# writingindy/SWMHD

Measured on AMD Instinct MI355X. Metric: Mcell-steps/sec (fp64) on 4096^2 periodic grid, higher is better.
Workload: dtype f64

## Files before the change

### include/swmhd.h

```cpp
#ifndef SWMHD_H
#define SWMHD_H

#include <stdint.h>

#ifdef __cplusplus
extern "C" {
#endif

#define SWMHD_VERSION 300

#define SWMHD_FAST 0
#define SWMHD_STRICT 1
#define SWMHD_TILE_KERNEL 2
#define SWMHD_MARCH_KERNEL 4
#define SWMHD_WRAP_X 16
#define SWMHD_WRAP_Y 32
#define SWMHD_BOUNDED_X 256
#define SWMHD_BOUNDED_Y 512
#define SWMHD_GM_IS_PREV_STATE 1024
#define SWMHD_LEAVE_ROOM 64

#define SWMHD_PERIODIC 0
#define SWMHD_BOUNDED 1

#define SWMHD_OK 0
#define SWMHD_EINVAL 1
#define SWMHD_EHALO 2
#define SWMHD_ENOTSUP 3
#define SWMHD_ECOMM 4

int swmhd_version(void);
const char *swmhd_strerror(int rc);

int swmhd_event_create(void **event);
int swmhd_event_record(void *event, void *stream);
int swmhd_event_elapsed_ms(void *start, void *stop, float *ms);
int swmhd_event_destroy(void *event);
int swmhd_probe_fp64_issue(double *scratch, float *ns_per_wave_instruction, void *stream);
int swmhd_probe_copy(void *dst, const void *src, size_t bytes, int reps, float *gbytes_per_s, void *stream);

int swmhd_lorentz_jacobian_f64(const double *A, const double *h, double *Fx, double *Fy,
                               int Nx, int Ny, int Hx, int Hy, int64_t stride_y,
                               double dx, double dy, int flags, void *stream);
int swmhd_lorentz_jacobian_f32(const float *A, const float *h, float *Fx, float *Fy,
                               int Nx, int Ny, int Hx, int Hy, int64_t stride_y,
                               float dx, float dy, int flags, void *stream);
int swmhd_lorentz_jacobian_rows_f64(const double *A, const double *h, double *Fx, double *Fy,
                                    int Nx, int Ny, int Hx, int Hy, int64_t stride_y,
                                    double dx, double dy, int j_begin, int j_end, int flags, void *stream);
int swmhd_lorentz_jacobian_rows_f32(const float *A, const float *h, float *Fx, float *Fy,
                                    int Nx, int Ny, int Hx, int Hy, int64_t stride_y,
                                    float dx, float dy, int j_begin, int j_end, int flags, void *stream);

int swmhd_lorentz_divergence_f64(const double *A, const double *h, double *Fx, double *Fy,
                                 int Nx, int Ny, int Hx, int Hy, int64_t stride_y,
                                 double dx, double dy, int flags, void *stream);
int swmhd_lorentz_divergence_f32(const float *A, const float *h, float *Fx, float *Fy,
                                 int Nx, int Ny, int Hx, int Hy, int64_t stride_y,
                                 float dx, float dy, int flags, void *stream);
int swmhd_lorentz_divergence_rows_f64(const double *A, const double *h, double *Fx, double *Fy,
                                      int Nx, int Ny, int Hx, int Hy, int64_t stride_y,
                                      double dx, double dy, int topo_x, int topo_y,
                                      int j_begin, int j_end, int flags, void *stream);
int swmhd_lorentz_divergence_rows_f32(const float *A, const float *h, float *Fx, float *Fy,
                                      int Nx, int Ny, int Hx, int Hy, int64_t stride_y,
                                      float dx, float dy, int topo_x, int topo_y,
                                      int j_begin, int j_end, int flags, void *stream);

#define SWMHD_HALO_X 1
#define SWMHD_HALO_Y 2
int swmhd_fill_halo_periodic_f64(double *field, int Nx, int Ny, int Hx, int Hy, int64_t stride_y,
                                 int which, void *stream);
int swmhd_fill_halo_periodic_f32(float *field, int Nx, int Ny, int Hx, int Hy, int64_t stride_y,
                                 int which, void *stream);

int swmhd_fill_halo_periodic_multi_f64(double *const *fields, int nfields, int Nx, int Ny, int Hx, int Hy,
                                       int64_t stride_y, int which, void *stream);
int swmhd_fill_halo_periodic_multi_f32(float *const *fields, int nfields, int Nx, int Ny, int Hx, int Hy,
                                       int64_t stride_y, int which, void *stream);

int swmhd_fill_halo_f64(double *const *fields, int nf, int Nx, int Ny, int Hx, int Hy, int64_t stride_y, int topo_x, int topo_y,
                        int face_x, int face_y, const double *gradient, double dx, double dy, void *stream);
int swmhd_fill_halo_f32(float *const *fields, int nf, int Nx, int Ny, int Hx, int Hy, int64_t stride_y, int topo_x, int topo_y,
                        int face_x, int face_y, const float *gradient, float dx, float dy, void *stream);

#define SWMHD_CONSERVATIVE 0
#define SWMHD_VECTOR_INVARIANT 1
#define SWMHD_LORENTZ_NONE 0
#define SWMHD_LORENTZ_JACOBIAN 1
#define SWMHD_LORENTZ_DIVERGENCE 2
int swmhd_tendencies_f64(const double *q1, const double *q2, const double *h, const double *A,
                         double *G1, double *G2, double *Gh, double *GA,
                         int Nx, int Ny, int Hx, int Hy, int64_t stride_y, double dx, double dy,
                         double g, double f, int formulation, int lorentz,
                         int j_begin, int j_end, int flags, void *stream);
int swmhd_tendencies_f32(const float *q1, const float *q2, const float *h, const float *A,
                         float *G1, float *G2, float *Gh, float *GA,
                         int Nx, int Ny, int Hx, int Hy, int64_t stride_y, float dx, float dy,
                         float g, float f, int formulation, int lorentz,
                         int j_begin, int j_end, int flags, void *stream);

int swmhd_rk3_substep_f64(double *const *U, const double *const *Gn, const double *const *Gm,
                          int Nx, int Ny, int Hx, int Hy, int64_t stride_y,
                          double dt, double gamma, double zeta, int j_begin, int j_end, int flags, void *stream);
int swmhd_rk3_substep_f32(float *const *U, const float *const *Gn, const float *const *Gm,
                          int Nx, int Ny, int Hx, int Hy, int64_t stride_y,
                          float dt, float gamma, float zeta, int j_begin, int j_end, int flags, void *stream);

int swmhd_tendencies_rk3_f64(const double *const *q, double *const *qnew, double *const *Gn, const double *const *Gm,
                             int Nx, int Ny, int Hx, int Hy, int64_t stride_y, double dx, double dy,
                             double g, double f, int formulation, int lorentz,
                             double dt, double gamma, double zeta, int store_G,
                             int j_begin, int j_end, int flags, void *stream);
int swmhd_tendencies_rk3_f32(const float *const *q, float *const *qnew, float *const *Gn, const float *const *Gm,
                             int Nx, int Ny, int Hx, int Hy, int64_t stride_y, float dx, float dy,
                             float g, float f, int formulation, int lorentz,
                             float dt, float gamma, float zeta, int store_G,
                             int j_begin, int j_end, int flags, void *stream);

int swmhd_step_rk3_f64(double *const *q, double *const *q_alt, double *const *Ga, double *const *Gb,
                       int Nx, int Ny, int Hx, int Hy, int64_t stride_y, double dx, double dy,
                       double g, double f, int formulation, int lorentz, double dt, int nsteps,
                       int flags, int *state_in_alt, void *stream);
int swmhd_step_rk3_f32(float *const *q, float *const *q_alt, float *const *Ga, float *const *Gb,
                       int Nx, int Ny, int Hx, int Hy, int64_t stride_y, float dx, float dy,
                       float g, float f, int formulation, int lorentz, float dt, int nsteps,
                       int flags, int *state_in_alt, void *stream);

int swmhd_tendency_launch_geometry(int Nx, int rows, int formulation, int elem_size, int flags, int out[8]);

#define SWMHD_RING_ID_BYTES 128
typedef struct swmhd_ring swmhd_ring;
int swmhd_ring_available(const char *rccl_path);
int swmhd_ring_unique_id(const char *rccl_path, void *id128);
int swmhd_ring_create(swmhd_ring **ring, const char *rccl_path, int nranks, int rank, const void *id128);
int swmhd_ring_create_loopback(swmhd_ring **rings, int nranks, double timeout_s);
int swmhd_ring_destroy(swmhd_ring *ring);
const char *swmhd_ring_last_error(const swmhd_ring *ring);
void *swmhd_ring_comm_stream(const swmhd_ring *ring);

int swmhd_ring_exchange_y_f64(swmhd_ring *ring, double *const *fields, int nfields, int Nx, int Ny, int Hx, int Hy,
                              int64_t stride_y, void *stream);
int swmhd_ring_exchange_y_f32(swmhd_ring *ring, float *const *fields, int nfields, int Nx, int Ny, int Hx, int Hy,
                              int64_t stride_y, void *stream);

int swmhd_ring_step_rk3_f64(swmhd_ring *ring, double *const *q, double *const *q_alt, double *const *Ga, double *const *Gb,
                            int Nx, int Ny, int Hx, int Hy, int64_t stride_y, double dx, double dy,
                            double g, double f, int formulation, int lorentz, double dt, int nsteps,
                            int flags, int *state_in_alt, void *stream);
int swmhd_ring_step_rk3_f32(swmhd_ring *ring, float *const *q, float *const *q_alt, float *const *Ga, float *const *Gb,
                            int Nx, int Ny, int Hx, int Hy, int64_t stride_y, float dx, float dy,
                            float g, float f, int formulation, int lorentz, float dt, int nsteps,
                            int flags, int *state_in_alt, void *stream);
int swmhd_ring_join(swmhd_ring *ring, void *stream);

int swmhd_ring_time_launches(swmhd_ring *ring, int max_launches);
int swmhd_ring_launch_times(swmhd_ring *ring, float *ms, int *rows, int capacity);

#define SWMHD_DIAG_NOUT 7
#define SWMHD_DIAG_WORKSPACE (1024 * 7)
int swmhd_diagnostics_f64(const double *q1, const double *q2, const double *h, const double *A,
                          int Nx, int Ny, int Hx, int Hy, int64_t stride_y, double dx, double dy,
                          double g, double h_ref, int formulation, int j_begin, int j_end,
                          double *workspace, double *out, void *stream);
int swmhd_diagnostics_f32(const float *q1, const float *q2, const float *h, const float *A,
                          int Nx, int Ny, int Hx, int Hy, int64_t stride_y, float dx, float dy,
                          float g, float h_ref, int formulation, int j_begin, int j_end,
                          double *workspace, double *out, void *stream);

#ifdef __cplusplus
}
#endif
#endif
```

### swmhd_amd/_lib.py

```python
import ctypes as C
import os

_HERE = os.path.dirname(os.path.abspath(__file__))
LIB_PATH = os.path.join(_HERE, "libswmhd.so")
_LIB = None

STRICT = 1
FAST = 0
TILE_KERNEL = 2
MARCH_KERNEL = 4
WRAP_X, WRAP_Y = 16, 32
LEAVE_ROOM = 64
GM_IS_PREV_STATE = 1024
BOUNDED_X, BOUNDED_Y = 256, 512
KERNEL_FLAGS = {None: 0, "auto": 0, "tile": 2, "march": 4}
PERIODIC, BOUNDED = 0, 1
HALO_X, HALO_Y = 1, 2
DIAG_NOUT, DIAG_WORKSPACE = 7, 1024 * 7
CONSERVATIVE, VECTOR_INVARIANT = 0, 1
LORENTZ_NONE, LORENTZ_JACOBIAN, LORENTZ_DIVERGENCE = 0, 1, 2


def ptr_array(ptrs):
    return (C.c_void_p * len(ptrs))(*ptrs)


class SwmhdError(RuntimeError):
    pass


def _declare(lib):
    p, i, i64 = C.c_void_p, C.c_int, C.c_int64
    lib.swmhd_version.restype = i
    lib.swmhd_strerror.restype = C.c_char_p
    lib.swmhd_strerror.argtypes = [i]
    lib.swmhd_event_create.argtypes = [C.POINTER(p)]
    lib.swmhd_event_record.argtypes = [p, p]
    lib.swmhd_event_elapsed_ms.argtypes = [p, p, C.POINTER(C.c_float)]
    lib.swmhd_event_destroy.argtypes = [p]
    for n in ("create", "record", "elapsed_ms", "destroy"):
        getattr(lib, "swmhd_event_" + n).restype = i
    lib.swmhd_probe_fp64_issue.argtypes = [p, C.POINTER(C.c_float), p]
    lib.swmhd_probe_fp64_issue.restype = i
    lib.swmhd_probe_copy.argtypes = [p, p, C.c_size_t, i, C.POINTER(C.c_float), p]
    lib.swmhd_probe_copy.restype = i
    for sfx, ft in (("f64", C.c_double), ("f32", C.c_float)):
        for form in ("jacobian", "divergence"):
            f = getattr(lib, f"swmhd_lorentz_{form}_{sfx}")
            f.argtypes = [p, p, p, p, i, i, i, i, i64, ft, ft, i, p]
            f.restype = i
        f = getattr(lib, f"swmhd_lorentz_jacobian_rows_{sfx}")
        f.argtypes = [p, p, p, p, i, i, i, i, i64, ft, ft, i, i, i, p]
        f.restype = i
        f = getattr(lib, f"swmhd_lorentz_divergence_rows_{sfx}")
        f.argtypes = [p, p, p, p, i, i, i, i, i64, ft, ft, i, i, i, i, i, p]
        f.restype = i
        f = getattr(lib, f"swmhd_fill_halo_periodic_{sfx}")
        f.argtypes = [p, i, i, i, i, i64, i, p]
        f.restype = i
        f = getattr(lib, f"swmhd_fill_halo_{sfx}")
        f.argtypes = [C.POINTER(p), i, i, i, i, i, i64, i, i, i, i, p, ft, ft, p]
        f.restype = i
        f = getattr(lib, f"swmhd_fill_halo_periodic_multi_{sfx}")
        f.argtypes = [C.POINTER(p), i, i, i, i, i, i64, i, p]
        f.restype = i
        f = getattr(lib, f"swmhd_tendencies_{sfx}")
        f.argtypes = [p] * 8 + [i, i, i, i, i64, ft, ft, ft, ft, i, i, i, i, i, p]
        f.restype = i
        f = getattr(lib, f"swmhd_tendencies_rk3_{sfx}")
        f.argtypes = [C.POINTER(p)] * 4 + [i, i, i, i, i64, ft, ft, ft, ft, i, i, ft, ft, ft, i, i, i, i, p]
        f.restype = i
        f = getattr(lib, f"swmhd_step_rk3_{sfx}")
        f.argtypes = [C.POINTER(p)] * 4 + [i, i, i, i, i64, ft, ft, ft, ft, i, i, ft, i, i, C.POINTER(i), p]
        f.restype = i
        f = getattr(lib, f"swmhd_diagnostics_{sfx}")
        f.argtypes = [p, p, p, p, i, i, i, i, i64, ft, ft, ft, ft, i, i, i, p, p, p]
        f.restype = i
        f = getattr(lib, f"swmhd_rk3_substep_{sfx}")
        f.argtypes = [C.POINTER(p), C.POINTER(p), C.POINTER(p), i, i, i, i, i64, ft, ft, ft, i, i, i, p]
        f.restype = i
        f = getattr(lib, f"swmhd_ring_exchange_y_{sfx}")
        f.argtypes = [p, C.POINTER(p), i, i, i, i, i, i64, p]
        f.restype = i
        f = getattr(lib, f"swmhd_ring_step_rk3_{sfx}")
        f.argtypes = [p] + [C.POINTER(p)] * 4 + [i, i, i, i, i64, ft, ft, ft, ft, i, i, ft, i, i, C.POINTER(i), p]
        f.restype = i
    lib.swmhd_tendency_launch_geometry.argtypes = [i, i, i, i, i, C.POINTER(i)]
    lib.swmhd_tendency_launch_geometry.restype = i
    lib.swmhd_ring_available.argtypes = [C.c_char_p]
    lib.swmhd_ring_available.restype = i
    lib.swmhd_ring_unique_id.argtypes = [C.c_char_p, p]
    lib.swmhd_ring_unique_id.restype = i
    lib.swmhd_ring_create.argtypes = [C.POINTER(p), C.c_char_p, i, i, p]
    lib.swmhd_ring_create.restype = i
    lib.swmhd_ring_create_loopback.argtypes = [C.POINTER(p), i, C.c_double]
    lib.swmhd_ring_create_loopback.restype = i
    lib.swmhd_ring_destroy.argtypes = [p]
    lib.swmhd_ring_destroy.restype = i
    lib.swmhd_ring_last_error.argtypes = [p]
    lib.swmhd_ring_last_error.restype = C.c_char_p
    lib.swmhd_ring_comm_stream.argtypes = [p]
    lib.swmhd_ring_comm_stream.restype = p
    lib.swmhd_ring_join.argtypes = [p, p]
    lib.swmhd_ring_join.restype = i
    lib.swmhd_ring_time_launches.argtypes = [p, i]
    lib.swmhd_ring_time_launches.restype = i
    lib.swmhd_ring_launch_times.argtypes = [p, C.POINTER(C.c_float), C.POINTER(i), i]
    lib.swmhd_ring_launch_times.restype = i


EXPORTS = ["swmhd_version", "swmhd_strerror", "swmhd_tendency_launch_geometry", "swmhd_probe_fp64_issue", "swmhd_probe_copy"] + ["swmhd_event_" + n for n in ("create", "record", "elapsed_ms", "destroy")] + [
    f"swmhd_{name}_{sfx}" for sfx in ("f64", "f32") for name in (
        "lorentz_jacobian", "lorentz_jacobian_rows", "lorentz_divergence", "lorentz_divergence_rows",
        "fill_halo", "fill_halo_periodic", "fill_halo_periodic_multi", "tendencies", "tendencies_rk3", "rk3_substep", "step_rk3", "diagnostics",
        "ring_exchange_y", "ring_step_rk3")] + [
    "swmhd_ring_" + name for name in ("available", "unique_id", "create", "create_loopback", "destroy", "last_error", "comm_stream", "join", "time_launches",
                                      "launch_times")]
RING_ID_BYTES = 128


class TimingEvent:

    def __init__(self):
        self._e = C.c_void_p()
        check(lib().swmhd_event_create(C.byref(self._e)), "swmhd_event_create")

    def record(self, stream=None):
        if stream is None:
            import torch
            stream = torch.cuda.current_stream().cuda_stream
        check(lib().swmhd_event_record(self._e, C.c_void_p(stream)), "swmhd_event_record")

    def elapsed_time(self, stop):
        ms = C.c_float()
        check(lib().swmhd_event_elapsed_ms(self._e, stop._e, C.byref(ms)), "swmhd_event_elapsed_ms")
        return ms.value

    def __del__(self):
        try:
            if self._e:
                lib().swmhd_event_destroy(self._e)
        except Exception:
            pass


def lib():
    global _LIB
    if _LIB is None:
        path = os.environ.get("SWMHD_LIBRARY", LIB_PATH)
        if not os.path.exists(path):
            raise SwmhdError(
                f"{path} not found: build it with `python -c 'import __graft_entry__ as g; g.build()'` "
                "(hipcc --offload-arch=gfx950).  swmhd_amd has no CPU fallback.")
        _LIB = C.CDLL(path)
        _declare(_LIB)
    return _LIB


def tendency_launch_geometry(Nx, rows, formulation, elem_size=8, flags=0):
    out = (C.c_int * 8)()
    check(lib().swmhd_tendency_launch_geometry(Nx, rows, formulation, elem_size, flags, out), "swmhd_tendency_launch_geometry")
    keys = ("kind", "threads", "nstrips", "nseg", "rows_per_segment", "wg_per_cu", "halo_lanes", "cus")
    return dict(zip(keys, list(out)))


def source_hash():
    import glob, hashlib
    h = hashlib.sha256()
    src = os.path.join(_HERE, "csrc")
    for f in sorted(glob.glob(os.path.join(src, "*.hip")) + glob.glob(os.path.join(src, "*.inc")) + glob.glob(os.path.join(src, "*.hpp"))
                    + [os.path.join(src, "Makefile")]):
        h.update(os.path.basename(f).encode()); h.update(open(f, "rb").read())
    return h.hexdigest()[:16]


def check(rc, what=""):
    if rc != 0:
        raise SwmhdError(f"{what}: rc={rc}: {lib().swmhd_strerror(rc).decode()}")
```

### swmhd_amd/csrc/common.hpp

```cpp
#pragma once
#include <hip/hip_runtime.h>
#include <stdint.h>
#include <stdio.h>
#include <stdlib.h>

namespace swmhd {

template <typename T>
struct OpArgs {
    const T *A;
    const T *h;
    T *Fx;
    T *Fy;
    int Nx, Ny, Hx, Hy;
    long sy;
    T dx, dy, rdx, rdy;
    int j0, j1;
    int topo_x, topo_y;
    int kernel_variant;
    int edge_cols;
};

template <typename T> hipError_t launch_lorentz_jacobian_fast(const OpArgs<T> &a, hipStream_t s);
template <typename T> hipError_t launch_lorentz_jacobian_strict(const OpArgs<T> &a, hipStream_t s);
template <typename T> hipError_t launch_lorentz_divergence_fast(const OpArgs<T> &a, hipStream_t s);
template <typename T> hipError_t launch_lorentz_divergence_strict(const OpArgs<T> &a, hipStream_t s);

template <typename T>
hipError_t launch_fill_halo_periodic(T *interior, int Nx, int Ny, int Hx, int Hy, long sy, int which, hipStream_t s);
template <typename T>
hipError_t launch_fill_halo_periodic_multi(T *const *interiors, int nfields, int Nx, int Ny, int Hx, int Hy, long sy,
                                           int which, hipStream_t s);
template <typename T>
struct HaloBc {
    T *f[4];
    T grad[4][4];
    int nf, Nx, Ny, Hx, Hy, topo_x, topo_y, face_x, face_y;
    long sy;
    T dx, dy;
};
template <typename T> hipError_t launch_fill_halo_bc(const HaloBc<T> &a, hipStream_t s);

template <typename T>
struct TendArgs {
    const T *q1, *q2, *h, *A;
    T *G1, *G2, *Gh, *GA;
    int Nx, Ny, Hx, Hy;
    long sy;
    T dx, dy, rdx, rdy, grav, fcor;
    int j0, j1;
    int j0b, j1b;
    int fuse, first, store_G;
    int gm_prev;
    int drop_G;
    int wrap;
    int kernel_variant;
    int topo_x, topo_y;
    int leave_room;
    int edge_cols;
    T *Unew[4];
    const T *Gm[4];
    T dt, gamma, zeta;
    T dtg;
    T cu, cg;
};
constexpr int GM_IS_PREV_STATE = 1024;
template <typename T>
struct Rk3Stage {
    T gamma, zeta;
    int store_G;
    const T *const *Gm;
    int flags;
};
template <typename T>
struct Rk3Buffers {
    T *cur[4], *alt[4], *gn[4], *gm[4];
    int swaps = 0;
    bool set(T *const *q, T *const *q_alt, T *const *Ga, T *const *Gb) {
        for (int f = 0; f < 4; ++f) {
            if (!q[f] || !q_alt[f] || !Ga[f] || !Gb[f]) return false;
            cur[f] = q[f]; alt[f] = q_alt[f]; gn[f] = Ga[f]; gm[f] = Gb[f];
        }
        return true;
    }
    Rk3Stage<T> stage(int st, bool from_state) const {
        const T gam[3] = {T(8.0 / 15.0), T(5.0 / 12.0), T(3.0 / 4.0)};
        const T zet[3] = {T(0), T(-17.0 / 60.0), T(-5.0 / 12.0)};
        const bool fs = from_state && st == 1;
        return {gam[st], fs ? zet[1] / gam[0] : zet[st], (st == 1 || (st == 0 && !from_state)) ? 1 : 0,
                st == 0 ? nullptr : (fs ? alt : gm), fs ? GM_IS_PREV_STATE : 0};
    }
    void rotate() {
        for (int f = 0; f < 4; ++f) { T *t = cur[f]; cur[f] = alt[f]; alt[f] = t; t = gn[f]; gn[f] = gm[f]; gm[f] = t; }
        ++swaps;
    }
};

template <typename T>
struct Rk3Args {
    T *U[4];
    const T *Gn[4];
    const T *Gm[4];
    int Nx;
    long sy;
    int j0, j1;
    T dt, gamma, zeta;
    int first;
};
typedef int sw_v2i __attribute__((ext_vector_type(2)));
typedef float sw_f2 __attribute__((ext_vector_type(2)));
typedef sw_f2 sw_f2_u __attribute__((aligned(4)));
constexpr unsigned SW_OOB = 0xFFFFFFC0u;
template <typename T> __device__ __forceinline__ __amdgpu_buffer_rsrc_t out_rsrc(T *parent, unsigned bytes) {
    return __builtin_amdgcn_make_buffer_rsrc(parent, 0, (int)bytes, 0x00020000);
}
template <typename T> __device__ __forceinline__ void buffer_store(T v, __amdgpu_buffer_rsrc_t r, unsigned off) {
    if constexpr (sizeof(T) == 8) __builtin_amdgcn_raw_buffer_store_b64(__builtin_bit_cast(sw_v2i, v), r, off, 0, 0);
    else __builtin_amdgcn_raw_buffer_store_b32(__builtin_bit_cast(int, v), r, off, 0, 0);
}
template <int N> __device__ __forceinline__ void wait_vmem_all_but() {
    static_assert(N >= 0 && N < 64, "vmcnt is a 6-bit counter");
    __builtin_amdgcn_s_waitcnt((N & 15) | ((N >> 4) << 14) | (7 << 4) | (15 << 8));
}

struct ProgressPriority {
    int t1, t2, t3;
    __device__ __forceinline__ explicit ProgressPriority(int niter)
        : t1((niter * 3) / 5), t2((niter * 17) / 20), t3((niter * 19) / 20) {
        __builtin_amdgcn_s_setprio(3);
    }
    __device__ __forceinline__ void at(int it) const {
        if (it == t1) __builtin_amdgcn_s_setprio(2);
        if (it == t2) __builtin_amdgcn_s_setprio(1);
        if (it == t3) __builtin_amdgcn_s_setprio(0);
    }
};

struct MarchGeometry {
    int nt;
    int nstrips, nseg, LY;
    int wg_per_cu;
};
inline int device_cu_count() {
    static int cus = 0;
    if (cus <= 0) {
        int dev = 0, n = 0;
        if (hipGetDevice(&dev) != hipSuccess || hipDeviceGetAttribute(&n, hipDeviceAttributeMultiprocessorCount, dev) != hipSuccess || n <= 0)
            n = 256;
        cus = n;
    }
    return cus;
}
inline int env_knob(const char *name, int &cache) {
    if (cache == 0) {
        const char *e = getenv(name);
        const int v = e ? atoi(e) : 0;
        cache = v > 0 ? v : -1;
    }
    return cache > 0 ? cache : 0;
}
inline int leave_room_64ths(int rows) {
    static int cache = 0;
    const int v = env_knob("SWMHD_RING_ROOM", cache);
    return v > 0 ? (v < 32 ? v : 32) : (rows >= 3072 ? 1 : 3);
}
inline MarchGeometry march_geometry(int Nx, int rows, int xh, const int *nts, const int *wgs, int ncand, int ly_min, bool leave_room,
                                    int force_nt, int force_ly) {
    MarchGeometry g{};
    long best = -1;
    for (int k = 0; k < ncand; ++k) {
        const int txo = nts[k] - 2 * xh, ns = (Nx + txo - 1) / txo;
        const long lanes = (long)ns * nts[k];
        const bool take = force_nt ? nts[k] == force_nt : (best < 0 || lanes * 20 <= best * 19);
        if (take) { best = lanes; g.nt = nts[k]; g.nstrips = ns; g.wg_per_cu = wgs[k]; }
    }
    if (best < 0) { g.nt = nts[0]; g.nstrips = (Nx + nts[0] - 2 * xh - 1) / (nts[0] - 2 * xh); g.wg_per_cu = wgs[0]; }
    int slots = device_cu_count() * g.wg_per_cu;
    if (leave_room) slots -= (slots * leave_room_64ths(rows)) / 64;
    int LY = 32;
    for (int k = 1; k <= 64; ++k) {
        const int ns = (slots * k) / g.nstrips;
        if (ns < 1) continue;
        const int ly = (rows + ns - 1) / ns;
        if (ly <= 128) { LY = ly < ly_min ? ly_min : ly; break; }
    }
    if (force_ly > 0) LY = force_ly;
    g.LY = LY;
    g.nseg = (rows + LY - 1) / LY;
    return g;
}

template <typename T> hipError_t launch_tendency_fast(const TendArgs<T> &a, int formulation, int lorentz, hipStream_t s);
int tendency_launch_geometry(int Nx, int rows, int formulation, int elem_size, int kernel_variant, int leave_room, int wrap, int out[8]);
template <typename T> hipError_t launch_tendency_strict(const TendArgs<T> &a, int formulation, int lorentz, hipStream_t s);
template <typename T> hipError_t launch_rk3_substep_fast(const Rk3Args<T> &a, hipStream_t s);
template <typename T>
int tendencies_rk3_two_ranges(const T *const *q, T *const *qnew, T *const *Gn, const T *const *Gm, int Nx, int Ny, int Hx, int Hy, long sy,
                              T dx, T dy, T grav, T fcor, int formulation, int lorentz, T dt, T gamma, T zeta, int store_G, int j0, int j1,
                              int j0b, int j1b, int flags, void *stream);
template <typename T>
int fill_halo_periodic_multi(T *const *f, int nf, int Nx, int Ny, int Hx, int Hy, long sy, int which, void *stream);
template <typename T> hipError_t launch_rk3_substep_strict(const Rk3Args<T> &a, hipStream_t s);

template <typename T>
hipError_t launch_diagnostics(const T *q1, const T *q2, const T *h, const T *A, int Nx, int Ny, int j0, int j1, long sy, T dx, T dy,
                              T grav, T href, int form, double *workspace, double *out, hipStream_t s);

__device__ __forceinline__ int wrap_index(int v, int n, int lo, int hi, bool wrap) {
    if (wrap) v = v < 0 ? v + n : (v >= n ? v - n : v);
    return v < lo ? lo : (v > hi ? hi : v);
}

__device__ __forceinline__ unsigned xcd_remap(unsigned bid, unsigned nblk) {
    constexpr unsigned NXCD = 8;
    unsigned q = nblk / NXCD, r = nblk % NXCD;
    unsigned x = bid % NXCD, k = bid / NXCD;
    unsigned base = x < r ? x * (q + 1) : r * (q + 1) + (x - r) * q;
    return base + k;
}

}
```

### swmhd_amd/csrc/ring.hip

```cpp
#include "common.hpp"
#include "../../include/swmhd.h"
#include <chrono>
#include <condition_variable>
#include <cstring>
#include <dlfcn.h>
#include <memory>
#include <mutex>
#include <new>
#include <rccl/rccl.h>
#include <string>
#include <vector>

namespace {

struct RcclApi {
    void *handle = nullptr;
    ncclResult_t (*GetUniqueId)(ncclUniqueId *) = nullptr;
    ncclResult_t (*CommInitRank)(ncclComm_t *, int, ncclUniqueId, int) = nullptr;
    ncclResult_t (*CommDestroy)(ncclComm_t) = nullptr;
    ncclResult_t (*GroupStart)() = nullptr;
    ncclResult_t (*GroupEnd)() = nullptr;
    ncclResult_t (*Send)(const void *, size_t, ncclDataType_t, int, ncclComm_t, hipStream_t) = nullptr;
    ncclResult_t (*Recv)(void *, size_t, ncclDataType_t, int, ncclComm_t, hipStream_t) = nullptr;
    const char *(*GetErrorString)(ncclResult_t) = nullptr;
};

bool load_rccl(const char *path, RcclApi &api, std::string &err) {
    const char *candidates[] = {path, "librccl.so.1", "librccl.so"};
    for (const char *c : candidates) {
        if (!c || !*c) continue;
        api.handle = dlopen(c, RTLD_NOW | RTLD_LOCAL);
        if (api.handle) break;
        err = dlerror();
    }
    if (!api.handle) return false;
#define SW_SYM(field, name)                                                                \
    api.field = reinterpret_cast<decltype(api.field)>(dlsym(api.handle, name));           \
    if (!api.field) { err = std::string("missing symbol ") + name; return false; }
    SW_SYM(GetUniqueId, "ncclGetUniqueId")
    SW_SYM(CommInitRank, "ncclCommInitRank")
    SW_SYM(CommDestroy, "ncclCommDestroy")
    SW_SYM(GroupStart, "ncclGroupStart")
    SW_SYM(GroupEnd, "ncclGroupEnd")
    SW_SYM(Send, "ncclSend")
    SW_SYM(Recv, "ncclRecv")
    SW_SYM(GetErrorString, "ncclGetErrorString")
#undef SW_SYM
    return true;
}

struct LoopHub {
    static constexpr int MAXF = 8, SLOTS = 4;
    struct Post {
        unsigned long seq = 0;
        unsigned long done = 0;
        const char *send_s[SLOTS][MAXF] = {}, *send_n[SLOTS][MAXF] = {};
        size_t bytes[SLOTS] = {};
        int nf[SLOTS] = {};
        hipEvent_t ready[SLOTS] = {}, consumed[SLOTS] = {};
    };
    std::mutex mu;
    std::condition_variable cv;
    std::vector<Post> post;
    double timeout_s = 60.0;
    explicit LoopHub(int n) : post(n) {}
    ~LoopHub() {
        for (auto &p : post)
            for (int k = 0; k < SLOTS; ++k) { if (p.ready[k]) (void)hipEventDestroy(p.ready[k]); if (p.consumed[k]) (void)hipEventDestroy(p.consumed[k]); }
    }
};

}

struct swmhd_ring {
    RcclApi api;
    ncclComm_t comm = nullptr;
    std::shared_ptr<LoopHub> hub;
    int nranks = 1, rank = 0, south = 0, north = 0;
    hipStream_t comm_stream = nullptr;
    hipEvent_t ev_main = nullptr, ev_comm = nullptr;
    const void *pending = nullptr;
    std::string err;
    std::vector<hipEvent_t> t0, t1;
    std::vector<int> trows;
    size_t tcap = 0;
};

namespace {

int fail(swmhd_ring *r, const char *what, ncclResult_t rc) {
    r->err = std::string(what) + ": " + (r->api.GetErrorString ? r->api.GetErrorString(rc) : "rccl error");
    return SWMHD_ECOMM;
}
int hipfail(swmhd_ring *r, const char *what, hipError_t e) {
    r->err = std::string(what) + ": " + hipGetErrorString(e);
    return -(int)e;
}

template <typename T> constexpr ncclDataType_t nccl_type();
template <> constexpr ncclDataType_t nccl_type<double>() { return ncclFloat64; }
template <> constexpr ncclDataType_t nccl_type<float>() { return ncclFloat32; }

int loopback_exchange(swmhd_ring *r, const char *const *send_s, const char *const *send_n, char *const *recv_s, char *const *recv_n,
                      int nf, size_t bytes, hipStream_t s) {
    LoopHub &h = *r->hub;
    if (nf > LoopHub::MAXF) return SWMHD_EINVAL;
    hipError_t e;
    unsigned long k;
    int slot;
    {
        std::unique_lock<std::mutex> lk(h.mu);
        LoopHub::Post &me = h.post[r->rank];
        k = me.seq + 1; slot = (int)(k % LoopHub::SLOTS);
        if (!me.ready[slot] && (e = hipEventCreateWithFlags(&me.ready[slot], hipEventDisableTiming)) != hipSuccess) return hipfail(r, "loopback event", e);
        if (!me.consumed[slot] && (e = hipEventCreateWithFlags(&me.consumed[slot], hipEventDisableTiming)) != hipSuccess) return hipfail(r, "loopback event", e);
        if ((e = hipEventRecord(me.ready[slot], s)) != hipSuccess) return hipfail(r, "loopback record", e);
        for (int f = 0; f < nf; ++f) { me.send_s[slot][f] = send_s[f]; me.send_n[slot][f] = send_n[f]; }
        me.bytes[slot] = bytes; me.nf[slot] = nf;
        me.seq = k;
    }
    h.cv.notify_all();
    const auto deadline = std::chrono::steady_clock::now() + std::chrono::duration<double>(h.timeout_s);
    auto wait_for = [&](auto pred, const char *what) {
        std::unique_lock<std::mutex> lk(h.mu);
        if (!h.cv.wait_until(lk, deadline, pred)) {
            r->err = std::string("loopback exchange ") + std::to_string(k) + " of rank " + std::to_string(r->rank) + ": " + what +
                     " (every ring of the hub must be driven from its own host thread, and all of them must make the same calls)";
            return false;
        }
        return true;
    };
    const int peers[2] = {r->south, r->north};
    for (int side = 0; side < 2; ++side) {
        const int p = peers[side];
        if (!wait_for([&] { return h.post[p].seq >= k; }, "a neighbour did not reach its matching exchange")) return SWMHD_ECOMM;
        hipEvent_t ready; const char *src[LoopHub::MAXF]; size_t pbytes; int pnf;
        {
            std::unique_lock<std::mutex> lk(h.mu);
            const LoopHub::Post &pp = h.post[p];
            ready = pp.ready[slot]; pbytes = pp.bytes[slot]; pnf = pp.nf[slot];
            for (int f = 0; f < nf && f < pnf; ++f) src[f] = side == 0 ? pp.send_n[slot][f] : pp.send_s[slot][f];
        }
        if (pbytes != bytes || pnf != nf) { r->err = "loopback exchange: neighbour posted a different message (fields / bytes)"; return SWMHD_ECOMM; }
        if ((e = hipStreamWaitEvent(s, ready, 0)) != hipSuccess) return hipfail(r, "loopback wait", e);
        for (int f = 0; f < nf; ++f)
            if ((e = hipMemcpyAsync(side == 0 ? recv_s[f] : recv_n[f], src[f], bytes, hipMemcpyDeviceToDevice, s)) != hipSuccess)
                return hipfail(r, "loopback copy", e);
    }
    {
        std::unique_lock<std::mutex> lk(h.mu);
        LoopHub::Post &me = h.post[r->rank];
        if ((e = hipEventRecord(me.consumed[slot], s)) != hipSuccess) return hipfail(r, "loopback record", e);
        me.done = k;
    }
    h.cv.notify_all();
    for (int side = 0; side < 2; ++side) {
        const int p = peers[side];
        if (!wait_for([&] { return h.post[p].done >= k; }, "a neighbour did not take the rows sent to it")) return SWMHD_ECOMM;
        hipEvent_t consumed;
        { std::unique_lock<std::mutex> lk(h.mu); consumed = h.post[p].consumed[slot]; }
        if ((e = hipStreamWaitEvent(s, consumed, 0)) != hipSuccess) return hipfail(r, "loopback wait", e);
    }
    return SWMHD_OK;
}

template <typename T>
int exchange(swmhd_ring *r, T *const *fields, int nf, int Nx, int Ny, int Hx, int Hy, int64_t sy, hipStream_t s) {
    if (!r || !fields || nf <= 0) return SWMHD_EINVAL;
    if (Nx <= 0 || Ny < Hy || Hy <= 0 || sy < (int64_t)Nx + 2 * Hx) return SWMHD_EINVAL;
    const size_t count = (size_t)Hy * (size_t)sy;
    if (r->hub) {
        if (nf > LoopHub::MAXF) return SWMHD_EINVAL;
        const char *ss[LoopHub::MAXF], *sn[LoopHub::MAXF]; char *rs[LoopHub::MAXF], *rn[LoopHub::MAXF];
        for (int f = 0; f < nf; ++f) {
            T *p = fields[f];
            if (!p) return SWMHD_EINVAL;
            ss[f] = (const char *)(p + (size_t)Hy * sy); sn[f] = (const char *)(p + (size_t)Ny * sy);
            rs[f] = (char *)p; rn[f] = (char *)(p + (size_t)(Ny + Hy) * sy);
        }
        return loopback_exchange(r, ss, sn, rs, rn, nf, count * sizeof(T), s);
    }
    ncclResult_t rc = r->api.GroupStart();
    if (rc != ncclSuccess) return fail(r, "ncclGroupStart", rc);
    for (int f = 0; f < nf; ++f) {
        T *p = fields[f];
        if (!p) { r->api.GroupEnd(); return SWMHD_EINVAL; }
        T *send_s = p + (size_t)Hy * sy, *send_n = p + (size_t)Ny * sy;
        T *recv_s = p, *recv_n = p + (size_t)(Ny + Hy) * sy;
        if ((rc = r->api.Send(send_n, count, nccl_type<T>(), r->north, r->comm, s)) != ncclSuccess) break;
        if ((rc = r->api.Recv(recv_s, count, nccl_type<T>(), r->south, r->comm, s)) != ncclSuccess) break;
        if ((rc = r->api.Send(send_s, count, nccl_type<T>(), r->south, r->comm, s)) != ncclSuccess) break;
        if ((rc = r->api.Recv(recv_n, count, nccl_type<T>(), r->north, r->comm, s)) != ncclSuccess) break;
    }
    ncclResult_t rc2 = r->api.GroupEnd();
    if (rc != ncclSuccess) return fail(r, "ncclSend/ncclRecv", rc);
    if (rc2 != ncclSuccess) return fail(r, "ncclGroupEnd", rc2);
    return SWMHD_OK;
}

template <typename T>
int ring_step(swmhd_ring *r, T *const *q, T *const *q_alt, T *const *Ga, T *const *Gb, int Nx, int Ny, int Hx, int Hy, int64_t sy,
              T dx, T dy, T grav, T fcor, int formulation, int lorentz, T dt, int nsteps, int flags, int *state_in_alt,
              void *stream) {
    if (!r || !q || !q_alt || !Ga || !Gb || nsteps < 0) return SWMHD_EINVAL;
    if (flags & SWMHD_WRAP_Y) return SWMHD_EINVAL;
    if (Ny < 2 * Hy + 1) return SWMHD_EINVAL;
    hipStream_t s = (hipStream_t)stream, c = r->comm_stream;
    swmhd::Rk3Buffers<T> b;
    if (!b.set(q, q_alt, Ga, Gb)) return SWMHD_EINVAL;
    if (r->pending && r->pending != (const void *)b.cur[0]) {
        hipError_t e = hipEventRecord(r->ev_comm, c);
        if (e == hipSuccess) e = hipStreamWaitEvent(s, r->ev_comm, 0);
        if (e != hipSuccess) return hipfail(r, "join", e);
        r->pending = nullptr;
    }
    hipError_t e;
    const bool from_state = !(flags & SWMHD_STRICT);
    if ((e = hipEventRecord(r->ev_main, s)) != hipSuccess) return hipfail(r, "record", e);
    if ((e = hipStreamWaitEvent(c, r->ev_main, 0)) != hipSuccess) return hipfail(r, "wait", e);
    auto bail = [&](int code) {
        if (hipEventRecord(r->ev_comm, c) == hipSuccess) (void)hipStreamWaitEvent(s, r->ev_comm, 0);
        r->pending = nullptr;
        if (state_in_alt) *state_in_alt = b.swaps & 1;
        return code;
    };
    auto run = [&](const swmhd::Rk3Stage<T> &g, int j0, int j1, int j0b, int j1b, int fl, hipStream_t on) {
        return swmhd::tendencies_rk3_two_ranges<T>(b.cur, b.alt, b.gn, g.Gm, Nx, Ny, Hx, Hy, (long)sy, dx, dy, grav, fcor, formulation,
                                                   lorentz, dt, g.gamma, g.zeta, g.store_G, j0, j1, j0b, j1b, fl | g.flags, (void *)on);
    };
    auto run_interior = [&](const swmhd::Rk3Stage<T> &g, int j0, int j1, int fl) {
        if (r->t0.size() >= r->tcap) return run(g, j0, j1, 0, 0, fl, s);
        hipEvent_t t0 = nullptr, t1 = nullptr;
        if ((e = hipEventCreateWithFlags(&t0, hipEventDisableSystemFence)) != hipSuccess) return hipfail(r, "hipEventCreate", e);
        if ((e = hipEventCreateWithFlags(&t1, hipEventDisableSystemFence)) != hipSuccess) { (void)hipEventDestroy(t0); return hipfail(r, "hipEventCreate", e); }
        (void)hipEventRecord(t0, s);
        const int rc = run(g, j0, j1, 0, 0, fl, s);
        if (rc) { (void)hipEventDestroy(t0); (void)hipEventDestroy(t1); return rc; }
        (void)hipEventRecord(t1, s);
        r->t0.push_back(t0); r->t1.push_back(t1); r->trows.push_back(j1 - j0);
        return 0;
    };
    if ((flags & SWMHD_WRAP_X) && Hy >= 9 && Ny >= 32) {
        const int ilo[3] = {3, 9, 12}, blo[3] = {-6, -3, 0};
        const int bflags = flags | ((!(flags & (SWMHD_STRICT | SWMHD_TILE_KERNEL | SWMHD_MARCH_KERNEL)) && Nx >= 1024) ? SWMHD_MARCH_KERNEL : 0);
        for (int n = 0; n < nsteps; ++n) {
            for (int st = 0; st < 3; ++st) {
                const swmhd::Rk3Stage<T> g = b.stage(st, from_state);
                if (int rc = run_interior(g, ilo[st], Ny - ilo[st], flags | SWMHD_LEAVE_ROOM)) return bail(rc);
                if (st < 2) {
                    if ((e = hipEventRecord(r->ev_main, s)) != hipSuccess) return bail(hipfail(r, "record", e));
                }
                if (int rc = run(g, blo[st], ilo[st], Ny - ilo[st], Ny - blo[st], bflags, c)) return bail(rc);
                if (st < 2) {
                    if ((e = hipStreamWaitEvent(c, r->ev_main, 0)) != hipSuccess) return bail(hipfail(r, "wait", e));
                }
                b.rotate();
            }
            r->pending = nullptr;
            if ((e = hipEventRecord(r->ev_comm, c)) != hipSuccess) return bail(hipfail(r, "record", e));
            if ((e = hipStreamWaitEvent(s, r->ev_comm, 0)) != hipSuccess) return bail(hipfail(r, "wait", e));
            if (int rc = exchange<T>(r, b.cur, 4, Nx, Ny, Hx, Hy, sy, c)) return bail(rc);
            r->pending = b.cur[0];
        }
        if (state_in_alt) *state_in_alt = b.swaps & 1;
        return SWMHD_OK;
    }
    for (int n = 0; n < nsteps; ++n)
        for (int st = 0; st < 3; ++st) {
            const swmhd::Rk3Stage<T> g = b.stage(st, from_state);
            int rc;
            const bool split = r->pending != nullptr;
            if ((rc = split ? run_interior(g, Hy, Ny - Hy, flags | SWMHD_LEAVE_ROOM) : run_interior(g, 0, Ny, flags))) return bail(rc);
            if (split) {
                if ((rc = run(g, 0, Hy, Ny - Hy, Ny, flags, c))) return bail(rc);
                if ((e = hipEventRecord(r->ev_comm, c)) != hipSuccess) return bail(hipfail(r, "record", e));
                if ((e = hipStreamWaitEvent(s, r->ev_comm, 0)) != hipSuccess) return bail(hipfail(r, "wait", e));
            }
            b.rotate();
            r->pending = nullptr;
            if (split && (flags & SWMHD_WRAP_X)) {
                if ((rc = exchange<T>(r, b.cur, 4, Nx, Ny, Hx, Hy, sy, c))) return bail(rc);
                r->pending = b.cur[0];
                if ((e = hipEventRecord(r->ev_main, s)) != hipSuccess) return bail(hipfail(r, "record", e));
                if ((e = hipStreamWaitEvent(c, r->ev_main, 0)) != hipSuccess) return bail(hipfail(r, "wait", e));
                continue;
            }
            if (!(flags & SWMHD_WRAP_X) && (rc = swmhd::fill_halo_periodic_multi<T>(b.cur, 4, Nx, Ny, Hx, Hy, (long)sy, SWMHD_HALO_X, (void *)s)))
                return bail(rc);
            if ((e = hipEventRecord(r->ev_main, s)) != hipSuccess) return bail(hipfail(r, "record", e));
            if ((e = hipStreamWaitEvent(c, r->ev_main, 0)) != hipSuccess) return bail(hipfail(r, "wait", e));
            if ((rc = exchange<T>(r, b.cur, 4, Nx, Ny, Hx, Hy, sy, c))) return bail(rc);
            r->pending = b.cur[0];
        }
    if (state_in_alt) *state_in_alt = b.swaps & 1;
    return SWMHD_OK;
}

}

extern "C" {

int swmhd_ring_available(const char *rccl_path) {
    RcclApi api;
    std::string err;
    return load_rccl(rccl_path, api, err) ? SWMHD_OK : SWMHD_ENOTSUP;
}

int swmhd_ring_unique_id(const char *rccl_path, void *id128) {
    if (!id128) return SWMHD_EINVAL;
    RcclApi api;
    std::string err;
    if (!load_rccl(rccl_path, api, err)) return SWMHD_ENOTSUP;
    ncclUniqueId id;
    if (api.GetUniqueId(&id) != ncclSuccess) return SWMHD_ECOMM;
    static_assert(sizeof(id) == SWMHD_RING_ID_BYTES, "ncclUniqueId size");
    memcpy(id128, &id, sizeof(id));
    return SWMHD_OK;
}

int swmhd_ring_create(swmhd_ring **out, const char *rccl_path, int nranks, int rank, const void *id128) {
    if (!out || !id128 || nranks < 1 || rank < 0 || rank >= nranks) return SWMHD_EINVAL;
    swmhd_ring *r = new (std::nothrow) swmhd_ring;
    if (!r) return SWMHD_EINVAL;
    if (!load_rccl(rccl_path, r->api, r->err)) { delete r; return SWMHD_ENOTSUP; }
    r->nranks = nranks; r->rank = rank;
    r->south = (rank + nranks - 1) % nranks;
    r->north = (rank + 1) % nranks;
    ncclUniqueId id;
    memcpy(&id, id128, sizeof(id));
    if (r->api.CommInitRank(&r->comm, nranks, id, rank) != ncclSuccess) { delete r; return SWMHD_ECOMM; }
    int lo = 0, hi = 0;
    (void)hipDeviceGetStreamPriorityRange(&lo, &hi);
    hipError_t e = hipStreamCreateWithPriority(&r->comm_stream, hipStreamNonBlocking, hi);
    if (e == hipSuccess) e = hipEventCreateWithFlags(&r->ev_main, hipEventDisableTiming);
    if (e == hipSuccess) e = hipEventCreateWithFlags(&r->ev_comm, hipEventDisableTiming);
    if (e != hipSuccess) { swmhd_ring_destroy(r); return -(int)e; }
    *out = r;
    return SWMHD_OK;
}

int swmhd_ring_create_loopback(swmhd_ring **out, int nranks, double timeout_s) {
    if (!out || nranks < 1 || nranks > 64) return SWMHD_EINVAL;
    std::shared_ptr<LoopHub> hub;
    try { hub = std::make_shared<LoopHub>(nranks); } catch (...) { return SWMHD_EINVAL; }
    if (timeout_s > 0) hub->timeout_s = timeout_s;
    int lo = 0, hi = 0;
    (void)hipDeviceGetStreamPriorityRange(&lo, &hi);
    for (int k = 0; k < nranks; ++k) out[k] = nullptr;
    for (int k = 0; k < nranks; ++k) {
        swmhd_ring *r = new (std::nothrow) swmhd_ring;
        hipError_t e = r ? hipSuccess : hipErrorOutOfMemory;
        if (r) {
            r->hub = hub; r->nranks = nranks; r->rank = k;
            r->south = (k + nranks - 1) % nranks; r->north = (k + 1) % nranks;
            e = hipStreamCreateWithPriority(&r->comm_stream, hipStreamNonBlocking, hi);
            if (e == hipSuccess) e = hipEventCreateWithFlags(&r->ev_main, hipEventDisableTiming);
            if (e == hipSuccess) e = hipEventCreateWithFlags(&r->ev_comm, hipEventDisableTiming);
        }
        if (e != hipSuccess) {
            if (r) swmhd_ring_destroy(r);
            for (int j = 0; j < k; ++j) { swmhd_ring_destroy(out[j]); out[j] = nullptr; }
            return -(int)e;
        }
        out[k] = r;
    }
    return SWMHD_OK;
}

int swmhd_ring_destroy(swmhd_ring *r) {
    if (!r) return SWMHD_OK;
    if (r->comm_stream) (void)hipStreamSynchronize(r->comm_stream);
    for (auto ev : r->t0) (void)hipEventDestroy(ev);
    for (auto ev : r->t1) (void)hipEventDestroy(ev);
    if (r->comm) r->api.CommDestroy(r->comm);
    if (r->ev_main) (void)hipEventDestroy(r->ev_main);
    if (r->ev_comm) (void)hipEventDestroy(r->ev_comm);
    if (r->comm_stream) (void)hipStreamDestroy(r->comm_stream);
    delete r;
    return SWMHD_OK;
}

const char *swmhd_ring_last_error(const swmhd_ring *r) { return r ? r->err.c_str() : "null ring"; }

void *swmhd_ring_comm_stream(const swmhd_ring *r) { return r ? (void *)r->comm_stream : nullptr; }

int swmhd_ring_join(swmhd_ring *r, void *stream) {
    if (!r) return SWMHD_EINVAL;
    if (!r->pending) return SWMHD_OK;
    hipError_t e = hipEventRecord(r->ev_comm, r->comm_stream);
    if (e == hipSuccess) e = hipStreamWaitEvent((hipStream_t)stream, r->ev_comm, 0);
    if (e != hipSuccess) return hipfail(r, "join", e);
    r->pending = nullptr;
    return SWMHD_OK;
}

int swmhd_ring_time_launches(swmhd_ring *r, int max_launches) {
    if (!r || max_launches < 0) return SWMHD_EINVAL;
    for (auto ev : r->t0) (void)hipEventDestroy(ev);
    for (auto ev : r->t1) (void)hipEventDestroy(ev);
    r->t0.clear(); r->t1.clear(); r->trows.clear();
    r->tcap = (size_t)max_launches;
    return SWMHD_OK;
}

int swmhd_ring_launch_times(swmhd_ring *r, float *ms, int *rows, int capacity) {
    if (!r || !ms || !rows) return -1;
    int n = 0;
    for (size_t i = 0; i < r->t0.size() && n < capacity; ++i) {
        if (hipEventSynchronize(r->t1[i]) != hipSuccess) break;
        if (hipEventElapsedTime(&ms[n], r->t0[i], r->t1[i]) != hipSuccess) break;
        rows[n++] = r->trows[i];
    }
    return n;
}

#define SWMHD_DEF_RING(sfx, T)                                                                                                   \
    int swmhd_ring_exchange_y_##sfx(swmhd_ring *r, T *const *fields, int nfields, int Nx, int Ny, int Hx, int Hy, int64_t sy,    \
                                    void *stream) {                                                                              \
        return exchange<T>(r, fields, nfields, Nx, Ny, Hx, Hy, sy, (hipStream_t)stream);                                         \
    }                                                                                                                            \
    int swmhd_ring_step_rk3_##sfx(swmhd_ring *r, T *const *q, T *const *q_alt, T *const *Ga, T *const *Gb, int Nx, int Ny,       \
                                  int Hx, int Hy, int64_t sy, T dx, T dy, T g, T f, int formulation, int lorentz, T dt,          \
                                  int nsteps, int flags, int *state_in_alt, void *stream) {                                      \
        return ring_step<T>(r, q, q_alt, Ga, Gb, Nx, Ny, Hx, Hy, sy, dx, dy, g, f, formulation, lorentz, dt, nsteps, flags,      \
                            state_in_alt, stream);                                                                               \
    }

SWMHD_DEF_RING(f64, double)
SWMHD_DEF_RING(f32, float)

}
```

### swmhd_amd/csrc/swmhd_api.hip

```cpp
#include "../../include/swmhd.h"
#include "common.hpp"
#include <math.h>

using namespace swmhd;

namespace {

inline int hiprc(hipError_t e) { return e == hipSuccess ? SWMHD_OK : -(int)e; }

template <typename T>
int lorentz_common(bool divergence, const T *A, const T *h, T *Fx, T *Fy, int Nx, int Ny, int Hx, int Hy,
                   int64_t sy, T dx, T dy, int topo_x, int topo_y, int j_begin, int j_end, int flags, void *stream) {
    if (!A || !h || !Fx || !Fy) return SWMHD_EINVAL;
    if (Nx <= 0 || Ny <= 0 || Hx < 0 || Hy < 0 || sy < (int64_t)Nx + 2 * Hx) return SWMHD_EINVAL;
    if (!(dx > T(0)) || !(dy > T(0))) return SWMHD_EINVAL;
    if (j_begin < 0 || j_end > Ny || j_begin > j_end) return SWMHD_EINVAL;
    const int need = divergence ? 3 : 2;
    if (Hx < need || Hy < need) return SWMHD_EHALO;
    if ((topo_x != SWMHD_BOUNDED && topo_x != SWMHD_PERIODIC) || (topo_y != SWMHD_BOUNDED && topo_y != SWMHD_PERIODIC))
        return SWMHD_EINVAL;
    if (!divergence && (topo_x != SWMHD_PERIODIC || topo_y != SWMHD_PERIODIC)) return SWMHD_EINVAL;
    if (flags & ~(SWMHD_STRICT | SWMHD_TILE_KERNEL | SWMHD_MARCH_KERNEL)) return SWMHD_EINVAL;
    if (j_begin == j_end) return SWMHD_OK;
    OpArgs<T> a;
    a.kernel_variant = (flags & SWMHD_TILE_KERNEL) ? 1 : ((flags & SWMHD_MARCH_KERNEL) ? 2 : 0);
    const long off = (long)Hy * sy + Hx;
    a.A = A + off; a.h = h + off; a.Fx = Fx + off; a.Fy = Fy + off;
    a.Nx = Nx; a.Ny = Ny; a.Hx = Hx; a.Hy = Hy; a.sy = (long)sy;
    a.dx = dx; a.dy = dy; a.rdx = T(1) / dx; a.rdy = T(1) / dy;
    a.j0 = j_begin; a.j1 = j_end; a.topo_x = topo_x; a.topo_y = topo_y;
    a.edge_cols = 0;
    hipStream_t s = (hipStream_t)stream;
    const bool strict = (flags & SWMHD_STRICT) != 0;
    hipError_t e;
    if (divergence) e = strict ? launch_lorentz_divergence_strict<T>(a, s) : launch_lorentz_divergence_fast<T>(a, s);
    else e = strict ? launch_lorentz_jacobian_strict<T>(a, s) : launch_lorentz_jacobian_fast<T>(a, s);
    return hiprc(e);
}

template <typename T>
int halo_common(T *f, int Nx, int Ny, int Hx, int Hy, int64_t sy, int which, void *stream) {
    if (!f || Nx <= 0 || Ny <= 0 || Hx < 0 || Hy < 0 || sy < (int64_t)Nx + 2 * Hx) return SWMHD_EINVAL;
    if (Hx > Nx || Hy > Ny) return SWMHD_EHALO;
    if (which & ~(SWMHD_HALO_X | SWMHD_HALO_Y)) return SWMHD_EINVAL;
    return hiprc(launch_fill_halo_periodic<T>(f + (long)Hy * sy + Hx, Nx, Ny, Hx, Hy, (long)sy, which, (hipStream_t)stream));
}

template <typename T>
int halo_multi_common(T *const *f, int nf, int Nx, int Ny, int Hx, int Hy, int64_t sy, int which, void *stream) {
    if (!f || nf < 1 || nf > 4 || Nx <= 0 || Ny <= 0 || Hx < 0 || Hy < 0 || sy < (int64_t)Nx + 2 * Hx) return SWMHD_EINVAL;
    if (Hx > Nx || Hy > Ny) return SWMHD_EHALO;
    if (which & ~(SWMHD_HALO_X | SWMHD_HALO_Y)) return SWMHD_EINVAL;
    T *p[4] = {nullptr, nullptr, nullptr, nullptr};
    for (int k = 0; k < nf; ++k) {
        if (!f[k]) return SWMHD_EINVAL;
        p[k] = f[k] + (long)Hy * sy + Hx;
    }
    return hiprc(launch_fill_halo_periodic_multi<T>(p, nf, Nx, Ny, Hx, Hy, (long)sy, which, (hipStream_t)stream));
}

template <typename T>
int halo_bc_common(T *const *f, int nf, int Nx, int Ny, int Hx, int Hy, int64_t sy, int topo_x, int topo_y, int face_x, int face_y,
                   const T *gradient, T dx, T dy, void *stream) {
    if (!f || nf < 1 || nf > 4 || Nx <= 0 || Ny <= 0 || Hx < 0 || Hy < 0 || sy < (int64_t)Nx + 2 * Hx) return SWMHD_EINVAL;
    if ((topo_x != SWMHD_BOUNDED && topo_x != SWMHD_PERIODIC) || (topo_y != SWMHD_BOUNDED && topo_y != SWMHD_PERIODIC)) return SWMHD_EINVAL;
    if (Hx > Nx || Hy > Ny) return SWMHD_EHALO;
    if ((topo_x == SWMHD_BOUNDED && Hx < 1) || (topo_y == SWMHD_BOUNDED && Hy < 1)) return SWMHD_EHALO;
    if (!(dx > T(0)) || !(dy > T(0))) return SWMHD_EINVAL;
    HaloBc<T> a;
    for (int k = 0; k < 4; ++k) {
        a.f[k] = nullptr;
        for (int e = 0; e < 4; ++e) a.grad[k][e] = (gradient && k < nf) ? gradient[4 * k + e] : T(NAN);
    }
    for (int k = 0; k < nf; ++k) {
        if (!f[k]) return SWMHD_EINVAL;
        a.f[k] = f[k] + (long)Hy * sy + Hx;
    }
    a.nf = nf; a.Nx = Nx; a.Ny = Ny; a.Hx = Hx; a.Hy = Hy; a.topo_x = topo_x; a.topo_y = topo_y; a.face_x = face_x; a.face_y = face_y;
    a.sy = (long)sy; a.dx = dx; a.dy = dy;
    return hiprc(launch_fill_halo_bc<T>(a, (hipStream_t)stream));
}

template <typename T>
struct FuseRk3 {
    T *Unew[4];
    const T *const *Gm;
    T dt, gamma, zeta;
    int store_G;
};

template <typename T>
int tend_common(const T *q1, const T *q2, const T *h, const T *A, T *G1, T *G2, T *Gh, T *GA, int Nx, int Ny, int Hx, int Hy,
                int64_t sy, T dx, T dy, T grav, T fcor, int formulation, int lorentz, int j0, int j1, int flags, void *stream,
                const FuseRk3<T> *rk = nullptr, int j0b = 0, int j1b = 0) {
    if (!q1 || !q2 || !h || !A || !G1 || !G2 || !Gh || !GA) return SWMHD_EINVAL;
    if (Nx <= 0 || Ny <= 0 || Hx < 0 || Hy < 0 || sy < (int64_t)Nx + 2 * Hx) return SWMHD_EINVAL;
    if (!(dx > T(0)) || !(dy > T(0))) return SWMHD_EINVAL;
    const int ext = ((flags & (SWMHD_WRAP_Y | SWMHD_BOUNDED_Y)) || Hy < 3) ? 0 : Hy - 3;
    if (j0 < -ext || j1 > Ny + ext || j0 > j1) return SWMHD_EINVAL;
    if (j1b > j0b && (j0b < j1 || j1b > Ny + ext)) return SWMHD_EINVAL;
    if (flags & ~(SWMHD_STRICT | SWMHD_TILE_KERNEL | SWMHD_MARCH_KERNEL | SWMHD_WRAP_X | SWMHD_WRAP_Y | SWMHD_LEAVE_ROOM | SWMHD_BOUNDED_X | SWMHD_BOUNDED_Y | SWMHD_GM_IS_PREV_STATE)) return SWMHD_EINVAL;
    if (flags & SWMHD_GM_IS_PREV_STATE) {
        if (!rk || !rk->Gm) return SWMHD_EINVAL;
        if (flags & (SWMHD_STRICT | SWMHD_BOUNDED_X | SWMHD_BOUNDED_Y)) return SWMHD_ENOTSUP;
    }
    if (((flags & SWMHD_BOUNDED_X) && (flags & SWMHD_WRAP_X)) || ((flags & SWMHD_BOUNDED_Y) && (flags & SWMHD_WRAP_Y))) return SWMHD_EINVAL;
    if ((flags & (SWMHD_BOUNDED_X | SWMHD_BOUNDED_Y)) && (flags & SWMHD_MARCH_KERNEL)) return SWMHD_ENOTSUP;
    if (((flags & SWMHD_WRAP_X) && Hx > Nx) || ((flags & SWMHD_WRAP_Y) && Hy > Ny)) return SWMHD_EHALO;
    if (formulation != SWMHD_CONSERVATIVE && formulation != SWMHD_VECTOR_INVARIANT) return SWMHD_EINVAL;
    const bool ok = lorentz == SWMHD_LORENTZ_NONE || (formulation == SWMHD_VECTOR_INVARIANT && lorentz == SWMHD_LORENTZ_JACOBIAN) ||
                    (formulation == SWMHD_CONSERVATIVE && lorentz == SWMHD_LORENTZ_DIVERGENCE);
    if (!ok) return SWMHD_EINVAL;
    if (Hx < 3 || Hy < 3) return SWMHD_EHALO;
    if (j0 == j1 && j1b <= j0b) return SWMHD_OK;
    TendArgs<T> a;
    const long off = (long)Hy * sy + Hx;
    a.q1 = q1 + off; a.q2 = q2 + off; a.h = h + off; a.A = A + off;
    a.G1 = G1 + off; a.G2 = G2 + off; a.Gh = Gh + off; a.GA = GA + off;
    a.Nx = Nx; a.Ny = Ny; a.Hx = Hx; a.Hy = Hy; a.sy = (long)sy;
    a.dx = dx; a.dy = dy; a.rdx = T(1) / dx; a.rdy = T(1) / dy; a.grav = grav; a.fcor = fcor; a.j0 = j0; a.j1 = j1;
    a.j0b = j1b > j0b ? j0b : 0; a.j1b = j1b > j0b ? j1b : 0;
    a.fuse = 0; a.first = 0; a.store_G = 1; a.drop_G = 0; a.dt = a.gamma = a.zeta = T(0);
    a.gm_prev = (flags & SWMHD_GM_IS_PREV_STATE) ? 1 : 0; a.cu = a.cg = a.dtg = T(0);
    a.wrap = ((flags & SWMHD_WRAP_X) ? 1 : 0) | ((flags & SWMHD_WRAP_Y) ? 2 : 0);
    a.leave_room = (flags & SWMHD_LEAVE_ROOM) ? 1 : 0;
    a.edge_cols = 0;
    a.topo_x = (flags & SWMHD_BOUNDED_X) ? SWMHD_BOUNDED : SWMHD_PERIODIC; a.topo_y = (flags & SWMHD_BOUNDED_Y) ? SWMHD_BOUNDED : SWMHD_PERIODIC;
    a.kernel_variant = (flags & SWMHD_TILE_KERNEL) ? 1 : ((flags & SWMHD_MARCH_KERNEL) ? 2 : 0);
    for (int f = 0; f < 4; ++f) { a.Unew[f] = nullptr; a.Gm[f] = nullptr; }
    if (rk) {
        a.fuse = 1; a.first = rk->Gm ? 0 : 1; a.store_G = rk->store_G; a.dt = rk->dt; a.gamma = rk->gamma; a.zeta = rk->zeta;
        a.cu = a.gm_prev ? rk->zeta : T(0); a.cg = a.gm_prev ? -rk->zeta : rk->dt * rk->zeta; a.dtg = rk->dt * rk->gamma;
        for (int f = 0; f < 4; ++f) { a.Unew[f] = rk->Unew[f] + off; a.Gm[f] = rk->Gm ? rk->Gm[f] + off : nullptr; }
    }
    hipStream_t s = (hipStream_t)stream;
    return hiprc((flags & SWMHD_STRICT) ? launch_tendency_strict<T>(a, formulation, lorentz, s)
                                        : launch_tendency_fast<T>(a, formulation, lorentz, s));
}

template <typename T>
int tend_rk3_common(const T *const *q, T *const *qnew, T *const *Gn, const T *const *Gm, int Nx, int Ny, int Hx, int Hy, int64_t sy,
                    T dx, T dy, T grav, T fcor, int formulation, int lorentz, T dt, T gamma, T zeta, int store_G, int j0, int j1,
                    int flags, void *stream, int j0b = 0, int j1b = 0) {
    if (!q || !qnew || !Gn) return SWMHD_EINVAL;
    for (int f = 0; f < 4; ++f) {
        if (!q[f] || !qnew[f] || !Gn[f] || (Gm && !Gm[f])) return SWMHD_EINVAL;
        for (int k = 0; k < 4; ++k)
            if (qnew[f] == q[k]) return SWMHD_EINVAL;
    }
    FuseRk3<T> rk{{qnew[0], qnew[1], qnew[2], qnew[3]}, Gm, dt, gamma, zeta, store_G ? 1 : 0};
    return tend_common<T>(q[0], q[1], q[2], q[3], Gn[0], Gn[1], Gn[2], Gn[3], Nx, Ny, Hx, Hy, sy, dx, dy, grav, fcor, formulation,
                          lorentz, j0, j1, flags, stream, &rk, j0b, j1b);
}

template <typename T>
int rk3_common(T *const *U, const T *const *Gn, const T *const *Gm, int Nx, int Ny, int Hx, int Hy, int64_t sy, T dt, T gamma,
               T zeta, int j0, int j1, int flags, void *stream) {
    if (!U || !Gn || Nx <= 0 || Ny <= 0 || Hx < 0 || Hy < 0 || sy < (int64_t)Nx + 2 * Hx) return SWMHD_EINVAL;
    if (j0 < 0 || j1 > Ny || j0 > j1 || (flags & ~SWMHD_STRICT)) return SWMHD_EINVAL;
    Rk3Args<T> a;
    const long off = (long)Hy * sy + Hx;
    for (int f = 0; f < 4; ++f) {
        if (!U[f] || !Gn[f] || (Gm && !Gm[f])) return SWMHD_EINVAL;
        a.U[f] = U[f] + off; a.Gn[f] = Gn[f] + off; a.Gm[f] = Gm ? Gm[f] + off : Gn[f] + off;
    }
    a.Nx = Nx; a.sy = (long)sy; a.j0 = j0; a.j1 = j1; a.dt = dt; a.gamma = gamma; a.zeta = zeta; a.first = Gm ? 0 : 1;
    hipStream_t s = (hipStream_t)stream;
    return hiprc((flags & SWMHD_STRICT) ? launch_rk3_substep_strict<T>(a, s) : launch_rk3_substep_fast<T>(a, s));
}

template <typename T>
int step_common(T *const *q, T *const *q_alt, T *const *Ga, T *const *Gb, int Nx, int Ny, int Hx, int Hy, int64_t sy, T dx, T dy, T grav,
                T fcor, int formulation, int lorentz, T dt, int nsteps, int flags, int *state_in_alt, void *stream) {
    if (!q || !q_alt || !Ga || !Gb || nsteps < 0) return SWMHD_EINVAL;
    if (flags & (SWMHD_BOUNDED_X | SWMHD_BOUNDED_Y)) return SWMHD_ENOTSUP;
    Rk3Buffers<T> b;
    if (!b.set(q, q_alt, Ga, Gb)) return SWMHD_EINVAL;
    const bool from_state = !(flags & SWMHD_STRICT);
    const int need = (SWMHD_HALO_X | SWMHD_HALO_Y) & ~(((flags & SWMHD_WRAP_X) ? SWMHD_HALO_X : 0) | ((flags & SWMHD_WRAP_Y) ? SWMHD_HALO_Y : 0));
    for (int n = 0; n < nsteps; ++n)
        for (int st = 0; st < 3; ++st) {
            const Rk3Stage<T> g = b.stage(st, from_state);
            int rc = tend_rk3_common<T>(b.cur, b.alt, b.gn, g.Gm, Nx, Ny, Hx, Hy, sy, dx, dy, grav, fcor, formulation, lorentz, dt, g.gamma,
                                        g.zeta, g.store_G, 0, Ny, flags | g.flags, stream);
            if (rc) return rc;
            b.rotate();
            if (need && (rc = halo_multi_common<T>(b.cur, 4, Nx, Ny, Hx, Hy, sy, need, stream))) return rc;
        }
    if (state_in_alt) *state_in_alt = b.swaps & 1;
    return SWMHD_OK;
}

template <typename T>
int diag_common(const T *q1, const T *q2, const T *h, const T *A, int Nx, int Ny, int Hx, int Hy, int64_t sy, T dx, T dy, T grav,
                T href, int form, int j0, int j1, double *ws, double *out, void *stream) {
    if (!q1 || !q2 || !h || !A || !ws || !out) return SWMHD_EINVAL;
    if (Nx <= 0 || Ny <= 0 || Hx < 0 || Hy < 0 || sy < (int64_t)Nx + 2 * Hx || !(dx > T(0)) || !(dy > T(0))) return SWMHD_EINVAL;
    if (j0 < 0 || j1 > Ny || j0 > j1) return SWMHD_EINVAL;
    if (form != SWMHD_CONSERVATIVE && form != SWMHD_VECTOR_INVARIANT) return SWMHD_EINVAL;
    if (Hx < 1 || Hy < 1) return SWMHD_EHALO;
    const long off = (long)Hy * sy + Hx;
    return hiprc(launch_diagnostics<T>(q1 + off, q2 + off, h + off, A + off, Nx, Ny, j0, j1, (long)sy, dx, dy, grav, href, form, ws,
                                       out, (hipStream_t)stream));
}

}

namespace swmhd {
template <typename T>
int tendencies_rk3_two_ranges(const T *const *q, T *const *qnew, T *const *Gn, const T *const *Gm, int Nx, int Ny, int Hx, int Hy, long sy,
                              T dx, T dy, T grav, T fcor, int formulation, int lorentz, T dt, T gamma, T zeta, int store_G, int j0, int j1,
                              int j0b, int j1b, int flags, void *stream) {
    return tend_rk3_common<T>(q, qnew, Gn, Gm, Nx, Ny, Hx, Hy, (int64_t)sy, dx, dy, grav, fcor, formulation, lorentz, dt, gamma, zeta,
                              store_G, j0, j1, flags, stream, j0b, j1b);
}
template <typename T>
int fill_halo_periodic_multi(T *const *f, int nf, int Nx, int Ny, int Hx, int Hy, long sy, int which, void *stream) {
    return halo_multi_common<T>(f, nf, Nx, Ny, Hx, Hy, (int64_t)sy, which, stream);
}
static_assert(GM_IS_PREV_STATE == SWMHD_GM_IS_PREV_STATE, "common.hpp mirrors swmhd.h");
#define SW_INST(T)                                                                                                                   \
    template int tendencies_rk3_two_ranges<T>(const T *const *, T *const *, T *const *, const T *const *, int, int, int, int, long, T, \
                                              T, T, T, int, int, T, T, T, int, int, int, int, int, int, void *);                      \
    template int fill_halo_periodic_multi<T>(T *const *, int, int, int, int, int, long, int, void *);
SW_INST(double)
SW_INST(float)
#undef SW_INST
}

extern "C" {

int swmhd_version(void) { return SWMHD_VERSION; }

const char *swmhd_strerror(int rc) {
    switch (rc) {
        case SWMHD_OK: return "success";
        case SWMHD_EINVAL: return "invalid argument (null pointer, bad extents, stride, spacing, row range or flags)";
        case SWMHD_EHALO: return "halo too small for the operator's stencil (Jacobian form needs 2, divergence form 3)";
        case SWMHD_ENOTSUP: return "not supported by this build (or: the RCCL library could not be loaded)";
        case SWMHD_ECOMM: return "RCCL reported an error (swmhd_ring_last_error has its text)";
        default: return rc < 0 ? hipGetErrorString((hipError_t)(-rc)) : "unknown swmhd error";
    }
}

int swmhd_event_create(void **event) {
    if (!event) return SWMHD_EINVAL;
    hipEvent_t e;
    const hipError_t rc = hipEventCreateWithFlags(&e, hipEventDisableSystemFence);
    if (rc != hipSuccess) return hiprc(rc);
    *event = (void *)e;
    return SWMHD_OK;
}
int swmhd_event_record(void *event, void *stream) {
    return event ? hiprc(hipEventRecord((hipEvent_t)event, (hipStream_t)stream)) : SWMHD_EINVAL;
}
int swmhd_event_elapsed_ms(void *start, void *stop, float *ms) {
    if (!start || !stop || !ms) return SWMHD_EINVAL;
    const hipError_t rc = hipEventSynchronize((hipEvent_t)stop);
    if (rc != hipSuccess) return hiprc(rc);
    return hiprc(hipEventElapsedTime(ms, (hipEvent_t)start, (hipEvent_t)stop));
}
int swmhd_event_destroy(void *event) { return event ? hiprc(hipEventDestroy((hipEvent_t)event)) : SWMHD_OK; }

int swmhd_tendency_launch_geometry(int Nx, int rows, int formulation, int elem_size, int flags, int out[8]) {
    if (!out || Nx <= 0 || rows <= 0 || (elem_size != 4 && elem_size != 8)) return SWMHD_EINVAL;
    if (formulation != SWMHD_CONSERVATIVE && formulation != SWMHD_VECTOR_INVARIANT) return SWMHD_EINVAL;
    const int variant = (flags & SWMHD_TILE_KERNEL) ? 1 : ((flags & SWMHD_MARCH_KERNEL) ? 2 : 0);
    return tendency_launch_geometry(Nx, rows, formulation, elem_size, (flags & SWMHD_STRICT) ? 1 : variant, (flags & SWMHD_LEAVE_ROOM) ? 1 : 0,
                                    ((flags & SWMHD_WRAP_X) ? 1 : 0) | ((flags & SWMHD_WRAP_Y) ? 2 : 0), out);
}

#define SWMHD_DEF_LORENTZ(sfx, T)                                                                                      \
    int swmhd_lorentz_jacobian_##sfx(const T *A, const T *h, T *Fx, T *Fy, int Nx, int Ny, int Hx, int Hy,            \
                                     int64_t sy, T dx, T dy, int flags, void *stream) {                                \
        return lorentz_common<T>(false, A, h, Fx, Fy, Nx, Ny, Hx, Hy, sy, dx, dy, 0, 0, 0, Ny, flags, stream);         \
    }                                                                                                                  \
    int swmhd_lorentz_jacobian_rows_##sfx(const T *A, const T *h, T *Fx, T *Fy, int Nx, int Ny, int Hx, int Hy,       \
                                          int64_t sy, T dx, T dy, int j0, int j1, int flags, void *stream) {           \
        return lorentz_common<T>(false, A, h, Fx, Fy, Nx, Ny, Hx, Hy, sy, dx, dy, 0, 0, j0, j1, flags, stream);        \
    }                                                                                                                  \
    int swmhd_lorentz_divergence_##sfx(const T *A, const T *h, T *Fx, T *Fy, int Nx, int Ny, int Hx, int Hy,          \
                                       int64_t sy, T dx, T dy, int flags, void *stream) {                              \
        return lorentz_common<T>(true, A, h, Fx, Fy, Nx, Ny, Hx, Hy, sy, dx, dy, 0, 0, 0, Ny, flags, stream);          \
    }                                                                                                                  \
    int swmhd_lorentz_divergence_rows_##sfx(const T *A, const T *h, T *Fx, T *Fy, int Nx, int Ny, int Hx, int Hy,     \
                                            int64_t sy, T dx, T dy, int tx, int ty, int j0, int j1, int flags,         \
                                            void *stream) {                                                            \
        return lorentz_common<T>(true, A, h, Fx, Fy, Nx, Ny, Hx, Hy, sy, dx, dy, tx, ty, j0, j1, flags, stream);       \
    }                                                                                                                  \
    int swmhd_fill_halo_periodic_##sfx(T *f, int Nx, int Ny, int Hx, int Hy, int64_t sy, int which, void *stream) {    \
        return halo_common<T>(f, Nx, Ny, Hx, Hy, sy, which, stream);                                                   \
    }                                                                                                                  \
    int swmhd_fill_halo_##sfx(T *const *f, int nf, int Nx, int Ny, int Hx, int Hy, int64_t sy, int topo_x, int topo_y,  \
                              int face_x, int face_y, const T *gradient, T dx, T dy, void *stream) {                       \
        return halo_bc_common<T>(f, nf, Nx, Ny, Hx, Hy, sy, topo_x, topo_y, face_x, face_y, gradient, dx, dy, stream);     \
    }                                                                                                                  \
    int swmhd_fill_halo_periodic_multi_##sfx(T *const *f, int nf, int Nx, int Ny, int Hx, int Hy, int64_t sy,          \
                                             int which, void *stream) {                                                \
        return halo_multi_common<T>(f, nf, Nx, Ny, Hx, Hy, sy, which, stream);                                         \
    }                                                                                                                  \
    int swmhd_tendencies_##sfx(const T *q1, const T *q2, const T *h, const T *A, T *G1, T *G2, T *Gh, T *GA, int Nx,   \
                               int Ny, int Hx, int Hy, int64_t sy, T dx, T dy, T g, T f, int formulation, int lorentz, \
                               int j0, int j1, int flags, void *stream) {                                              \
        return tend_common<T>(q1, q2, h, A, G1, G2, Gh, GA, Nx, Ny, Hx, Hy, sy, dx, dy, g, f, formulation, lorentz,    \
                              j0, j1, flags, stream);                                                                  \
    }                                                                                                                  \
    int swmhd_tendencies_rk3_##sfx(const T *const *q, T *const *qnew, T *const *Gn, const T *const *Gm, int Nx, int Ny, \
                                   int Hx, int Hy, int64_t sy, T dx, T dy, T g, T f, int formulation, int lorentz, T dt, \
                                   T gamma, T zeta, int store_G, int j0, int j1, int flags, void *stream) {              \
        return tend_rk3_common<T>(q, qnew, Gn, Gm, Nx, Ny, Hx, Hy, sy, dx, dy, g, f, formulation, lorentz, dt, gamma,   \
                                  zeta, store_G, j0, j1, flags, stream);                                                \
    }                                                                                                                  \
    int swmhd_diagnostics_##sfx(const T *q1, const T *q2, const T *h, const T *A, int Nx, int Ny, int Hx, int Hy,      \
                                int64_t sy, T dx, T dy, T g, T href, int form, int j0, int j1, double *ws, double *out, \
                                void *stream) {                                                                        \
        return diag_common<T>(q1, q2, h, A, Nx, Ny, Hx, Hy, sy, dx, dy, g, href, form, j0, j1, ws, out, stream);       \
    }                                                                                                                  \
    int swmhd_step_rk3_##sfx(T *const *q, T *const *q_alt, T *const *Ga, T *const *Gb, int Nx, int Ny, int Hx, int Hy,   \
                             int64_t sy, T dx, T dy, T g, T f, int formulation, int lorentz, T dt, int nsteps, int flags,\
                             int *state_in_alt, void *stream) {                                                        \
        return step_common<T>(q, q_alt, Ga, Gb, Nx, Ny, Hx, Hy, sy, dx, dy, g, f, formulation, lorentz, dt, nsteps, flags, \
                              state_in_alt, stream);                                                                   \
    }                                                                                                                  \
    int swmhd_rk3_substep_##sfx(T *const *U, const T *const *Gn, const T *const *Gm, int Nx, int Ny, int Hx, int Hy,   \
                                int64_t sy, T dt, T gamma, T zeta, int j0, int j1, int flags, void *stream) {          \
        return rk3_common<T>(U, Gn, Gm, Nx, Ny, Hx, Hy, sy, dt, gamma, zeta, j0, j1, flags, stream);                   \
    }

SWMHD_DEF_LORENTZ(f64, double)
SWMHD_DEF_LORENTZ(f32, float)

}
```

### swmhd_amd/csrc/tendency_march_kernels.inc

```

template <typename TA> __device__ __forceinline__ void segment_rows(const TA &a, int seg, int LY, int &J0, int &J1) {
    const int nsa = (a.j1 - a.j0 + LY - 1) / LY;
    const bool second = seg >= nsa;
    const int base = second ? a.j0b + (seg - nsa) * LY : a.j0 + seg * LY, end = second ? a.j1b : a.j1;
    J0 = base;
    J1 = base + LY < end ? base + LY : end;
}

template <typename T, int LOR, int NT, int MODE>
__global__ __launch_bounds__(NT, 3) void k_tendency_vi_march(TendArgs<T> a, int nstrips, int nseg, int LY) {
    constexpr bool FUSE = (MODE & 1) != 0, HAS_GM = (MODE & 2) != 0, STORE_G = (MODE & 4) != 0;
    constexpr int XH = 3, RW = NT + 2 * XH, TXO = NT - 2 * XH;
    __shared__ T Ru[3][RW];
    __shared__ T Rvn[1][RW];
    __shared__ __attribute__((aligned(16))) T RHA[4][RW][2];
    __shared__ T RBx[3][RW];
    __shared__ T RBy[3][RW];
    __shared__ T RFh[1][RW];
    __shared__ T RFA[1][RW];
    __shared__ T RK[1][RW];
    __shared__ T RZUV[RW][3];

    const unsigned bid = xcd_remap(blockIdx.x, (unsigned)(nstrips * nseg));
    const int strip = (int)(bid % nstrips), seg = (int)(bid / nstrips);
    const int x0 = strip * TXO;
    int J0, J1;
    segment_rows(a, seg, LY, J0, J1);
    const int c = threadIdx.x, lc = c + XH;
    const int gx = x0 - XH + c;
    const bool wx = (a.wrap & 1) != 0, wy = (a.wrap & 2) != 0;
    const int gxc = wrap_index(gx, a.Nx, -a.Hx, a.Nx + a.Hx - 1, wx);
    const int ylo = -a.Hy, yhi = a.Ny + a.Hy - 1;
    const T rdx = a.rdx, rdy = a.rdy;
    const Geo<T> g{a.dx, a.dy, a.rdx, a.rdy};
    const bool col_ok = (c >= XH) && (c < NT - XH) && (gx < a.Nx);

    T uw[8], vw[7], zw[7], svw[7], hw[7], aw[7];
    T fhy = T(0), fay = T(0), km = T(0);

    const long off0 = (long)a.Hy * a.sy + a.Hx;
    const int isy = (int)a.sy;
    auto LD = [&](const T *interior, unsigned ob) -> T { return *reinterpret_cast<const T *>(reinterpret_cast<const char *>(interior - off0) + ob); };
    const unsigned colb = (unsigned)(gxc + a.Hx) * (unsigned)sizeof(T);
    auto rowoff = [&](int row) -> unsigned { return (unsigned)((row + a.Hy) * isy) * (unsigned)sizeof(T); };
    const unsigned pbytes = (unsigned)((a.Ny + 2 * a.Hy) * isy) * (unsigned)sizeof(T);
    __amdgpu_buffer_rsrc_t rG[4], rU[4];
    if constexpr (STORE_G) {
        rG[0] = out_rsrc(a.G1 - off0, pbytes); rG[1] = out_rsrc(a.G2 - off0, pbytes);
        rG[2] = out_rsrc(a.Gh - off0, pbytes); rG[3] = out_rsrc(a.GA - off0, pbytes);
    }
    if constexpr (FUSE) {
#pragma unroll
        for (int f = 0; f < 4; ++f) rU[f] = out_rsrc(a.Unew[f] - off0, pbytes);
    }

    {
        const unsigned colm = (unsigned)(wrap_index(gx - 1, a.Nx, -a.Hx, a.Nx + a.Hx - 1, wx) + a.Hx) * (unsigned)sizeof(T);
        const unsigned colp = (unsigned)(wrap_index(gx + 1, a.Nx, -a.Hx, a.Nx + a.Hx - 1, wx) + a.Hx) * (unsigned)sizeof(T);
        unsigned ro[7];
#pragma unroll
        for (int k = 0; k < 7; ++k) ro[k] = rowoff(wrap_index(J0 - 3 + k, a.Ny, ylo, yhi, wy));
        T pu[7], pv[7], ph[7], pa[7], pvl[5];
#pragma unroll
        for (int k = 0; k < 7; ++k) { pu[k] = LD(a.q1, ro[k] + colb); pv[k] = LD(a.q2, ro[k] + colb); ph[k] = LD(a.h, ro[k] + colb); pa[k] = LD(a.A, ro[k] + colb); }
#pragma unroll
        for (int k = 0; k < 5; ++k) pvl[k] = LD(a.q2, ro[k + 1] + colm);
        const T ue_m = LD(a.q1, ro[2] + colp);
        T a_wm = T(0), a_em = T(0), a_wo = T(0), a_eo = T(0);
        if constexpr (LOR == 1) {
            a_wm = LD(a.A, ro[2] + colm); a_em = LD(a.A, ro[2] + colp);
            a_wo = LD(a.A, ro[3] + colm); a_eo = LD(a.A, ro[3] + colp);
        }
#pragma unroll
        for (int k = 0; k < 7; ++k) uw[k] = pu[k];
#pragma unroll
        for (int k = 0; k < 6; ++k) { vw[k] = pv[k + 1]; hw[k] = ph[k + 1]; aw[k] = pa[k + 1]; }
#pragma unroll
        for (int k = 0; k < 5; ++k) {
            zw[k] = (pv[k + 1] - pvl[k]) * rdx - (pu[k + 1] - pu[k]) * rdy;
            svw[k] = pvl[k] + pv[k + 1];
        }
        uw[7] = T(0); vw[6] = T(0); zw[5] = T(0); zw[6] = T(0); svw[5] = T(0); svw[6] = T(0); hw[6] = T(1); aw[6] = T(0);
        fhy = upwind_weno<T>(vw[2], ph);
        fay = upwind_weno<T>(vw[2], pa);
        km = T(0.25) * ((sq(uw[2]) + sq(ue_m)) + (sq(vw[1]) + sq(vw[2])));
        const int q3o = ((J0 % 3) + 3) % 3, q3m = (q3o + 2) % 3;
        Ru[q3m][lc] = uw[2];
        RHA[(J0 - 1) & 3][lc][0] = aw[1];
        RHA[J0 & 3][lc][0] = aw[2];
        if constexpr (LOR == 1) {
            const T rhm = recip<T>(hw[1]), rho = recip<T>(hw[2]);
            RBy[q3m][lc] = (T(0.5) * rdx) * (a_em - a_wm) * rhm;
            RBx[q3m][lc] = -(T(0.5) * rdy) * (aw[2] - aw[0]) * rhm;
            RBy[q3o][lc] = (T(0.5) * rdx) * (a_eo - a_wo) * rho;
            RBx[q3o][lc] = -(T(0.5) * rdy) * (aw[3] - aw[1]) * rho;
        }
    }

    auto body = [&](const int it) {
        constexpr int LU = 7, LW = 6;
        T *const U = uw, *const V = vw, *const Z = zw, *const SV = svw, *const Hh = hw, *const Aa = aw;
        const int jr = J0 - 3 + it;
        const int jo = jr - 3;
        {
            const unsigned ob = rowoff(wrap_index(jr + 1, a.Ny, ylo, yhi, wy)) + colb;
            uw[LU] = LD(a.q1, ob); vw[LW] = LD(a.q2, ob); hw[LW] = LD(a.h, ob); aw[LW] = LD(a.A, ob);
        }
        T gm0 = T(0), gm1 = T(0), gm2 = T(0), gm3 = T(0);
        const unsigned rowb = rowoff(jo);

        const int s3o = ((jo % 3) + 3) % 3, s3m = (s3o + 2) % 3, s3p = (s3o + 1) % 3;
        const int s4o = jo & 3, s4p = (jo + 1) & 3;

        Ru[s3o][lc] = U[3];
        RHA[s4o][lc][1] = Hh[2];
        RHA[s4p][lc][0] = Aa[3];
        Rvn[0][lc] = V[5];
        __syncthreads();

        {
            const T vl = Rvn[0][lc - 1];
            Z[5] = (V[5] - vl) * rdx - (U[6] - U[5]) * rdy;
            SV[5] = vl + V[5];
        }
        if constexpr (LOR == 1) {
            const T cxA = RHA[s4p][lc + 1][0] - RHA[s4p][lc - 1][0];
            const T cyA = Aa[4] - Aa[2];
            const T rh = recip<T>(Hh[3]);
            RBy[s3p][lc] = (T(0.5) * rdx) * cxA * rh;
            RBx[s3p][lc] = -(T(0.5) * rdy) * cyA * rh;
        }
        {
            const T ue2 = Ru[s3o][lc + 1];
            RK[0][lc] = T(0.25) * ((sq(U[3]) + sq(ue2)) + (sq(V[2]) + sq(V[3])));
        }
        RZUV[lc][0] = Z[2];
        RZUV[lc][1] = T(0.5) * (U[2] + U[3]);
        RZUV[lc][2] = T(0.5) * SV[2];
        {
            const T uadv = U[3];
            const bool pos = uadv >= T(0);
            const int base = pos ? lc - 3 : lc + 2, st = pos ? 1 : -1;
            T qh[5], qa[5];
#pragma unroll
            for (int k = 0; k < 5; ++k) { const T *r = RHA[s4o][base + st * k]; qa[k] = r[0]; qh[k] = r[1]; }
            RFh[0][lc] = uadv * weno5_upwind_ordered<T>(qh, pos);
            RFA[0][lc] = uadv * weno5_upwind_ordered<T>(qa, pos);
        }
        __syncthreads();
        if constexpr (FUSE && HAS_GM) {
            const unsigned og = rowb + colb;
            gm0 = LD(a.Gm[0], og); gm1 = LD(a.Gm[1], og); gm2 = LD(a.Gm[2], og); gm3 = LD(a.Gm[3], og);
        }

        const T fhy_n = upwind_weno<T>(V[3], Hh);
        const T fay_n = upwind_weno<T>(V[3], Aa);
        const T vhat = T(0.25) * (SV[2] + SV[3]);
        const T vortU = -upwind_weno_vel_raw<T>(vhat, Z, U, SV);
        const T *su0 = Ru[s3m], *su1 = Ru[s3o];
        const T ue = su1[lc + 1];
        const T uhat = T(0.25) * ((su0[lc] + su0[lc + 1]) + (U[3] + ue));
        T vortV;
        {
            const bool pos = uhat >= T(0);
            const int base = pos ? lc - 2 : lc + 3, st = pos ? 1 : -1;
            T zx[5], ufx[5], vfx[5];
#pragma unroll
            for (int k = 0; k < 5; ++k) { const T *r = RZUV[base + st * k]; zx[k] = r[0]; ufx[k] = r[1]; vfx[k] = r[2]; }
            vortV = uhat * weno5_vel_upwind_ordered<T>(zx, ufx, vfx, pos);
        }
        const T kc = RK[0][lc], kl = RK[0][lc - 1];
        const T hl = RHA[s4o][lc - 1][1];
        T Fx = T(0), Fy = T(0);
        if constexpr (LOR == 1) {
            auto A_ = [&](int di, int dj) -> T { return di == 0 ? Aa[2 + dj] : RHA[(jo + dj) & 3][lc + di][0]; };
            auto H_ = [&](int di, int dj) -> T { return di == 0 ? Hh[2 + dj] : hl; };
            auto BX_ = [&](int di, int dj) -> T { return RBx[dj < 0 ? s3m : (dj > 0 ? s3p : s3o)][lc + di]; };
            auto BY_ = [&](int di, int dj) -> T { return RBy[dj < 0 ? s3m : (dj > 0 ? s3p : s3o)][lc + di]; };
            jac_force<T>(A_, H_, BX_, BY_, 0, 0, g, Fx, Fy);
        }
        const T G1 = -vortU - (kc - kl) * rdx - a.grav * (Hh[2] - hl) * rdx + a.fcor * vhat + Fx;
        const T G2 = -vortV - (kc - km) * rdy - a.grav * (Hh[2] - Hh[1]) * rdy - a.fcor * uhat + Fy;
        const T Gh = -((RFh[0][lc + 1] - RFh[0][lc]) * rdx + (fhy_n - fhy) * rdy);
        const T GA = -((RFA[0][lc + 1] - RFA[0][lc]) * rdx + (fay_n - fay) * rdy)
                     + Aa[2] * ((ue - U[3]) * rdx + (V[3] - V[2]) * rdy);
        const unsigned o = col_ok ? rowb + colb : SW_OOB;
        const T Gs[4] = {G1, G2, Gh, GA};
        if constexpr (STORE_G) {
            const unsigned oG = a.drop_G ? SW_OOB : o;
#pragma unroll
            for (int f = 0; f < 4; ++f) buffer_store<T>(Gs[f], rG[f], oG);
        }
        if constexpr (FUSE) {
            const T Us[4] = {U[3], V[2], Hh[2], Aa[2]};
            const T Gms[4] = {gm0, gm1, gm2, gm3};
#pragma unroll
            for (int f = 0; f < 4; ++f) {
                T un;
                if constexpr (!HAS_GM) un = Us[f] + a.dtg * Gs[f];
                else if constexpr (STORE_G) un = fma_<T>(a.cg, Gms[f], fma_<T>(a.dtg, Gs[f], fma_<T>(a.cu, Us[f], Us[f])));
                else un = Us[f] + a.dt * (a.gamma * Gs[f] + a.zeta * Gms[f]);
                buffer_store<T>(un, rU[f], o);
            }
        }
        fhy = fhy_n; fay = fay_n; km = kc;
        constexpr int YOUNGER = ((FUSE && HAS_GM) ? 4 : 0) + (STORE_G ? 4 : 0) + (FUSE ? 4 : 0);
        wait_vmem_all_but<YOUNGER>();
    };
    auto shift1 = [&]() {
#pragma unroll
        for (int k = 0; k < 7; ++k) uw[k] = uw[k + 1];
#pragma unroll
        for (int k = 0; k < 6; ++k) { vw[k] = vw[k + 1]; hw[k] = hw[k + 1]; aw[k] = aw[k + 1]; }
#pragma unroll
        for (int k = 0; k < 5; ++k) { zw[k] = zw[k + 1]; svw[k] = svw[k + 1]; }
    };

    const int niter = (J1 - J0) + 6;
    const ProgressPriority prio(niter);
    int it = 6;
    for (; it < niter; ++it) {
        prio.at(it);
        body(it);
        shift1();
    }
}

constexpr int CONS_W3_MODES = (1 << 7) | (1 << 5) | (1 << 4);
constexpr int cons_minwaves(int mode, int elem_size) { return elem_size == 4 ? 3 : (((CONS_W3_MODES >> mode) & 1) ? 3 : 2); }
template <typename T, int LOR, int NT, int MODE>
__global__ __launch_bounds__(NT, cons_minwaves(MODE, (int)sizeof(T))) void k_tendency_cons_march(TendArgs<T> a, int nstrips, int nseg, int LY) {
    constexpr bool FUSE = (MODE & 1) != 0, HAS_GM = (MODE & 2) != 0, STORE_G = (MODE & 4) != 0;
    constexpr int XH = 3, RW = NT + 2 * XH, TXO = NT - 2 * XH;
    __shared__ T Ruh[3][RW];
    __shared__ T Rvh[3][RW];
    __shared__ T Rh[3][RW];
    __shared__ T RA[4][RW];
    __shared__ T RXu[1][RW];
    __shared__ T RXv[1][RW];
    __shared__ T RXa[1][RW];
    __shared__ T RUe[1][RW];
    __shared__ T RBx[1][LOR == 2 ? RW : 1];
    __shared__ T RHBx[LOR == 2 ? 2 : 1][LOR == 2 ? RW : 1];
    __shared__ T RBy[1][LOR == 2 ? RW : 1];
    __shared__ T RHBy[LOR == 2 ? 2 : 1][LOR == 2 ? RW : 1];
    __shared__ T RF1[LOR == 2 ? 1 : 1][LOR == 2 ? RW : 1];
    __shared__ T RG1[LOR == 2 ? 1 : 1][LOR == 2 ? RW : 1];

    const unsigned bid = xcd_remap(blockIdx.x, (unsigned)(nstrips * nseg));
    const int strip = (int)(bid % nstrips), seg = (int)(bid / nstrips);
    const int x0 = strip * TXO;
    int J0, J1;
    segment_rows(a, seg, LY, J0, J1);
    const int c = threadIdx.x, lc = c + XH;
    const int gx = x0 - XH + c;
    const bool wx = (a.wrap & 1) != 0, wy = (a.wrap & 2) != 0;
    const int gxc = wrap_index(gx, a.Nx, -a.Hx, a.Nx + a.Hx - 1, wx);
    const int ylo = -a.Hy, yhi = a.Ny + a.Hy - 1;
    const T rdx = a.rdx, rdy = a.rdy;
    const Geo<T> g{a.dx, a.dy, a.rdx, a.rdy};
    const bool col_ok = (c >= XH) && (c < NT - XH) && (gx < a.Nx);
    const T hg = T(0.5) * a.grav;

    T uw[6], vw[6], aw[6], hw[5];
#pragma unroll
    for (int k = 0; k < 6; ++k) { uw[k] = T(0); vw[k] = T(0); aw[k] = T(0); }
#pragma unroll
    for (int k = 0; k < 5; ++k) hw[k] = T(1);
    T bxw[5], byw[5], hbx_pub = T(0), hby_pub = T(0);
#pragma unroll
    for (int k = 0; k < 5; ++k) { bxw[k] = T(0); byw[k] = T(0); }
    T d1 = T(0), d2 = T(0), fya_s = T(0), hff_s = T(1), vs_ = T(0);

    const long off0 = (long)a.Hy * a.sy + a.Hx;
    const int isy = (int)a.sy;
    auto LD = [&](const T *interior, unsigned ob) -> T { return *reinterpret_cast<const T *>(reinterpret_cast<const char *>(interior - off0) + ob); };
    const unsigned colb = (unsigned)(gxc + a.Hx) * (unsigned)sizeof(T);
    auto rowoff = [&](int row) -> unsigned { return (unsigned)((row + a.Hy) * isy) * (unsigned)sizeof(T); };
    auto ldrow = [&](int row, T &nu, T &nv, T &nh, T &na) {
        const unsigned ob = rowoff(wrap_index(row, a.Ny, ylo, yhi, wy)) + colb;
        nu = LD(a.q1, ob); nv = LD(a.q2, ob); nh = LD(a.h, ob); na = LD(a.A, ob);
    };
    const unsigned pbytes = (unsigned)((a.Ny + 2 * a.Hy) * isy) * (unsigned)sizeof(T);
    __amdgpu_buffer_rsrc_t rG[4], rU[4];
    if constexpr (STORE_G) {
        rG[0] = out_rsrc(a.G1 - off0, pbytes); rG[1] = out_rsrc(a.G2 - off0, pbytes);
        rG[2] = out_rsrc(a.Gh - off0, pbytes); rG[3] = out_rsrc(a.GA - off0, pbytes);
    }
    if constexpr (FUSE) {
#pragma unroll
        for (int f = 0; f < 4; ++f) rU[f] = out_rsrc(a.Unew[f] - off0, pbytes);
    }
    auto insert_row = [&](T nu, T nv, T nh, T na) {
#pragma unroll
        for (int k = 0; k < 5; ++k) { uw[k] = uw[k + 1]; vw[k] = vw[k + 1]; aw[k] = aw[k + 1]; }
#pragma unroll
        for (int k = 0; k < 4; ++k) hw[k] = hw[k + 1];
        uw[5] = nu; vw[5] = nv; aw[5] = na; hw[4] = nh;
    };
    {
        const int jo = J0;
        auto colo = [&](int dxi) -> unsigned { return (unsigned)(wrap_index(gx + dxi, a.Nx, -a.Hx, a.Nx + a.Hx - 1, wx) + a.Hx) * (unsigned)sizeof(T); };
        const unsigned cm1 = colo(-1), cm2 = colo(-2), cp1 = colo(1);
        unsigned ro[7];
#pragma unroll
        for (int k = 0; k < 7; ++k) ro[k] = rowoff(wrap_index(J0 - 3 + k, a.Ny, ylo, yhi, wy));
        T pu[7], pv[7], ph[7], pa[7];
#pragma unroll
        for (int k = 0; k < 7; ++k) { pu[k] = LD(a.q1, ro[k] + colb); pv[k] = LD(a.q2, ro[k] + colb); ph[k] = LD(a.h, ro[k] + colb); pa[k] = LD(a.A, ro[k] + colb); }
        T Hm1[4], Am1[6], Ap1[5], Am2[2];
#pragma unroll
        for (int k = 0; k < 4; ++k) Hm1[k] = LD(a.h, ro[k + 1] + cm1);
        const T Vm2 = LD(a.q2, ro[3] + cm2), Vm1 = LD(a.q2, ro[3] + cm1), Vp1 = LD(a.q2, ro[3] + cp1);
        if constexpr (LOR == 2) {
#pragma unroll
            for (int k = 0; k < 6; ++k) Am1[k] = LD(a.A, ro[k] + cm1);
#pragma unroll
            for (int k = 0; k < 5; ++k) Ap1[k] = LD(a.A, ro[k] + cp1);
            Am2[0] = LD(a.A, ro[2] + cm2); Am2[1] = LD(a.A, ro[3] + cm2);
        }
#pragma unroll
        for (int k = 0; k < 6; ++k) { uw[k] = pu[k + 1]; vw[k] = pv[k + 1]; aw[k] = pa[k + 1]; }
#pragma unroll
        for (int k = 0; k < 5; ++k) hw[k] = ph[k + 2];
        T F2 = T(0), G2 = T(0);
        if constexpr (LOR == 2) {
            T m_[4], n_[4], bx_[4], by_[4];
#pragma unroll
            for (int t = 0; t < 4; ++t) {
                m_[t] = -(T(0.25) * rdy) * ((Am1[t + 2] - Am1[t]) + (pa[t + 2] - pa[t]));
                n_[t] = (T(0.25) * rdx) * ((Ap1[t] - Am1[t]) + (Ap1[t + 1] - Am1[t + 1]));
                bx_[t] = m_[t] * (T(2) * recip<T>(Hm1[t] + ph[t + 1]));
                by_[t] = n_[t] * (T(2) * recip<T>(ph[t] + ph[t + 1]));
            }
            bxw[1] = bx_[0]; bxw[2] = bx_[1]; bxw[3] = bx_[2]; bxw[4] = bx_[3];
            byw[1] = by_[0]; byw[2] = by_[1]; byw[3] = by_[2]; byw[4] = by_[3];
            hbx_pub = m_[2];
            hby_pub = n_[3];
            RHBx[(jo + 1) & 1][lc] = m_[1];
            RHBy[jo & 1][lc] = n_[2];
            const T hby_w = (T(0.25) * rdx) * ((pa[2] - Am2[0]) + (pa[3] - Am2[1]));
            F2 = g.dx * upwind_biased_product<T>(T(0.5) * (hby_w + n_[2]), left3<T>(bx_[0], bx_[1], bx_[2]), right3<T>(bx_[1], bx_[2], bx_[3]));
            G2 = g.dx * upwind_biased_product<T>(T(0.5) * (n_[1] + n_[2]), left3<T>(by_[0], by_[1], by_[2]), right3<T>(by_[1], by_[2], by_[3]));
        }
        const T hff0 = T(0.25) * ((Hm1[1] + ph[2]) + (Hm1[2] + ph[3]));
        const T vtf = g.dx * sym4<T>(Vm2, Vm1, pv[3], Vp1);
        const T hvu0 = upwind_weno<T>(vtf, pu) * recip<T>(hff0);
        const T rhyf = T(2) * recip<T>(ph[2] + ph[3]);
        fya_s = g.dx * upwind_weno<T>(pv[3], pa) * rhyf;
        vs_ = pv[3] * rhyf;
        const T vtc = g.dx * sym4<T>(pv[1], pv[2], pv[3], pv[4]);
        T hvv0;
        {
            const auto pos = vtc >= T(0);
            T q[5];
#pragma unroll
            for (int k = 0; k < 5; ++k) q[k] = pos ? pv[k] : pv[5 - k];
            hvv0 = vtc * weno5_upwind_ordered<T>(q, pos) * recip<T>(ph[2]);
        }
        d1 = F2 - hvu0; d2 = G2 - hvv0; hff_s = hff0;
        const int r3o = ((jo % 3) + 3) % 3, r3m = (r3o + 2) % 3, r3p = (r3o + 1) % 3;
        Ruh[r3m][lc] = uw[1];
        Rvh[r3o][lc] = vw[2];
        Rh[r3o][lc] = hw[1];
        Rh[r3p][lc] = hw[2];
        RA[jo & 3][lc] = aw[2]; RA[(jo + 1) & 3][lc] = aw[3]; RA[(jo + 2) & 3][lc] = aw[4];
    }

    auto body = [&](const int it, auto steady_tag) {
        constexpr bool STEADY = decltype(steady_tag)::value;
        const int jr = J0 - 3 + it, jo = jr - 3, jf = jr - 1;
        T nu, nv, nh, na;
        ldrow(jr + 1, nu, nv, nh, na);
        T gm0 = T(0), gm1 = T(0), gm2 = T(0), gm3 = T(0);
        const unsigned rowb = rowoff(jo);
        const int r3o = ((jo % 3) + 3) % 3, r3m = (r3o + 2) % 3, r3p = (r3o + 1) % 3;

        Ruh[r3o][lc] = uw[2];
        Rvh[r3p][lc] = vw[3];
        Rh[r3m][lc] = hw[3];
        RA[jr & 3][lc] = aw[5];
        if constexpr (LOR == 2) {
            RBx[0][lc] = bxw[3];
            RHBx[jo & 1][lc] = hbx_pub;
            RBy[0][lc] = byw[3];
            RHBy[(jo + 1) & 1][lc] = hby_pub;
        }
        __syncthreads();

        const T *su = Ruh[r3o], *sv0 = Rvh[r3o], *sv1 = Rvh[r3p], *sh0 = Rh[r3o], *sh1 = Rh[r3p], *sa0 = RA[jo & 3];
        const T hc = hw[1], hl = sh0[lc - 1];
        const T rhc = recip<T>(hc);
        const T rhxf = T(2) * recip<T>(hl + hc);
        {
            const T ut = g.dy * sym4<T>(su[lc - 1], su[lc], su[lc + 1], su[lc + 2]);
            {
                const bool pos = ut >= T(0);
                const int base = pos ? lc - 2 : lc + 3, st = pos ? 1 : -1;
                T q[5];
#pragma unroll
                for (int k = 0; k < 5; ++k) q[k] = su[base + st * k];
                RXu[0][lc] = ut * weno5_upwind_ordered<T>(q, pos) * rhc;
            }
            const T utf = g.dy * sym4<T>(uw[0], uw[1], uw[2], uw[3]);
            {
                const bool pos = utf >= T(0);
                const int base = pos ? lc - 3 : lc + 2, st = pos ? 1 : -1;
                T q[5];
#pragma unroll
                for (int k = 0; k < 5; ++k) q[k] = sv0[base + st * k];
                RXv[0][lc] = utf * weno5_upwind_ordered<T>(q, pos) * recip<T>(hff_s);
            }
            {
                const T uadv = uw[2];
                const bool pos = uadv >= T(0);
                const int base = pos ? lc - 3 : lc + 2, st = pos ? 1 : -1;
                T q[5];
#pragma unroll
                for (int k = 0; k < 5; ++k) q[k] = sa0[base + st * k];
                RXa[0][lc] = g.dy * uadv * weno5_upwind_ordered<T>(q, pos) * rhxf;
                RUe[0][lc] = uadv * rhxf;
            }
        }
        __builtin_amdgcn_sched_barrier(0);
        if constexpr (LOR == 2) {
            const T *bx0 = RBx[0], *hbx0 = RHBx[jo & 1], *hbxm = RHBx[(jo + 1) & 1], *by0 = RBy[0];
            RF1[0][lc] = g.dy * upwind_biased_product<T>(T(0.5) * (hbx0[lc] + hbx0[lc + 1]), left3<T>(bx0[lc - 1], bx0[lc], bx0[lc + 1]),
                                                         right3<T>(bx0[lc], bx0[lc + 1], bx0[lc + 2]));
            RG1[0][lc] = g.dy * upwind_biased_product<T>(T(0.5) * (hbxm[lc] + hbx0[lc]), left3<T>(by0[lc - 2], by0[lc - 1], by0[lc]),
                                                         right3<T>(by0[lc - 1], by0[lc], by0[lc + 1]));
            __builtin_amdgcn_sched_barrier(0);
            const T *am = RA[(jf - 1) & 3], *a0 = RA[jf & 3], *ap = RA[(jf + 1) & 3], *shf = Rh[r3m];
            const T m = -(T(0.25) * rdy) * ((ap[lc - 1] - am[lc - 1]) + (aw[5] - aw[3]));
            const T n = (T(0.25) * rdx) * ((am[lc + 1] - am[lc - 1]) + (a0[lc + 1] - a0[lc - 1]));
            const T bx = m * (T(2) * recip<T>(shf[lc - 1] + hw[3]));
            const T by = n * (T(2) * recip<T>(hw[2] + hw[3]));
#pragma unroll
            for (int k = 0; k < 4; ++k) { bxw[k] = bxw[k + 1]; byw[k] = byw[k + 1]; }
            bxw[4] = bx; byw[4] = by;
            hby_pub = n;
            hbx_pub = bxw[3] * (T(0.5) * (sh1[lc - 1] + hw[2]));
        }
        __syncthreads();
        if constexpr (STEADY && FUSE && HAS_GM) {
            const unsigned og = rowb + colb;
            gm0 = LD(a.Gm[0], og); gm1 = LD(a.Gm[1], og); gm2 = LD(a.Gm[2], og); gm3 = LD(a.Gm[3], og);
        }

        if (!STEADY && it < 5) {
            hff_s = T(0.25) * ((sh1[lc - 1] + hw[2]) + (hl + hc));
        } else {
        const T hn1 = hw[2];
        const T hff_n = T(0.25) * ((hl + hc) + (sh1[lc - 1] + hn1));
        const T rhyf_n = T(2) * recip<T>(hc + hn1);
        const T vtf = g.dx * sym4<T>(sv1[lc - 2], sv1[lc - 1], vw[3], sv1[lc + 1]);
        const T hvu_n = upwind_weno<T>(vtf, uw) * recip<T>(hff_n);
        const T fya_n = g.dx * upwind_weno<T>(vw[3], aw) * rhyf_n;
        const T vn = vw[3] * rhyf_n;
        const T vtc = g.dx * sym4<T>(vw[1], vw[2], vw[3], vw[4]);
        T hvv_c;
        {
            const bool pos = vtc >= T(0);
            T q[5];
#pragma unroll
            for (int k = 0; k < 5; ++k) q[k] = pos ? vw[k] : vw[5 - k];
            hvv_c = vtc * weno5_upwind_ordered<T>(q, pos) * rhc;
        }
        T f2n = T(0), g2n = T(0);
        if constexpr (LOR == 2) {
            const T *hby1 = RHBy[(jo + 1) & 1];
            const T hby_o = RHBy[jo & 1][lc], hby_n = hby1[lc];
            f2n = g.dx * upwind_biased_product<T>(T(0.5) * (hby1[lc - 1] + hby_n), left3<T>(bxw[1], bxw[2], bxw[3]), right3<T>(bxw[2], bxw[3], bxw[4]));
            g2n = g.dx * upwind_biased_product<T>(T(0.5) * (hby_o + hby_n), left3<T>(byw[1], byw[2], byw[3]), right3<T>(byw[2], byw[3], byw[4]));
        }
        const T d1n = f2n - hvu_n, d2n = g2n - hvv_c;
        if constexpr (STEADY) {
            const T rAz = rdx * rdy;
            T xu = -(RXu[0][lc] - RXu[0][lc - 1]), xv = -(RXv[0][lc + 1] - RXv[0][lc]);
            if constexpr (LOR == 2) {
                xu += RF1[0][lc] - RF1[0][lc - 1];
                xv += RG1[0][lc + 1] - RG1[0][lc];
            }
            const T vbar = T(0.25) * ((sv0[lc - 1] + vw[2]) + (sv1[lc - 1] + vw[3]));
            const T G1 = rAz * (xu + (d1n - d1)) - (hg * sq(hc) - hg * sq(hl)) * rdx + a.fcor * vbar;
            const T ubar = T(0.25) * ((uw[1] + Ruh[r3m][lc + 1]) + (uw[2] + su[lc + 1]));
            const T G2 = rAz * (xv + (d2n - d2)) - (hg * sq(hc) - hg * sq(hw[0])) * rdy - a.fcor * ubar;
            const T ue_t = su[lc + 1];
            const T Gh = -((ue_t - uw[2]) * rdx + (vw[3] - vw[2]) * rdy);
            const T GA = -rAz * ((RXa[0][lc + 1] - RXa[0][lc]) + (fya_n - fya_s))
                         + aw[2] * ((RUe[0][lc + 1] - RUe[0][lc]) * rdx + (vn - vs_) * rdy);
            const unsigned o = col_ok ? rowb + colb : SW_OOB;
            const T Gs[4] = {G1, G2, Gh, GA};
            if constexpr (STORE_G) {
                const unsigned oG = a.drop_G ? SW_OOB : o;
#pragma unroll
                for (int f = 0; f < 4; ++f) buffer_store<T>(Gs[f], rG[f], oG);
            }
            if constexpr (FUSE) {
                const T Us[4] = {uw[2], vw[2], hc, aw[2]};
                const T Gms[4] = {gm0, gm1, gm2, gm3};
#pragma unroll
                for (int f = 0; f < 4; ++f) {
                    T un;
                    if constexpr (!HAS_GM) un = Us[f] + a.dtg * Gs[f];
                    else if constexpr (STORE_G) un = fma_<T>(a.cg, Gms[f], fma_<T>(a.dtg, Gs[f], fma_<T>(a.cu, Us[f], Us[f])));
                else un = Us[f] + a.dt * (a.gamma * Gs[f] + a.zeta * Gms[f]);
                    buffer_store<T>(un, rU[f], o);
                }
            }
        }
        d1 = d1n; d2 = d2n; fya_s = fya_n; hff_s = hff_n; vs_ = vn;
        }
        constexpr int YOUNGER = STEADY ? ((FUSE && HAS_GM) ? 4 : 0) + (STORE_G ? 4 : 0) + (FUSE ? 4 : 0) : 0;
        wait_vmem_all_but<YOUNGER>();
        insert_row(nu, nv, nh, na);
    };

    const int niter = (J1 - J0) + 6;
    const ProgressPriority prio(niter);
    for (int it = 6; it < niter; ++it) {
        prio.at(it);
        body(it, std::true_type{});
    }
}
```

### swmhd_amd/csrc/tendency_pk_kernels.inc

```


template <int LOR, int NT, int MODE>
__global__ __launch_bounds__(NT, 3) void k_tendency_vi_march_pk(TendArgs<float> a, int nstrips, int nseg, int LY) {
    using T = sw_f2;
    using S = float;
    constexpr bool FUSE = (MODE & 1) != 0, HAS_GM = (MODE & 2) != 0, STORE_G = (MODE & 4) != 0;
    constexpr int XL = 2, PAD = 4, RW = 2 * NT + 2 * PAD, TXO = 2 * (NT - 2 * XL);
    __shared__ __attribute__((aligned(8))) S Ru[3][RW];
    __shared__ __attribute__((aligned(8))) S Rvn[1][RW];
    __shared__ __attribute__((aligned(8))) S RA[4][RW];
    __shared__ __attribute__((aligned(8))) S RH[2][RW];
    __shared__ __attribute__((aligned(8))) S RBx[3][RW];
    __shared__ __attribute__((aligned(8))) S RBy[3][RW];
    __shared__ __attribute__((aligned(8))) S RFh[1][RW];
    __shared__ __attribute__((aligned(8))) S RFA[1][RW];
    __shared__ __attribute__((aligned(8))) S RK[1][RW];
    __shared__ __attribute__((aligned(8))) S RZ[1][RW];
    __shared__ __attribute__((aligned(8))) S RUf[1][RW];
    __shared__ __attribute__((aligned(8))) S RVf[1][RW];

    const unsigned bid = xcd_remap(blockIdx.x, (unsigned)(nstrips * nseg));
    const int strip = (int)(bid % nstrips), seg = (int)(bid / nstrips);
    const int x0 = strip * TXO;
    int J0, J1;
    segment_rows(a, seg, LY, J0, J1);
    const int lane = threadIdx.x, lc = 2 * lane + PAD;
    const int gx0 = x0 - 2 * XL + 2 * lane;
    const bool wy = (a.wrap & 2) != 0;
    const int xlo = -a.Hx, xhi = a.Nx + a.Hx - 1, ylo = -a.Hy, yhi = a.Ny + a.Hy - 1;
    auto wrapx = [&](int x) -> int { return wrap_index(x, a.Nx, xlo, xhi, true); };
    const T rdx = T(a.rdx), rdy = T(a.rdy);
    const Geo<T> g{T(a.dx), T(a.dy), T(a.rdx), T(a.rdy)};
    const bool col_ok = (lane >= XL) && (lane < NT - XL) && (gx0 < a.Nx);

    auto P = [&](const S *row, int k) -> T { T v; v.x = row[lc + k]; v.y = row[lc + k + 1]; return v; };
    auto W = [&](S *row, T v) { *reinterpret_cast<T *>(row + lc) = v; };

    T uw[8], vw[7], vlw[7], hw[7], aw[7];
    T fhy = T(0), fay = T(0), km = T(0);

    const long off0 = (long)a.Hy * a.sy + a.Hx;
    const int isy = (int)a.sy;
    auto LD = [&](const S *interior, unsigned ob) -> T { return *reinterpret_cast<const sw_f2_u *>(reinterpret_cast<const char *>(interior - off0) + ob); };
    auto LD1 = [&](const S *interior, unsigned ob) -> S { return *reinterpret_cast<const S *>(reinterpret_cast<const char *>(interior - off0) + ob); };
    const int gxw = wrap_index(gx0, a.Nx, xlo, xhi - 1, true);
    const unsigned colb = (unsigned)(gxw + a.Hx) * (unsigned)sizeof(S);
    auto rowoff = [&](int row) -> unsigned { return (unsigned)((row + a.Hy) * isy) * (unsigned)sizeof(S); };
    const unsigned pbytes = (unsigned)((a.Ny + 2 * a.Hy) * isy) * (unsigned)sizeof(S);
    __amdgpu_buffer_rsrc_t rG[4], rU[4];
    if constexpr (STORE_G) {
        rG[0] = out_rsrc(a.G1 - off0, pbytes); rG[1] = out_rsrc(a.G2 - off0, pbytes);
        rG[2] = out_rsrc(a.Gh - off0, pbytes); rG[3] = out_rsrc(a.GA - off0, pbytes);
    }
    if constexpr (FUSE) {
#pragma unroll
        for (int f = 0; f < 4; ++f) rU[f] = out_rsrc(a.Unew[f] - off0, pbytes);
    }

    {
        const unsigned colm = (unsigned)(wrapx(gx0 - 1) + a.Hx) * (unsigned)sizeof(S);
        const unsigned colp = (unsigned)(wrapx(gx0 + 2) + a.Hx) * (unsigned)sizeof(S);
        unsigned ro[7];
#pragma unroll
        for (int k = 0; k < 7; ++k) ro[k] = rowoff(wrap_index(J0 - 3 + k, a.Ny, ylo, yhi, wy));
        T pu[7], pv[7], ph[7], pa[7];
        S pvl[6];
#pragma unroll
        for (int k = 0; k < 7; ++k) { pu[k] = LD(a.q1, ro[k] + colb); pv[k] = LD(a.q2, ro[k] + colb); ph[k] = LD(a.h, ro[k] + colb); pa[k] = LD(a.A, ro[k] + colb); }
#pragma unroll
        for (int k = 0; k < 6; ++k) pvl[k] = LD1(a.q2, ro[k + 1] + colm);
        const S ue_r = LD1(a.q1, ro[2] + colp);
        S a_wm = 0, a_em = 0, a_wo = 0, a_eo = 0;
        if constexpr (LOR == 1) {
            a_wm = LD1(a.A, ro[2] + colm); a_em = LD1(a.A, ro[2] + colp);
            a_wo = LD1(a.A, ro[3] + colm); a_eo = LD1(a.A, ro[3] + colp);
        }
#pragma unroll
        for (int k = 0; k < 7; ++k) uw[k] = pu[k];
#pragma unroll
        for (int k = 0; k < 6; ++k) { vw[k] = pv[k + 1]; vlw[k] = T{pvl[k], pv[k + 1].x}; hw[k] = ph[k + 1]; aw[k] = pa[k + 1]; }
        uw[7] = T(0); vw[6] = T(0); vlw[6] = T(0); hw[6] = T(1); aw[6] = T(0);
        fhy = upwind_weno<T>(vw[2], ph);
        fay = upwind_weno<T>(vw[2], pa);
        const T ue_m = T{uw[2].y, ue_r};
        km = T(0.25) * ((sq(uw[2]) + sq(ue_m)) + (sq(vw[1]) + sq(vw[2])));
        const int q3o = ((J0 % 3) + 3) % 3, q3m = (q3o + 2) % 3;
        W(Ru[q3m], uw[2]);
        W(RA[(J0 - 1) & 3], aw[1]);
        W(RA[J0 & 3], aw[2]);
        if constexpr (LOR == 1) {
            const T rhm = recip<T>(hw[1]), rho = recip<T>(hw[2]);
            const T cxm = T{aw[1].y - a_wm, a_em - aw[1].x}, cxo = T{aw[2].y - a_wo, a_eo - aw[2].x};
            W(RBy[q3m], (T(0.5) * rdx) * cxm * rhm);
            W(RBx[q3m], -(T(0.5) * rdy) * (aw[2] - aw[0]) * rhm);
            W(RBy[q3o], (T(0.5) * rdx) * cxo * rho);
            W(RBx[q3o], -(T(0.5) * rdy) * (aw[3] - aw[1]) * rho);
        }
    }

    const int niter = (J1 - J0) + 6;
    const ProgressPriority prio(niter);
    for (int it = 6; it < niter; ++it) {
        prio.at(it);
        T *const U = uw, *const V = vw, *const VL = vlw, *const Hh = hw, *const Aa = aw;
        const int jr = J0 - 3 + it, jo = jr - 3;
        {
            const unsigned ob = rowoff(wrap_index(jr + 1, a.Ny, ylo, yhi, wy)) + colb;
            uw[7] = LD(a.q1, ob); vw[6] = LD(a.q2, ob); hw[6] = LD(a.h, ob); aw[6] = LD(a.A, ob);
        }
        T gm0 = T(0), gm1 = T(0), gm2 = T(0), gm3 = T(0);
        const unsigned rowb = rowoff(jo);
        const int s3o = ((jo % 3) + 3) % 3, s3m = (s3o + 2) % 3, s3p = (s3o + 1) % 3;
        const int s4o = jo & 3, s4p = (jo + 1) & 3;

        W(Ru[s3o], U[3]);
        W(RH[jo & 1], Hh[2]);
        W(RA[s4p], Aa[3]);
        W(Rvn[0], V[5]);
        __syncthreads();

        VL[5] = P(Rvn[0], -1);
        if constexpr (LOR == 1) {
            const T cxA = P(RA[s4p], 1) - P(RA[s4p], -1);
            const T cyA = Aa[4] - Aa[2];
            const T rh = recip<T>(Hh[3]);
            W(RBy[s3p], (T(0.5) * rdx) * cxA * rh);
            W(RBx[s3p], -(T(0.5) * rdy) * cyA * rh);
        }
        {
            const T ue2 = P(Ru[s3o], 1);
            W(RK[0], T(0.25) * ((sq(U[3]) + sq(ue2)) + (sq(V[2]) + sq(V[3]))));
        }
        W(RZ[0], (V[2] - VL[2]) * rdx - (U[3] - U[2]) * rdy);
        W(RUf[0], T(0.5) * (U[2] + U[3]));
        W(RVf[0], T(0.5) * (VL[2] + V[2]));
        {
            const T uadv = U[3];
            T qh[6], qa[6];
#pragma unroll
            for (int k = 0; k < 6; ++k) { qh[k] = P(RH[jo & 1], k - 3); qa[k] = P(RA[s4o], k - 3); }
            W(RFh[0], upwind_weno<T>(uadv, qh));
            W(RFA[0], upwind_weno<T>(uadv, qa));
        }
        __syncthreads();
        if constexpr (FUSE && HAS_GM) {
            const unsigned og = rowb + colb;
            gm0 = LD(a.Gm[0], og); gm1 = LD(a.Gm[1], og); gm2 = LD(a.Gm[2], og); gm3 = LD(a.Gm[3], og);
        }

        const T fhy_n = upwind_weno<T>(V[3], Hh);
        const T fay_n = upwind_weno<T>(V[3], Aa);
        T zy[6], svy[6];
#pragma unroll
        for (int k = 0; k < 6; ++k) {
            zy[k] = (V[k] - VL[k]) * rdx - (U[k + 1] - U[k]) * rdy;
            svy[k] = VL[k] + V[k];
        }
        const T vhat = T(0.25) * (svy[2] + svy[3]);
        const T vortU = -upwind_weno_vel_raw<T>(vhat, zy, U, svy);
        const T ue = P(Ru[s3o], 1);
        const T uhat = T(0.25) * ((U[2] + P(Ru[s3m], 1)) + (U[3] + ue));
        T vortV;
        {
            T zx[6], ufx[6], vfx[6];
#pragma unroll
            for (int k = 0; k < 6; ++k) { zx[k] = P(RZ[0], k - 2); ufx[k] = P(RUf[0], k - 2); vfx[k] = P(RVf[0], k - 2); }
            vortV = upwind_weno_vel<T>(uhat, zx, ufx, vfx);
        }
        const T kc = P(RK[0], 0), kl = P(RK[0], -1);
        const T hl = P(RH[jo & 1], -1);
        T Fx = T(0), Fy = T(0);
        if constexpr (LOR == 1) {
            auto A_ = [&](int di, int dj) -> T { return di == 0 ? Aa[2 + dj] : P(RA[(jo + dj) & 3], di); };
            auto H_ = [&](int di, int dj) -> T { return di == 0 ? Hh[2 + dj] : hl; };
            auto BX_ = [&](int di, int dj) -> T { return P(RBx[dj < 0 ? s3m : (dj > 0 ? s3p : s3o)], di); };
            auto BY_ = [&](int di, int dj) -> T { return P(RBy[dj < 0 ? s3m : (dj > 0 ? s3p : s3o)], di); };
            jac_force<T>(A_, H_, BX_, BY_, 0, 0, g, Fx, Fy);
        }
        const T G1 = -vortU - (kc - kl) * rdx - T(a.grav) * (Hh[2] - hl) * rdx + T(a.fcor) * vhat + Fx;
        const T G2 = -vortV - (kc - km) * rdy - T(a.grav) * (Hh[2] - Hh[1]) * rdy - T(a.fcor) * uhat + Fy;
        const T Gh = -((P(RFh[0], 1) - P(RFh[0], 0)) * rdx + (fhy_n - fhy) * rdy);
        const T GA = -((P(RFA[0], 1) - P(RFA[0], 0)) * rdx + (fay_n - fay) * rdy)
                     + Aa[2] * ((ue - U[3]) * rdx + (V[3] - V[2]) * rdy);
        const unsigned o = col_ok ? rowb + colb : SW_OOB;
        const T Gs[4] = {G1, G2, Gh, GA};
        if constexpr (STORE_G) {
#pragma unroll
            for (int f = 0; f < 4; ++f) buffer_store<T>(Gs[f], rG[f], o);
        }
        if constexpr (FUSE) {
            const T Us[4] = {U[3], V[2], Hh[2], Aa[2]};
            const T Gms[4] = {gm0, gm1, gm2, gm3};
#pragma unroll
            for (int f = 0; f < 4; ++f) {
                T un;
                if constexpr (!HAS_GM) un = Us[f] + T(a.dtg) * Gs[f];
                else if constexpr (STORE_G) un = fma_<T>(T(a.cg), Gms[f], fma_<T>(T(a.dtg), Gs[f], fma_<T>(T(a.cu), Us[f], Us[f])));
                else un = Us[f] + T(a.dt) * (T(a.gamma) * Gs[f] + T(a.zeta) * Gms[f]);
                buffer_store<T>(un, rU[f], o);
            }
        }
        fhy = fhy_n; fay = fay_n; km = kc;
        constexpr int YOUNGER = ((FUSE && HAS_GM) ? 4 : 0) + (STORE_G ? 4 : 0) + (FUSE ? 4 : 0);
        wait_vmem_all_but<YOUNGER>();
#pragma unroll
        for (int k = 0; k < 7; ++k) uw[k] = uw[k + 1];
#pragma unroll
        for (int k = 0; k < 6; ++k) { vw[k] = vw[k + 1]; vlw[k] = vlw[k + 1]; hw[k] = hw[k + 1]; aw[k] = aw[k + 1]; }
    }
}
```

### swmhd_amd/csrc/tendency_tile_kernels.inc

```

#ifndef SWMHD_STRICT
#error "include with SWMHD_STRICT defined"
#endif

namespace swmhd {
namespace {

constexpr bool STRICT = (SWMHD_STRICT != 0);

#include <type_traits>
#include "tile_common.inc"
#include "lorentz_device.inc"
#include "sw_device.inc"

template <typename T, int FORM, int LOR, int TX, int TYB, int RY, bool BND = false>
__global__ __launch_bounds__(TX *TYB) void k_tendency_tile(TendArgs<T> a, int ntx, int nty) {
    constexpr int TY = TYB * RY, NT = TX * TYB;
    constexpr int W = TX + 6, HH = TY + 6;
    __shared__ T s1[HH][W];
    __shared__ T s2[HH][W];
    __shared__ T sh[HH][W];
    __shared__ T sA[HH][W];
    constexpr int LW = LOR == 1 ? TX + 2 : (LOR == 2 ? TX + 4 : 1), LH = LOR == 1 ? TY + 2 : (LOR == 2 ? TY + 4 : 1);
    constexpr int LO = LOR == 1 ? 1 : 2;
    __shared__ T sL0[LH][LW];
    __shared__ T sL1[LH][LW];
    __shared__ T sL2[LOR == 2 ? LH : 1][LOR == 2 ? LW : 1];
    __shared__ T sL3[LOR == 2 ? LH : 1][LOR == 2 ? LW : 1];

    const unsigned bid = xcd_remap(blockIdx.x, (unsigned)(ntx * nty));
    const int tyi = (int)(bid / ntx), ntya = (a.j1 - a.j0 + TY - 1) / TY;
    const bool second = tyi >= ntya;
    int txi = (int)(bid % ntx);
    if (a.edge_cols && txi > 0) txi = (a.Nx + TX - 1) / TX - (ntx - txi);
    const int x0 = txi * TX, y0 = second ? a.j0b + (tyi - ntya) * TY : a.j0 + tyi * TY, jend = second ? a.j1b : a.j1;
    const int tid = threadIdx.y * TX + threadIdx.x;
    const int xlo = -a.Hx, xhi = a.Nx + a.Hx - 1, ylo = -a.Hy, yhi = a.Ny + a.Hy - 1;
    const Geo<T> g{a.dx, a.dy, a.rdx, a.rdy};

    load_tile<T, W, HH, NT>(s1, a.q1, a.sy, x0 - 3, y0 - 3, xlo, xhi, ylo, yhi, tid, a.Nx, a.Ny, a.wrap);
    load_tile<T, W, HH, NT>(s2, a.q2, a.sy, x0 - 3, y0 - 3, xlo, xhi, ylo, yhi, tid, a.Nx, a.Ny, a.wrap);
    load_tile<T, W, HH, NT>(sh, a.h, a.sy, x0 - 3, y0 - 3, xlo, xhi, ylo, yhi, tid, a.Nx, a.Ny, a.wrap);
    load_tile<T, W, HH, NT>(sA, a.A, a.sy, x0 - 3, y0 - 3, xlo, xhi, ylo, yhi, tid, a.Nx, a.Ny, a.wrap);
    __syncthreads();

    auto U_ = [&](int ii, int jj) -> T { return s1[jj + 3][ii + 3]; };
    auto V_ = [&](int ii, int jj) -> T { return s2[jj + 3][ii + 3]; };
    auto H_ = [&](int ii, int jj) -> T { return sh[jj + 3][ii + 3]; };
    auto A_ = [&](int ii, int jj) -> T { return sA[jj + 3][ii + 3]; };
    auto L0_ = [&](int ii, int jj) -> T { return sL0[jj + LO][ii + LO]; };
    auto L1_ = [&](int ii, int jj) -> T { return sL1[jj + LO][ii + LO]; };
    auto L2_ = [&](int ii, int jj) -> T { return sL2[jj + LO][ii + LO]; };
    auto L3_ = [&](int ii, int jj) -> T { return sL3[jj + LO][ii + LO]; };

    if constexpr (LOR == 1) {
        for (int e = tid; e < LW * LH; e += NT) {
            int r = e / LW, c = e - r * LW;
            T bx, by;
            jac_centre_B<T>(A_, H_, c - 1, r - 1, g, bx, by);
            sL0[r][c] = bx; sL1[r][c] = by;
        }
        __syncthreads();
    } else if constexpr (LOR == 2) {
        for (int e = tid; e < LW * LH; e += NT) {
            int r = e / LW, c = e - r * LW;
            T hbx, bx, hby, by;
            div_faces<T>(A_, H_, c - 2, r - 2, g, hbx, bx, hby, by);
            sL0[r][c] = hbx; sL1[r][c] = bx; sL2[r][c] = hby; sL3[r][c] = by;
        }
        __syncthreads();
    }

    auto gx6 = [&](auto &F, int f, int jj, T *q) {
#pragma unroll
        for (int m = 0; m < 6; ++m) q[m] = F(f - 3 + m, jj);
    };
    auto gy6 = [&](auto &F, int ii, int f, T *q) {
#pragma unroll
        for (int m = 0; m < 6; ++m) q[m] = F(ii, f - 3 + m);
    };
    const bool bx = BND && a.topo_x == 1, by = BND && a.topo_y == 1;
    auto oLx = [&](int ii) -> int { return BND ? left_order(bx, x0 + ii + 1, a.Nx) : 5; };
    auto oRx = [&](int ii) -> int { return BND ? right_order(bx, x0 + ii + 1, a.Nx) : 5; };
    auto oLy = [&](int jj) -> int { return BND ? left_order(by, y0 + jj + 1, a.Ny) : 5; };
    auto oRy = [&](int jj) -> int { return BND ? right_order(by, y0 + jj + 1, a.Ny) : 5; };
    auto s4x = [&](int ii) -> bool { return BND ? sym_fourth(bx, x0 + ii + 1, a.Nx) : true; };
    auto s4y = [&](int jj) -> bool { return BND ? sym_fourth(by, y0 + jj + 1, a.Ny) : true; };
    auto tflux_x = [&](auto &Uf, auto &C, int ii, int jj) -> T { T q[6]; gx6(C, ii, jj, q); return g.dy * upwind_recon<T>(Uf(ii, jj), q, oLx(ii), oRx(ii)); };
    auto tflux_y = [&](auto &Vf, auto &C, int ii, int jj) -> T { T q[6]; gy6(C, ii, jj, q); return g.dx * upwind_recon<T>(Vf(ii, jj), q, oLy(jj), oRy(jj)); };
    auto div_centered = [&](auto &Q1, auto &Q2, int ii, int jj) -> T {
        if constexpr (STRICT) return T(1) / (g.dx * g.dy) * ((g.dy * Q1(ii + 1, jj) - g.dy * Q1(ii, jj)) + (g.dx * Q2(ii, jj + 1) - g.dx * Q2(ii, jj)));
        else return (Q1(ii + 1, jj) - Q1(ii, jj)) * g.rdx + (Q2(ii, jj + 1) - Q2(ii, jj)) * g.rdy;
    };
    auto avg4 = [&](T p, T q, T r, T s) -> T {
        if constexpr (STRICT) return ((p + q) / T(2) + (r + s) / T(2)) / T(2);
        else return T(0.25) * ((p + q) + (r + s));
    };
    const T rAz = STRICT ? T(0) : g.rdx * g.rdy;

    const int i = threadIdx.x, gxi = x0 + i;
#pragma unroll 1
    for (int r = 0; r < RY; ++r) {
        const int j = threadIdx.y * RY + r, gyj = y0 + j;
        T G1, G2, Gh, GA;
        if constexpr (FORM == 1) {
            auto zeta = [&](int ii, int jj) -> T {
                if constexpr (STRICT) return ((g.dy * V_(ii, jj) - g.dy * V_(ii - 1, jj)) - (g.dx * U_(ii, jj) - g.dx * U_(ii, jj - 1))) / (g.dx * g.dy);
                else return (V_(ii, jj) - V_(ii - 1, jj)) * g.rdx - (U_(ii, jj) - U_(ii, jj - 1)) * g.rdy;
            };
            auto u_ff = [&](int ii, int jj) -> T { return half_sum<T>(U_(ii, jj - 1), U_(ii, jj)); };
            auto v_ff = [&](int ii, int jj) -> T { return half_sum<T>(V_(ii - 1, jj), V_(ii, jj)); };
            auto Kh = [&](int ii, int jj) -> T {
                if constexpr (STRICT) return ((sq(U_(ii, jj)) + sq(U_(ii + 1, jj))) / T(2) + (sq(V_(ii, jj)) + sq(V_(ii, jj + 1))) / T(2)) / T(2);
                else return T(0.25) * ((sq(U_(ii, jj)) + sq(U_(ii + 1, jj))) + (sq(V_(ii, jj)) + sq(V_(ii, jj + 1))));
            };
            T z[6], us[6], vs[6];
            T vhat;
            if constexpr (STRICT) vhat = (((g.dx * V_(i - 1, j) + g.dx * V_(i - 1, j + 1)) / T(2) + (g.dx * V_(i, j) + g.dx * V_(i, j + 1)) / T(2)) / T(2)) / g.dx;
            else vhat = T(0.25) * ((V_(i - 1, j) + V_(i - 1, j + 1)) + (V_(i, j) + V_(i, j + 1)));
#pragma unroll
            for (int m = 0; m < 6; ++m) { int jj = j - 2 + m; z[m] = zeta(i, jj); us[m] = u_ff(i, jj); vs[m] = v_ff(i, jj); }
            T vortU = -upwind_recon_vel<T>(vhat, z, us, vs, oLy(j), oRy(j));
            T uhat;
            if constexpr (STRICT) uhat = (((g.dy * U_(i, j - 1) + g.dy * U_(i + 1, j - 1)) / T(2) + (g.dy * U_(i, j) + g.dy * U_(i + 1, j)) / T(2)) / T(2)) / g.dy;
            else uhat = T(0.25) * ((U_(i, j - 1) + U_(i + 1, j - 1)) + (U_(i, j) + U_(i + 1, j)));
#pragma unroll
            for (int m = 0; m < 6; ++m) { int ii = i - 2 + m; z[m] = zeta(ii, j); us[m] = u_ff(ii, j); vs[m] = v_ff(ii, j); }
            T vortV = upwind_recon_vel<T>(uhat, z, us, vs, oLx(i), oRx(i));
            T k00 = Kh(i, j);
            T Fx = T(0), Fy = T(0);
            if constexpr (LOR == 1) jac_force<T>(A_, H_, L0_, L1_, i, j, g, Fx, Fy);
            if constexpr (STRICT) {
                T bern_u = (k00 - Kh(i - 1, j)) / g.dx;
                T div_u = vortU + bern_u;
                T pgx = a.grav * ((H_(i, j) - H_(i - 1, j)) / g.dx);
                T xfU = -a.fcor * avg4(V_(i - 1, j), V_(i, j), V_(i - 1, j + 1), V_(i, j + 1));
                G1 = -div_u - pgx - xfU + Fx;
                T bern_v = (k00 - Kh(i, j - 1)) / g.dy;
                T div_v = vortV + bern_v;
                T pgy = a.grav * ((H_(i, j) - H_(i, j - 1)) / g.dy);
                T yfU = a.fcor * avg4(U_(i, j - 1), U_(i + 1, j - 1), U_(i, j), U_(i + 1, j));
                G2 = -div_v - pgy - yfU + Fy;
                T Az = g.dx * g.dy;
                Gh = -(T(1) / Az * ((tflux_x(U_, H_, i + 1, j) - tflux_x(U_, H_, i, j)) + (tflux_y(V_, H_, i, j + 1) - tflux_y(V_, H_, i, j))));
                T div_Uc = T(1) / Az * ((tflux_x(U_, A_, i + 1, j) - tflux_x(U_, A_, i, j)) + (tflux_y(V_, A_, i, j + 1) - tflux_y(V_, A_, i, j)));
                GA = -div_Uc + A_(i, j) * div_centered(U_, V_, i, j);
            } else {
                G1 = -vortU - (k00 - Kh(i - 1, j)) * g.rdx - a.grav * (H_(i, j) - H_(i - 1, j)) * g.rdx
                     + a.fcor * avg4(V_(i - 1, j), V_(i, j), V_(i - 1, j + 1), V_(i, j + 1)) + Fx;
                G2 = -vortV - (k00 - Kh(i, j - 1)) * g.rdy - a.grav * (H_(i, j) - H_(i, j - 1)) * g.rdy
                     - a.fcor * avg4(U_(i, j - 1), U_(i + 1, j - 1), U_(i, j), U_(i + 1, j)) + Fy;
                Gh = -rAz * ((tflux_x(U_, H_, i + 1, j) - tflux_x(U_, H_, i, j)) + (tflux_y(V_, H_, i, j + 1) - tflux_y(V_, H_, i, j)));
                GA = -rAz * ((tflux_x(U_, A_, i + 1, j) - tflux_x(U_, A_, i, j)) + (tflux_y(V_, A_, i, j + 1) - tflux_y(V_, A_, i, j)))
                     + A_(i, j) * div_centered(U_, V_, i, j);
            }
        } else {
            auto dv = [&](T x, T y) -> T { if constexpr (STRICT) return x / y; else return x * recip<T>(y); };
            auto h_ff = [&](int ii, int jj) -> T { return avg4(H_(ii - 1, jj - 1), H_(ii, jj - 1), H_(ii - 1, jj), H_(ii, jj)); };
            auto flux_huu = [&](int ii, int jj) -> T {
                T q[6]; gx6(U_, ii + 1, jj, q);
                T ut = symc<T>(s4x(ii), g.dy * U_(ii - 1, jj), g.dy * U_(ii, jj), g.dy * U_(ii + 1, jj), g.dy * U_(ii + 2, jj));
                return dv(upwind_recon<T>(ut, q, oLx(ii), oRx(ii)), H_(ii, jj));
            };
            auto flux_hvu = [&](int ii, int jj) -> T {
                T q[6]; gy6(U_, ii, jj, q);
                T vt = symc<T>(s4x(ii), g.dx * V_(ii - 2, jj), g.dx * V_(ii - 1, jj), g.dx * V_(ii, jj), g.dx * V_(ii + 1, jj));
                return dv(upwind_recon<T>(vt, q, oLy(jj), oRy(jj)), h_ff(ii, jj));
            };
            auto flux_huv = [&](int ii, int jj) -> T {
                T q[6]; gx6(V_, ii, jj, q);
                T ut = symc<T>(s4y(jj), g.dy * U_(ii, jj - 2), g.dy * U_(ii, jj - 1), g.dy * U_(ii, jj), g.dy * U_(ii, jj + 1));
                return dv(upwind_recon<T>(ut, q, oLx(ii), oRx(ii)), h_ff(ii, jj));
            };
            auto flux_hvv = [&](int ii, int jj) -> T {
                T q[6]; gy6(V_, ii, jj + 1, q);
                T vt = symc<T>(s4y(jj), g.dx * V_(ii, jj - 1), g.dx * V_(ii, jj), g.dx * V_(ii, jj + 1), g.dx * V_(ii, jj + 2));
                return dv(upwind_recon<T>(vt, q, oLy(jj), oRy(jj)), H_(ii, jj));
            };
            T Fx = T(0), Fy = T(0);
            if constexpr (LOR == 2) {
                const T rAzs = T(1) / (g.dx * g.dy);
                const int iJ = gxi + 1, jJ = gyj + 1;
                const int cF1 = BND ? wall_code(bx, iJ, 0, a.Nx) : 0, cF1m = BND ? wall_code(bx, iJ - 1, 0, a.Nx) : 0;
                const int cG1 = BND ? wall_code(bx, iJ, 1, a.Nx + 1) : 0, cG1p = BND ? wall_code(bx, iJ + 1, 1, a.Nx + 1) : 0;
                const int cF2 = BND ? wall_code(by, jJ, 1, a.Ny + 1) : 0, cF2p = BND ? wall_code(by, jJ + 1, 1, a.Ny + 1) : 0;
                const int cG2 = BND ? wall_code(by, jJ, 0, a.Ny) : 0, cG2m = BND ? wall_code(by, jJ - 1, 0, a.Ny) : 0;
                Fx = rAzs * ((div_F1<T>(L0_, L1_, i, j, g, cF1) - div_F1<T>(L0_, L1_, i - 1, j, g, cF1m)) + (div_F2<T>(L2_, L1_, i, j + 1, g, cF2p) - div_F2<T>(L2_, L1_, i, j, g, cF2)));
                Fy = rAzs * ((div_G1<T>(L0_, L3_, i + 1, j, g, cG1p) - div_G1<T>(L0_, L3_, i, j, g, cG1)) + (div_G2<T>(L2_, L3_, i, j, g, cG2) - div_G2<T>(L2_, L3_, i, j - 1, g, cG2m)));
            }
            const T Vol = g.dx * g.dy;
            const T hg = T(0.5) * a.grav;
            T div_u = T(1) / Vol * ((flux_huu(i, j) - flux_huu(i - 1, j)) + (flux_hvu(i, j + 1) - flux_hvu(i, j)));
            T pgx = STRICT ? (hg * sq(H_(i, j)) - hg * sq(H_(i - 1, j))) / g.dx : (hg * sq(H_(i, j)) - hg * sq(H_(i - 1, j))) * g.rdx;
            T xfU = -a.fcor * avg4(V_(i - 1, j), V_(i, j), V_(i - 1, j + 1), V_(i, j + 1));
            G1 = -div_u - pgx - xfU + Fx;
            T div_v = T(1) / Vol * ((flux_huv(i + 1, j) - flux_huv(i, j)) + (flux_hvv(i, j) - flux_hvv(i, j - 1)));
            T pgy = STRICT ? (hg * sq(H_(i, j)) - hg * sq(H_(i, j - 1))) / g.dy : (hg * sq(H_(i, j)) - hg * sq(H_(i, j - 1))) * g.rdy;
            T yfU = a.fcor * avg4(U_(i, j - 1), U_(i + 1, j - 1), U_(i, j), U_(i + 1, j));
            G2 = -div_v - pgy - yfU + Fy;
            T dUh;
            if constexpr (STRICT) dUh = T(1) / Vol * ((g.dy * U_(i + 1, j) - g.dy * U_(i, j)) + (g.dx * V_(i, j + 1) - g.dx * V_(i, j)));
            else dUh = (U_(i + 1, j) - U_(i, j)) * g.rdx + (V_(i, j + 1) - V_(i, j)) * g.rdy;
            Gh = -dUh;
            T he = half_sum<T>(H_(i, j), H_(i + 1, j)), hw = half_sum<T>(H_(i - 1, j), H_(i, j));
            T hn = half_sum<T>(H_(i, j), H_(i, j + 1)), hs = half_sum<T>(H_(i, j - 1), H_(i, j));
            T fxe = dv(tflux_x(U_, A_, i + 1, j), he), fxw = dv(tflux_x(U_, A_, i, j), hw);
            T fyn = dv(tflux_y(V_, A_, i, j + 1), hn), fys = dv(tflux_y(V_, A_, i, j), hs);
            T div_Uc = T(1) / Vol * ((fxe - fxw) + (fyn - fys));
            T ue = dv(U_(i + 1, j), he), uw = dv(U_(i, j), hw), vn = dv(V_(i, j + 1), hn), vs_ = dv(V_(i, j), hs);
            T c_div_U = A_(i, j) * (T(1) / Vol * ((g.dy * ue - g.dy * uw) + (g.dx * vn - g.dx * vs_)));
            GA = -div_Uc + c_div_U;
        }
        if (gxi < a.Nx && gyj < jend) {
            const long o = (long)gyj * a.sy + gxi;
            if (a.store_G) { a.G1[o] = G1; a.G2[o] = G2; a.Gh[o] = Gh; a.GA[o] = GA; }
            if (a.fuse) {
                const T Gs[4] = {G1, G2, Gh, GA};
                const T Us[4] = {U_(i, j), V_(i, j), H_(i, j), A_(i, j)};
#pragma unroll
                for (int f = 0; f < 4; ++f) {
                    T un;
                    if (a.first) {
                        if constexpr (STRICT) un = Us[f] + a.dt * a.gamma * Gs[f];
                        else un = Us[f] + (a.dt * a.gamma) * Gs[f];
                    } else if (!STRICT && a.gm_prev) {
                        un = Us[f] + (a.dt * a.gamma) * Gs[f] + a.zeta * (Us[f] - a.Gm[f][o]);
                    } else {
                        un = Us[f] + a.dt * (a.gamma * Gs[f] + a.zeta * a.Gm[f][o]);
                    }
                    a.Unew[f][o] = un;
                }
            }
        }
    }
}

template <typename T>
__global__ void k_rk3_substep(Rk3Args<T> a) {
    const int x = blockIdx.x * blockDim.x + threadIdx.x;
    const int y = a.j0 + blockIdx.y;
    if (x >= a.Nx || y >= a.j1) return;
    const long o = (long)y * a.sy + x;
#pragma unroll
    for (int f = 0; f < 4; ++f) {
        T u = a.U[f][o];
        if (a.first) {
            if constexpr (STRICT) u += a.dt * a.gamma * a.Gn[f][o];
            else u += (a.dt * a.gamma) * a.Gn[f][o];
        } else {
            u += a.dt * (a.gamma * a.Gn[f][o] + a.zeta * a.Gm[f][o]);
        }
        a.U[f][o] = u;
    }
}

#if !SWMHD_STRICT
#include "tendency_march_kernels.inc"
#include "tendency_pk_kernels.inc"
#endif

}

#define LAUNCH_NAME_(base, sfx) base##sfx
#define LAUNCH_NAME(base, sfx) LAUNCH_NAME_(base, sfx)

constexpr long SW_MARCH_MIN_CELLS = 330000L;

#if !SWMHD_STRICT
static bool tendency_uses_packed_fp32(int Nx, int formulation, int wrap) {
    return formulation == 1 && (wrap & 1) && (Nx % 2 == 0) && Nx >= 8;
}
static MarchGeometry packed_fp32_geometry(int Nx, int rows, int leave_room) {
    static int ly_cache = 0;
    MarchGeometry g{};
    g.nt = 256; g.wg_per_cu = 3; g.nstrips = (Nx + 503) / 504;
    int slots = device_cu_count() * g.wg_per_cu;
    if (leave_room) slots -= (slots * leave_room_64ths(rows)) / 64;
    int LY = 32;
    for (int k = 1; k <= 64; ++k) {
        const int ns = (slots * k) / g.nstrips;
        if (ns < 1) continue;
        const int ly = (rows + ns - 1) / ns;
        if (ly <= 128) { LY = ly < 6 ? 6 : ly; break; }
    }
    if (const int f = env_knob("SWMHD_T_LY", ly_cache)) LY = f;
    g.LY = LY; g.nseg = (rows + LY - 1) / LY;
    return g;
}
static MarchGeometry tendency_march_geometry(int Nx, int rows, int formulation, int leave_room, int elem_size, int mode = 7) {
    static int ly_cache = 0, nt_cache = 0;
    const int force_ly = env_knob("SWMHD_T_LY", ly_cache), force_nt = env_knob("SWMHD_T_NT", nt_cache);
    if (formulation == 1) {
        static const int nts[2] = {256, 128}, wgs64[2] = {3, 6}, wgs32[2] = {4, 8};
        return march_geometry(Nx, rows, 3, nts, elem_size == 8 ? wgs64 : wgs32, 2, 6, leave_room != 0, force_nt, force_ly);
    }
    const int w = cons_minwaves(mode, elem_size);
    const int nts[2] = {256, 128}, wgs[2] = {w, 2 * w};
    return march_geometry(Nx, rows, 3, nts, wgs, 2, 6, leave_room != 0, force_nt, force_ly);
}
#endif

template <typename T>
hipError_t LAUNCH_NAME(launch_tendency_, LAUNCH_SFX)(const TendArgs<T> &a, int formulation, int lorentz, hipStream_t s) {
    constexpr int TX = 64, TYB = 4, RY = 2;
    const bool two = a.j1b > a.j0b;
    const int rows_b = two ? a.j1b - a.j0b : 0;
    [[maybe_unused]] const int rows = a.j1 - a.j0 + rows_b;
    auto one_by_one = [&]() {
        TendArgs<T> b = a;
        b.j0b = b.j1b = 0;
        hipError_t e = LAUNCH_NAME(launch_tendency_, LAUNCH_SFX)<T>(b, formulation, lorentz, s);
        if (e != hipSuccess) return e;
        b.j0 = a.j0b; b.j1 = a.j1b;
        return LAUNCH_NAME(launch_tendency_, LAUNCH_SFX)<T>(b, formulation, lorentz, s);
    };
    if (two && a.j1 <= a.j0) return one_by_one();
    int ntx = (a.Nx + TX - 1) / TX, nty = (a.j1 - a.j0 + TYB * RY - 1) / (TYB * RY) + (rows_b + TYB * RY - 1) / (TYB * RY);
    if (ntx <= 0 || nty <= 0) return hipSuccess;
    if (a.edge_cols) {
        const int ne = (a.Nx % TX == 0 || a.Nx % TX >= 8) ? 2 : 3;
        ntx = ntx < ne ? ntx : ne;
    }
#if !SWMHD_STRICT
    const bool fits32 = (long)(a.Ny + 2 * a.Hy) * a.sy * (long)sizeof(T) < (1L << 32) - 64;
    const bool bnd = a.topo_x == 1 || a.topo_y == 1;
    const bool march = !bnd && fits32 && (a.kernel_variant == 2 || (a.kernel_variant == 0 && (long)a.Nx * rows >= SW_MARCH_MIN_CELLS));
    if (bnd && !two && !a.edge_cols && fits32 && a.kernel_variant == 0 && (long)a.Nx * rows >= SW_MARCH_MIN_CELLS && a.Nx >= 4 * TX &&
        a.Ny >= 48) {
        constexpr int FW = 8;
        TendArgs<T> p = a;
        p.topo_x = p.topo_y = 0;
        hipError_t e = LAUNCH_NAME(launch_tendency_, LAUNCH_SFX)<T>(p, formulation, lorentz, s);
        if (e != hipSuccess) return e;
        TendArgs<T> f = a;
        f.kernel_variant = 1;
        if (a.topo_y == 1) {
            const int a0 = a.j0, a1 = a.j1 < FW ? a.j1 : FW, b0 = a.j0 > a.Ny - FW ? a.j0 : a.Ny - FW, b1 = a.j1;
            f.j0 = a0; f.j1 = a1 > a0 ? a1 : a0; f.j0b = b0; f.j1b = b1 > b0 ? b1 : b0;
            if (f.j1 > f.j0 || f.j1b > f.j0b) {
                e = LAUNCH_NAME(launch_tendency_, LAUNCH_SFX)<T>(f, formulation, lorentz, s);
                if (e != hipSuccess) return e;
            }
        }
        if (a.topo_x == 1) {
            f.j0 = a.j0; f.j1 = a.j1; f.j0b = f.j1b = 0; f.edge_cols = 1;
            e = LAUNCH_NAME(launch_tendency_, LAUNCH_SFX)<T>(f, formulation, lorentz, s);
            if (e != hipSuccess) return e;
        }
        return hipSuccess;
    }
    auto two_range_segments = [&](int LY) { return (a.j1 - a.j0 + LY - 1) / LY + (rows_b + LY - 1) / LY; };
    if constexpr (std::is_same<T, float>::value) {
        if (march && tendency_uses_packed_fp32(a.Nx, formulation, a.wrap)) {
            const MarchGeometry mg = packed_fp32_geometry(a.Nx, rows, a.leave_room);
            const int nstrips = mg.nstrips, LY = mg.LY, nseg = two ? two_range_segments(LY) : mg.nseg;
            dim3 mgrid(nstrips * nseg), mblock(256);
            int mode = (a.fuse ? 1 : 0) | ((a.fuse && !a.first) ? 2 : 0) | ((a.store_G || !a.fuse) ? 4 : 0);
            TendArgs<T> ap = a;
            if (a.gm_prev && mode == 3) { mode = 7; ap.drop_G = 1; }
#define SW_PK_MARCH(MODE_)                                                                                                  \
            case MODE_:                                                                                                         \
                if (lorentz == 1) hipLaunchKernelGGL((k_tendency_vi_march_pk<1, 256, MODE_>), mgrid, mblock, 0, s, ap, nstrips, nseg, LY); \
                else hipLaunchKernelGGL((k_tendency_vi_march_pk<0, 256, MODE_>), mgrid, mblock, 0, s, ap, nstrips, nseg, LY);            \
                break;
            switch (mode) { SW_PK_MARCH(4) SW_PK_MARCH(5) SW_PK_MARCH(1) SW_PK_MARCH(7) SW_PK_MARCH(3) default: return hipErrorInvalidValue; }
#undef SW_PK_MARCH
            return hipGetLastError();
        }
    }
    if (march) {
        int mode = (a.fuse ? 1 : 0) | ((a.fuse && !a.first) ? 2 : 0) | ((a.store_G || !a.fuse) ? 4 : 0);
        TendArgs<T> ax = a;
        if (formulation == 0 && mode == 3 && sizeof(T) == 8 && cons_minwaves(7, 8) > cons_minwaves(3, 8)) {
            mode = 7; ax.drop_G = 1;
        }
        if (a.gm_prev && mode == 3) { mode = 7; ax.drop_G = 1; }
        if (formulation == 0 && mode == 1 && sizeof(T) == 8 && cons_minwaves(5, 8) > cons_minwaves(1, 8)) {
            mode = 5; ax.drop_G = 1;
        }
        const MarchGeometry mg = tendency_march_geometry(a.Nx, rows, formulation, a.leave_room, (int)sizeof(T), mode);
        const int nstrips = mg.nstrips, LY = mg.LY, nseg = two ? two_range_segments(LY) : mg.nseg;
        dim3 mgrid(nstrips * nseg), mblock(mg.nt);
        if (formulation == 1) {
#define SW_VI_GO(NT_, MODE_)                                                                                                \
            do {                                                                                                                \
                if (lorentz == 1) hipLaunchKernelGGL((k_tendency_vi_march<T, 1, NT_, MODE_>), mgrid, mblock, 0, s, ax, nstrips, nseg, LY); \
                else hipLaunchKernelGGL((k_tendency_vi_march<T, 0, NT_, MODE_>), mgrid, mblock, 0, s, ax, nstrips, nseg, LY);            \
            } while (0)
#define SW_VI_MARCH(MODE_)                                                                                                  \
            case MODE_:                                                                                                         \
                if (mg.nt == 128) SW_VI_GO(128, MODE_);                                                                         \
                else SW_VI_GO(256, MODE_);                                                                                      \
                break;
            switch (mode) { SW_VI_MARCH(4) SW_VI_MARCH(5) SW_VI_MARCH(1) SW_VI_MARCH(7) SW_VI_MARCH(3) default: return hipErrorInvalidValue; }
#undef SW_VI_MARCH
#undef SW_VI_GO
        } else {
#define SW_CONS_MARCH(MODE_)                                                                                                \
            case MODE_:                                                                                                         \
                if (mg.nt == 128) {                                                                                             \
                    if (lorentz == 2) hipLaunchKernelGGL((k_tendency_cons_march<T, 2, 128, MODE_>), mgrid, mblock, 0, s, ax, nstrips, nseg, LY); \
                    else hipLaunchKernelGGL((k_tendency_cons_march<T, 0, 128, MODE_>), mgrid, mblock, 0, s, ax, nstrips, nseg, LY);            \
                } else {                                                                                                        \
                    if (lorentz == 2) hipLaunchKernelGGL((k_tendency_cons_march<T, 2, 256, MODE_>), mgrid, mblock, 0, s, ax, nstrips, nseg, LY); \
                    else hipLaunchKernelGGL((k_tendency_cons_march<T, 0, 256, MODE_>), mgrid, mblock, 0, s, ax, nstrips, nseg, LY);            \
                }                                                                                                               \
                break;
            switch (mode) { SW_CONS_MARCH(4) SW_CONS_MARCH(5) SW_CONS_MARCH(1) SW_CONS_MARCH(7) SW_CONS_MARCH(3) default: return hipErrorInvalidValue; }
#undef SW_CONS_MARCH
        }
        return hipGetLastError();
    }
#endif
#if !SWMHD_STRICT
    if (!(a.topo_x == 1 || a.topo_y == 1) && (long)a.Nx * rows < SW_MARCH_MIN_CELLS) {
        constexpr int RY1 = 1;
        const int nty1 = (a.j1 - a.j0 + TYB * RY1 - 1) / (TYB * RY1) + (rows_b + TYB * RY1 - 1) / (TYB * RY1);
        dim3 grid1(ntx * nty1), block1(TX, TYB);
        if (formulation == 1 && lorentz == 1) hipLaunchKernelGGL((k_tendency_tile<T, 1, 1, TX, TYB, RY1>), grid1, block1, 0, s, a, ntx, nty1);
        else if (formulation == 1 && lorentz == 0) hipLaunchKernelGGL((k_tendency_tile<T, 1, 0, TX, TYB, RY1>), grid1, block1, 0, s, a, ntx, nty1);
        else if (formulation == 0 && lorentz == 2) hipLaunchKernelGGL((k_tendency_tile<T, 0, 2, TX, TYB, RY1>), grid1, block1, 0, s, a, ntx, nty1);
        else if (formulation == 0 && lorentz == 0) hipLaunchKernelGGL((k_tendency_tile<T, 0, 0, TX, TYB, RY1>), grid1, block1, 0, s, a, ntx, nty1);
        else return hipErrorInvalidValue;
        return hipGetLastError();
    }
#endif
    dim3 grid(ntx * nty), block(TX, TYB);
    if (a.topo_x == 1 || a.topo_y == 1) {
        if (formulation == 1 && lorentz == 1) hipLaunchKernelGGL((k_tendency_tile<T, 1, 1, TX, TYB, RY, true>), grid, block, 0, s, a, ntx, nty);
        else if (formulation == 1 && lorentz == 0) hipLaunchKernelGGL((k_tendency_tile<T, 1, 0, TX, TYB, RY, true>), grid, block, 0, s, a, ntx, nty);
        else if (formulation == 0 && lorentz == 2) hipLaunchKernelGGL((k_tendency_tile<T, 0, 2, TX, TYB, RY, true>), grid, block, 0, s, a, ntx, nty);
        else if (formulation == 0 && lorentz == 0) hipLaunchKernelGGL((k_tendency_tile<T, 0, 0, TX, TYB, RY, true>), grid, block, 0, s, a, ntx, nty);
        else return hipErrorInvalidValue;
        return hipGetLastError();
    }
    if (formulation == 1 && lorentz == 1) hipLaunchKernelGGL((k_tendency_tile<T, 1, 1, TX, TYB, RY>), grid, block, 0, s, a, ntx, nty);
    else if (formulation == 1 && lorentz == 0) hipLaunchKernelGGL((k_tendency_tile<T, 1, 0, TX, TYB, RY>), grid, block, 0, s, a, ntx, nty);
    else if (formulation == 0 && lorentz == 2) hipLaunchKernelGGL((k_tendency_tile<T, 0, 2, TX, TYB, RY>), grid, block, 0, s, a, ntx, nty);
    else if (formulation == 0 && lorentz == 0) hipLaunchKernelGGL((k_tendency_tile<T, 0, 0, TX, TYB, RY>), grid, block, 0, s, a, ntx, nty);
    else return hipErrorInvalidValue;
    return hipGetLastError();
}

template <typename T>
hipError_t LAUNCH_NAME(launch_rk3_substep_, LAUNCH_SFX)(const Rk3Args<T> &a, hipStream_t s) {
    if (a.j1 <= a.j0) return hipSuccess;
    hipLaunchKernelGGL((k_rk3_substep<T>), dim3((a.Nx + 255) / 256, a.j1 - a.j0), dim3(256), 0, s, a);
    return hipGetLastError();
}

#if !SWMHD_STRICT
int tendency_launch_geometry(int Nx, int rows, int formulation, int elem_size, int kernel_variant, int leave_room, int wrap, int out[8]) {
    const bool march = (kernel_variant == 2 || (kernel_variant == 0 && (long)Nx * rows >= SW_MARCH_MIN_CELLS));
    if (march && elem_size == 4 && tendency_uses_packed_fp32(Nx, formulation, wrap)) {
        const MarchGeometry mg = packed_fp32_geometry(Nx, rows, leave_room);
        out[0] = 3; out[1] = mg.nt; out[2] = mg.nstrips; out[3] = mg.nseg; out[4] = mg.LY; out[5] = mg.wg_per_cu; out[6] = 2;
    } else if (march) {
        const MarchGeometry mg = tendency_march_geometry(Nx, rows, formulation, leave_room, elem_size);
        out[0] = 2; out[1] = mg.nt; out[2] = mg.nstrips; out[3] = mg.nseg; out[4] = mg.LY; out[5] = mg.wg_per_cu; out[6] = 3;
    } else {
        const int ry = (kernel_variant == 1 || (long)Nx * rows >= SW_MARCH_MIN_CELLS) ? 2 : 1;
        out[0] = 1; out[1] = 256; out[2] = (Nx + 63) / 64; out[3] = (rows + 4 * ry - 1) / (4 * ry); out[4] = 4 * ry; out[5] = 0; out[6] = 3;
    }
    out[7] = device_cu_count();
    return 0;
}
#endif

template hipError_t LAUNCH_NAME(launch_tendency_, LAUNCH_SFX)<double>(const TendArgs<double> &, int, int, hipStream_t);
template hipError_t LAUNCH_NAME(launch_tendency_, LAUNCH_SFX)<float>(const TendArgs<float> &, int, int, hipStream_t);
template hipError_t LAUNCH_NAME(launch_rk3_substep_, LAUNCH_SFX)<double>(const Rk3Args<double> &, hipStream_t);
template hipError_t LAUNCH_NAME(launch_rk3_substep_, LAUNCH_SFX)<float>(const Rk3Args<float> &, hipStream_t);

}
```

### swmhd_amd/model.py

```python
import torch

from . import _lib
from .distributed import SlabDecomposition, agree_rc, exchange_y_halos
from .fields import Field, _SFX, _stream_ptr
from .grid import Center, Face

VectorInvariantFormulation, ConservativeFormulation = "VectorInvariant", "Conservative"
RK3_GAMMA = (8.0 / 15.0, 5.0 / 12.0, 3.0 / 4.0)
RK3_ZETA = (0.0, -17.0 / 60.0, -5.0 / 12.0)


def rk3_stage(stage, from_state):
    fs = from_state and stage == 1
    store = 1 if stage == 1 or (stage == 0 and not from_state) else 0
    return RK3_GAMMA[stage], RK3_ZETA[1] / RK3_GAMMA[0] if fs else RK3_ZETA[stage], store, fs


def loopback_rings(nranks, timeout_s=60.0):
    import ctypes
    arr = (ctypes.c_void_p * nranks)()
    _lib.check(_lib.lib().swmhd_ring_create_loopback(arr, nranks, float(timeout_s)), "swmhd_ring_create_loopback")
    return [ctypes.c_void_p(arr[k]) for k in range(nranks)]


class ShallowWaterModel:
    def __init__(self, grid, gravitational_acceleration=9.81, coriolis_f=1.0, formulation=VectorInvariantFormulation,
                 lorentz_forcing=True, dtype=torch.float64, device="cuda", strict=False, decomp=None, group=None,
                 overlap=True, fused=True, kernel="auto", fuse_halo=True, native_ring=True, boundary_conditions=None, ring=None):
        self.grid, self.g, self.f = grid, float(gravitational_acceleration), float(coriolis_f)
        self.formulation = formulation
        self.form_code = _lib.VECTOR_INVARIANT if formulation == VectorInvariantFormulation else _lib.CONSERVATIVE
        if not lorentz_forcing:
            self.lorentz_code = _lib.LORENTZ_NONE
        else:
            self.lorentz_code = _lib.LORENTZ_JACOBIAN if self.form_code == _lib.VECTOR_INVARIANT else _lib.LORENTZ_DIVERGENCE
        self.strict = strict
        self._flags = (_lib.STRICT if strict else _lib.FAST) | _lib.KERNEL_FLAGS[kernel]
        tx, ty = grid.topo_codes()
        self._bounded = (tx == _lib.BOUNDED, ty == _lib.BOUNDED)
        self._flags |= (_lib.BOUNDED_X if self._bounded[0] else 0) | (_lib.BOUNDED_Y if self._bounded[1] else 0)
        self.decomp = decomp or SlabDecomposition(grid.Ny_global, 1, 0)
        if any(self._bounded) and self.decomp.ring:
            raise _lib.SwmhdError("y-slab decomposition (ring halo exchange) supports (Periodic, Periodic) grids only (SWMHD_ENOTSUP)")
        self.boundary_conditions = dict(boundary_conditions or {})
        for name, bc in self.boundary_conditions.items():
            sides = [(bc.west, 0), (bc.east, 0), (bc.south, 1), (bc.north, 1)]
            if any(b is not None and not self._bounded[d] for b, d in sides):
                raise _lib.SwmhdError(f"boundary condition on a Periodic side of {name} (Oceananigans rejects it as well)")
        self.group, self.overlap = group, overlap
        n1, n2 = ("u", "v") if self.form_code == _lib.VECTOR_INVARIANT else ("uh", "vh")
        self.names = (n1, n2, "h", "A")
        locs = ((Face, Center), (Center, Face), (Center, Center), (Center, Center))
        mk = lambda loc: Field(grid, loc, dtype, device)
        self._state = {n: mk(l) for n, l in zip(self.names, locs)}
        self.fused = fused
        self._rwrap = 0
        if fuse_halo and grid.Nx >= grid.Hx and grid.Ny >= grid.Hy:
            self._rwrap = (0 if self._bounded[0] else _lib.WRAP_X) | (0 if (self.decomp.ring or self._bounded[1]) else _lib.WRAP_Y)
        self._halo_stale = False
        self._exchange_in_flight = False
        self._alt = {n: mk(l) for n, l in zip(self.names, locs)} if fused else None
        self.Gn = [mk(l) for l in locs]
        self.Gm = [mk(l) for l in locs]
        self.sfx = _SFX[dtype]
        self.clock_time, self.iteration = 0.0, 0
        self._comm_stream = torch.cuda.Stream() if (self.decomp.ring and torch.cuda.is_available()) else None
        self._L = _lib.lib()
        self.tendency_events = None
        if any(not f.data.is_cuda for f in self._state.values()):
            raise _lib.SwmhdError("ShallowWaterModel runs on the GPU only (no CPU fallback)")
        self._ring = None
        if ring is not None:
            if not (self.decomp.ring and fused and grid.Ny > 2 * grid.Hy):
                raise _lib.SwmhdError("ring= needs a ring decomposition, the fused stage kernel and a slab taller than its two strips")
            self._ring, self._comm_stream = ring, None
        elif self.decomp.ring and native_ring and fused and grid.Ny > 2 * grid.Hy:
            self._ring = self._create_ring()

    def _create_ring(self):
        import ctypes, os
        import torch.distributed as dist
        if not (dist.is_available() and dist.is_initialized() and dist.get_backend(self.group) == "nccl"):
            return None
        dev = self._raw_fields[0].data.device
        rccl = os.path.join(os.path.dirname(torch.__file__), "lib", "librccl.so")
        rccl = rccl.encode() if os.path.exists(rccl) else None
        rc = self._L.swmhd_ring_available(rccl)
        ok = torch.tensor([1 if rc == 0 else 0], dtype=torch.int32, device=dev)
        dist.all_reduce(ok, op=dist.ReduceOp.MIN, group=self.group)
        if int(ok.item()) == 0:
            if rc != 0:
                import sys
                print(f"swmhd_amd: native ring unavailable ({self._L.swmhd_strerror(rc).decode()}); using torch.distributed p2p",
                      file=sys.stderr)
            return None
        ident = torch.zeros(_lib.RING_ID_BYTES, dtype=torch.uint8)
        if self.decomp.rank == 0:
            buf = (ctypes.c_ubyte * _lib.RING_ID_BYTES)()
            _lib.check(self._L.swmhd_ring_unique_id(rccl, buf), "swmhd_ring_unique_id")
            ident = torch.tensor(list(buf), dtype=torch.uint8)
        ident = ident.to(dev)
        src = dist.get_global_rank(self.group, 0) if self.group is not None else 0
        dist.broadcast(ident, src=src, group=self.group)
        raw = bytes(ident.cpu().tolist())
        ring = ctypes.c_void_p()
        with torch.cuda.device(dev):
            rc = self._L.swmhd_ring_create(ctypes.byref(ring), rccl, self.decomp.world_size, self.decomp.rank,
                                           (ctypes.c_ubyte * _lib.RING_ID_BYTES).from_buffer_copy(raw))
        worst = agree_rc(rc, self.group, dev)
        if worst != 0:
            if rc == 0:
                self._L.swmhd_ring_destroy(ring)
                raise _lib.SwmhdError(f"swmhd_ring_create failed on another rank (rc {worst}); this rank destroyed its communicator")
            _lib.check(rc, "swmhd_ring_create")
        self._comm_stream = None
        return ring

    def _ring_check(self, rc, what):
        if rc == 4:
            raise _lib.SwmhdError(f"{what}: {self._L.swmhd_ring_last_error(self._ring).decode()}")
        _lib.check(rc, what)

    def ring_time_launches(self, n):
        self._ring_check(self._L.swmhd_ring_time_launches(self._ring, n), "swmhd_ring_time_launches")

    def ring_launch_times(self, capacity=4096):
        import ctypes
        ms, rows = (ctypes.c_float * capacity)(), (ctypes.c_int * capacity)()
        n = self._L.swmhd_ring_launch_times(self._ring, ms, rows, capacity)
        return [(ms[k], rows[k]) for k in range(max(n, 0))]

    def _join(self):
        if self._ring is not None:
            self._ring_check(self._L.swmhd_ring_join(self._ring, _stream_ptr()), "swmhd_ring_join")
        if self._comm_stream is not None:
            torch.cuda.current_stream().wait_stream(self._comm_stream)
        self._exchange_in_flight = False

    def close(self):
        ring, self._ring = getattr(self, "_ring", None), None
        if ring is not None:
            self._L.swmhd_ring_destroy(ring)

    def __del__(self):
        try:
            self.close()
        except Exception:
            pass

    def set(self, **kw):
        self._join()
        for k, v in kw.items():
            self._state[k].set(v)
        self.update_state()
        return self

    @property
    def solution(self):
        self._ensure_halos()
        return self._state

    @property
    def fields(self):
        self._ensure_halos()
        return [self._state[n] for n in self.names]

    @property
    def _raw_fields(self):
        return [self._state[n] for n in self.names]

    def _ensure_halos(self):
        if self._halo_stale:
            self.update_state()

    def _fill_bc(self, stream=None):
        import ctypes
        g = self.grid
        q = self._raw_fields
        ct = ctypes.c_double if self.sfx == "f64" else ctypes.c_float
        grads = []
        for n in self.names:
            bc = self.boundary_conditions.get(n)
            grads += bc.gradients() if bc is not None else [float("nan")] * 4
        f = getattr(self._L, f"swmhd_fill_halo_{self.sfx}")
        tx, ty = g.topo_codes()
        rc = f(_lib.ptr_array([x.ptr for x in q]), 4, g.Nx, g.Ny, g.Hx, g.Hy, q[0].stride_y, tx, ty, 0b0001, 0b0010,
               (ct * 16)(*grads), g.dx, g.dy, _stream_ptr(stream))
        _lib.check(rc, "swmhd_fill_halo")

    def _fill_x(self, stream=None):
        if any(self._bounded):
            return self._fill_bc(stream)
        g = self.grid
        q = self._raw_fields
        ptrs = _lib.ptr_array([f.ptr for f in q])
        which = _lib.HALO_X | (0 if self.decomp.ring else _lib.HALO_Y)
        f = getattr(self._L, f"swmhd_fill_halo_periodic_multi_{self.sfx}")
        _lib.check(f(ptrs, 4, g.Nx, g.Ny, g.Hx, g.Hy, q[0].stride_y, which, _stream_ptr(stream)), "fill_halo_multi")

    def update_state(self):
        self._join()
        self._halo_stale = False
        self._fill_x()
        q = self._raw_fields
        if self._ring is not None:
            g = self.grid
            f = getattr(self._L, f"swmhd_ring_exchange_y_{self.sfx}")
            rc = f(self._ring, _lib.ptr_array([x.ptr for x in q]), 4, g.Nx, g.Ny, g.Hx, g.Hy, q[0].stride_y, _stream_ptr())
            self._ring_check(rc, "swmhd_ring_exchange_y")
        elif self.decomp.ring:
            exchange_y_halos([f.data for f in q], self.grid.Ny, self.grid.Hy, self.decomp, self.group)

    def calculate_tendencies(self, rows=None, stream=None):
        if self.tendency_events is not None and rows is None:
            e0, e1 = _lib.TimingEvent(), _lib.TimingEvent()
            e0.record()
            self._calculate_tendencies(rows, stream)
            e1.record()
            self.tendency_events.append((e0, e1, self.grid.Ny))
        else:
            self._calculate_tendencies(rows, stream)

    def _calculate_tendencies(self, rows=None, stream=None):
        g = self.grid
        q = self._raw_fields
        j0, j1 = (0, g.Ny) if rows is None else rows
        f = getattr(self._L, f"swmhd_tendencies_{self.sfx}")
        rc = f(q[0].ptr, q[1].ptr, q[2].ptr, q[3].ptr, self.Gn[0].ptr, self.Gn[1].ptr, self.Gn[2].ptr, self.Gn[3].ptr,
               g.Nx, g.Ny, g.Hx, g.Hy, q[0].stride_y, g.dx, g.dy, self.g, self.f, self.form_code, self.lorentz_code,
               j0, j1, self._flags | self._rwrap, _stream_ptr(stream))
        _lib.check(rc, "swmhd_tendencies")

    def _substep(self, dt, stage):
        g = self.grid
        U = _lib.ptr_array([f.ptr for f in self._raw_fields])
        Gn = _lib.ptr_array([f.ptr for f in self.Gn])
        Gm = _lib.ptr_array([f.ptr for f in self.Gm]) if stage > 0 else None
        f = getattr(self._L, f"swmhd_rk3_substep_{self.sfx}")
        rc = f(U, Gn, Gm, g.Nx, g.Ny, g.Hx, g.Hy, self._raw_fields[0].stride_y, dt, RK3_GAMMA[stage], RK3_ZETA[stage], 0, g.Ny,
               _lib.STRICT if self.strict else _lib.FAST, _stream_ptr())
        _lib.check(rc, "swmhd_rk3_substep")

    def _stage_fused(self, dt, stage, rows=None, extra_flags=0):
        g = self.grid
        j0, j1 = (0, g.Ny) if rows is None else rows
        q = _lib.ptr_array([f.ptr for f in self._raw_fields])
        qn = _lib.ptr_array([self._alt[n].ptr for n in self.names])
        Gn = _lib.ptr_array([f.ptr for f in self.Gn])
        gamma, zeta, store, prev_state = rk3_stage(stage, not self.strict and not any(self._bounded))
        if prev_state:
            Gm, extra_flags = qn, extra_flags | _lib.GM_IS_PREV_STATE
        else:
            Gm = _lib.ptr_array([f.ptr for f in self.Gm]) if stage > 0 else None
        f = getattr(self._L, f"swmhd_tendencies_rk3_{self.sfx}")
        timed = self.tendency_events is not None and 2 * (j1 - j0) > g.Ny
        if timed:
            e0, e1 = _lib.TimingEvent(), _lib.TimingEvent()
            e0.record()
        rc = f(q, qn, Gn, Gm, g.Nx, g.Ny, g.Hx, g.Hy, self._raw_fields[0].stride_y, g.dx, g.dy, self.g, self.f, self.form_code,
               self.lorentz_code, dt, gamma, zeta, store, j0, j1,
               self._flags | self._rwrap | extra_flags, _stream_ptr())
        if timed:
            e1.record()
            self.tendency_events.append((e0, e1, j1 - j0))
        _lib.check(rc, "swmhd_tendencies_rk3")

    def _native_steps(self, dt, n):
        import ctypes
        gr, ring = self.grid, self._ring is not None
        wrap = self._rwrap & _lib.WRAP_X if ring else self._rwrap
        if ring and self._halo_stale and not wrap:
            self.update_state()
        swapped = ctypes.c_int(0)
        args = (_lib.ptr_array([f.ptr for f in self._raw_fields]), _lib.ptr_array([self._alt[nm].ptr for nm in self.names]),
                _lib.ptr_array([f.ptr for f in self.Gn]), _lib.ptr_array([f.ptr for f in self.Gm]), gr.Nx, gr.Ny, gr.Hx, gr.Hy,
                self._raw_fields[0].stride_y, gr.dx, gr.dy, self.g, self.f, self.form_code, self.lorentz_code, dt, n,
                self._flags | wrap, ctypes.byref(swapped), _stream_ptr())
        if ring:
            self._ring_check(getattr(self._L, f"swmhd_ring_step_rk3_{self.sfx}")(self._ring, *args), "swmhd_ring_step_rk3")
        else:
            _lib.check(getattr(self._L, f"swmhd_step_rk3_{self.sfx}")(*args), "swmhd_step_rk3")
        if swapped.value:
            self._state, self._alt = self._alt, self._state
            self.Gn, self.Gm = self.Gm, self.Gn
        if n > 0 and wrap:
            self._halo_stale = True
        self.clock_time += n * dt
        self.iteration += n

    def time_step(self, dt):
        if self._ring is not None:
            return self._native_steps(dt, 1)
        g, H = self.grid, 3
        multi = self.decomp.ring
        overlap = multi and self.overlap and self._comm_stream is not None and g.Ny > 2 * H
        for stage in range(3):
            run = (lambda rows=None, fl=0: self._stage_fused(dt, stage, rows, fl)) if self.fused else (lambda rows=None, fl=0: self.calculate_tendencies(rows=rows))
            if overlap and self._exchange_in_flight:
                run((H, g.Ny - H), _lib.LEAVE_ROOM)
                with torch.cuda.stream(self._comm_stream):
                    run((0, H))
                    run((g.Ny - H, g.Ny))
                torch.cuda.current_stream().wait_stream(self._comm_stream)
            else:
                run()
            if self.fused:
                self._state, self._alt = self._alt, self._state
            else:
                self._substep(dt, stage)
            self.Gn, self.Gm = self.Gm, self.Gn
            if any(self._bounded) or not (self._rwrap & _lib.WRAP_X):
                self._fill_x()
            else:
                self._halo_stale = True
            if multi:
                if overlap:
                    self._comm_stream.wait_stream(torch.cuda.current_stream())
                    with torch.cuda.stream(self._comm_stream):
                        exchange_y_halos([f.data for f in self._raw_fields], g.Ny, g.Hy, self.decomp, self.group, depth=H)
                    self._exchange_in_flight = True
                else:
                    exchange_y_halos([f.data for f in self._raw_fields], g.Ny, g.Hy, self.decomp, self.group, depth=H)
        self.clock_time += dt
        self.iteration += 1

    def capture_graph(self, dt):
        if self.decomp.ring or not self.fused:
            raise _lib.SwmhdError("capture_graph: single-GPU fused path only (halo exchange is not capturable)")
        self._ensure_halos()
        keep = [f.data.clone() for f in self._raw_fields] + [f.data.clone() for f in self.Gm]
        t0, i0 = self.clock_time, self.iteration
        side = torch.cuda.Stream()
        side.wait_stream(torch.cuda.current_stream())
        with torch.cuda.stream(side):
            self.time_step(dt); self.time_step(dt)
        torch.cuda.current_stream().wait_stream(side)
        self._graph = torch.cuda.CUDAGraph()
        with torch.cuda.graph(self._graph):
            self.time_step(dt); self.time_step(dt)
        self._graph_dt = dt
        self._graph_roles = self._roles()
        for f, k in zip(self._raw_fields + self.Gm, keep):
            f.data.copy_(k)
        self._halo_stale = False
        self.clock_time, self.iteration = t0, i0
        return self

    def _roles(self):
        return tuple(f.ptr for f in self._raw_fields) + tuple(f.ptr for f in self.Gn)

    def time_steps(self, n, dt):
        g = getattr(self, "_graph", None)
        if g is not None and self._graph_dt == dt and n >= 2 and self._roles() != self._graph_roles:
            self._driver_steps(dt, 1)
            n -= 1
        if g is not None and self._graph_dt == dt and self._roles() == self._graph_roles:
            for _ in range(n // 2):
                g.replay()
                self._halo_stale = self._halo_stale or bool(self._rwrap)
                self.clock_time += 2 * dt
                self.iteration += 2
            n = n % 2
        if n > 0:
            self._driver_steps(dt, n)

    def _driver_steps(self, dt, n):
        if self._ring is not None or (not self.decomp.ring and self.fused and self.tendency_events is None and not any(self._bounded)):
            return self._native_steps(dt, n)
        for _ in range(n):
            self.time_step(dt)

    def diagnostics(self, h_ref=1.0):
        g = self.grid
        self._join()
        if not hasattr(self, "_diag_ws"):
            self._diag_ws = torch.empty(_lib.DIAG_WORKSPACE, dtype=torch.float64, device=self.fields[0].data.device)
            self._diag_out = torch.empty(_lib.DIAG_NOUT, dtype=torch.float64, device=self.fields[0].data.device)
        q = self.fields
        f = getattr(self._L, f"swmhd_diagnostics_{self.sfx}")
        rc = f(q[0].ptr, q[1].ptr, q[2].ptr, q[3].ptr, g.Nx, g.Ny, g.Hx, g.Hy, q[0].stride_y, g.dx, g.dy, self.g, h_ref,
               self.form_code, 0, g.Ny, self._diag_ws.data_ptr(), self._diag_out.data_ptr(), _stream_ptr())
        _lib.check(rc, "swmhd_diagnostics")
        out = self._diag_out.clone()
        if self.decomp.world_size > 1:
            import torch.distributed as dist
            sums, maxs, mins = out[:3].clone(), out[3:6].clone(), out[6:].clone()
            if sums.is_cuda and dist.get_backend(self.group) == "gloo":
                sums, maxs, mins = sums.cpu(), maxs.cpu(), mins.cpu()
            dist.all_reduce(sums, op=dist.ReduceOp.SUM, group=self.group)
            dist.all_reduce(maxs, op=dist.ReduceOp.MAX, group=self.group)
            dist.all_reduce(mins, op=dist.ReduceOp.MIN, group=self.group)
            out = torch.cat([sums.cpu(), maxs.cpu(), mins.cpu()])
        v = out.cpu().tolist()
        return dict(kinetic_energy=v[0], magnetic_energy=v[1], potential_energy=v[2], total_energy=v[0] + v[1] + v[2],
                    max_abs_u=v[3], max_abs_v=v[4], max_abs_A=v[5], min_h=v[6])

    def save_checkpoint(self, path):
        import numpy as np
        self.synchronize()
        np.savez(path, time=self.clock_time, iteration=self.iteration,
                 **{n: f.numpy() for n, f in zip(self.names, self.fields)},
                 **{"Gm_" + n: f.numpy() for n, f in zip(self.names, self.Gm)})

    def load_checkpoint(self, path):
        import numpy as np
        self._join()
        z = np.load(path, allow_pickle=False)
        self._halo_stale = False
        for n, f in zip(self.names, self._raw_fields):
            f.data.copy_(torch.from_numpy(z[n]).to(f.data.dtype))
        for n, f in zip(self.names, self.Gm):
            f.data.copy_(torch.from_numpy(z["Gm_" + n]).to(f.data.dtype))
        self.clock_time, self.iteration = float(z["time"]), int(z["iteration"])
        return self

    def synchronize(self):
        self._ensure_halos()
        self._join()
        torch.cuda.synchronize()
```

Before: 13640.

## Reformulate fast-path RK3 around a shared anchor state buffer

Replaces the low-storage RK3 update on the non-strict path with an anchored form. Stage 0 writes the anchor W = U + dt/4·G alongside the stage-1 state. Stages 1 and 2 then compute W + dt·γ·G directly, so they no longer store G or mix in the previous state and tendency. New march-kernel modes (9, 11), a flag, and API validation are added. The aim is fewer register-held terms and simpler read/write patterns per stage, but stage 0 gains an extra four-field store and the rounding differs from the previous scheme.

```diff
diff --git a/include/swmhd.h b/include/swmhd.h
--- a/include/swmhd.h
+++ b/include/swmhd.h
@@ -18,6 +18,7 @@
 #define SWMHD_BOUNDED_X 256
 #define SWMHD_BOUNDED_Y 512
 #define SWMHD_GM_IS_PREV_STATE 1024
+#define SWMHD_RK3_ANCHOR 2048
 #define SWMHD_LEAVE_ROOM 64
 
 #define SWMHD_PERIODIC 0
diff --git a/swmhd_amd/_lib.py b/swmhd_amd/_lib.py
--- a/swmhd_amd/_lib.py
+++ b/swmhd_amd/_lib.py
@@ -12,6 +12,7 @@
 WRAP_X, WRAP_Y = 16, 32
 LEAVE_ROOM = 64
 GM_IS_PREV_STATE = 1024
+RK3_ANCHOR = 2048
 BOUNDED_X, BOUNDED_Y = 256, 512
 KERNEL_FLAGS = {None: 0, "auto": 0, "tile": 2, "march": 4}
 PERIODIC, BOUNDED = 0, 1
diff --git a/swmhd_amd/csrc/common.hpp b/swmhd_amd/csrc/common.hpp
--- a/swmhd_amd/csrc/common.hpp
+++ b/swmhd_amd/csrc/common.hpp
@@ -63,8 +63,12 @@
     T dt, gamma, zeta;
     T dtg;
     T cu, cg;
+    int anchor;
+    T dtw;
 };
 constexpr int GM_IS_PREV_STATE = 1024;
+constexpr int RK3_ANCHOR = 2048;
+constexpr double RK3_ANCHOR_WEIGHT = 0.25;
 template <typename T>
 struct Rk3Stage {
     T gamma, zeta;
@@ -83,12 +87,11 @@
         }
         return true;
     }
-    Rk3Stage<T> stage(int st, bool from_state) const {
+    Rk3Stage<T> stage(int st, bool anchor) const {
         const T gam[3] = {T(8.0 / 15.0), T(5.0 / 12.0), T(3.0 / 4.0)};
         const T zet[3] = {T(0), T(-17.0 / 60.0), T(-5.0 / 12.0)};
-        const bool fs = from_state && st == 1;
-        return {gam[st], fs ? zet[1] / gam[0] : zet[st], (st == 1 || (st == 0 && !from_state)) ? 1 : 0,
-                st == 0 ? nullptr : (fs ? alt : gm), fs ? GM_IS_PREV_STATE : 0};
+        if (anchor) return {gam[st], st == 0 ? T(RK3_ANCHOR_WEIGHT) : T(0), 0, st == 0 ? nullptr : (st == 1 ? gm : gn), RK3_ANCHOR};
+        return {gam[st], zet[st], st < 2 ? 1 : 0, st == 0 ? nullptr : gm, 0};
     }
     void rotate() {
         for (int f = 0; f < 4; ++f) { T *t = cur[f]; cur[f] = alt[f]; alt[f] = t; t = gn[f]; gn[f] = gm[f]; gm[f] = t; }
diff --git a/swmhd_amd/csrc/ring.hip b/swmhd_amd/csrc/ring.hip
--- a/swmhd_amd/csrc/ring.hip
+++ b/swmhd_amd/csrc/ring.hip
@@ -215,7 +215,7 @@
         r->pending = nullptr;
     }
     hipError_t e;
-    const bool from_state = !(flags & SWMHD_STRICT);
+    const bool anchor = !(flags & SWMHD_STRICT);
     if ((e = hipEventRecord(r->ev_main, s)) != hipSuccess) return hipfail(r, "record", e);
     if ((e = hipStreamWaitEvent(c, r->ev_main, 0)) != hipSuccess) return hipfail(r, "wait", e);
     auto bail = [&](int code) {
@@ -245,7 +245,7 @@
         const int bflags = flags | ((!(flags & (SWMHD_STRICT | SWMHD_TILE_KERNEL | SWMHD_MARCH_KERNEL)) && Nx >= 1024) ? SWMHD_MARCH_KERNEL : 0);
         for (int n = 0; n < nsteps; ++n) {
             for (int st = 0; st < 3; ++st) {
-                const swmhd::Rk3Stage<T> g = b.stage(st, from_state);
+                const swmhd::Rk3Stage<T> g = b.stage(st, anchor);
                 if (int rc = run_interior(g, ilo[st], Ny - ilo[st], flags | SWMHD_LEAVE_ROOM)) return bail(rc);
                 if (st < 2) {
                     if ((e = hipEventRecord(r->ev_main, s)) != hipSuccess) return bail(hipfail(r, "record", e));
@@ -267,7 +267,7 @@
     }
     for (int n = 0; n < nsteps; ++n)
         for (int st = 0; st < 3; ++st) {
-            const swmhd::Rk3Stage<T> g = b.stage(st, from_state);
+            const swmhd::Rk3Stage<T> g = b.stage(st, anchor);
             int rc;
             const bool split = r->pending != nullptr;
             if ((rc = split ? run_interior(g, Hy, Ny - Hy, flags | SWMHD_LEAVE_ROOM) : run_interior(g, 0, Ny, flags))) return bail(rc);
diff --git a/swmhd_amd/csrc/swmhd_api.hip b/swmhd_amd/csrc/swmhd_api.hip
--- a/swmhd_amd/csrc/swmhd_api.hip
+++ b/swmhd_amd/csrc/swmhd_api.hip
@@ -99,9 +99,13 @@
     const int ext = ((flags & (SWMHD_WRAP_Y | SWMHD_BOUNDED_Y)) || Hy < 3) ? 0 : Hy - 3;
     if (j0 < -ext || j1 > Ny + ext || j0 > j1) return SWMHD_EINVAL;
     if (j1b > j0b && (j0b < j1 || j1b > Ny + ext)) return SWMHD_EINVAL;
-    if (flags & ~(SWMHD_STRICT | SWMHD_TILE_KERNEL | SWMHD_MARCH_KERNEL | SWMHD_WRAP_X | SWMHD_WRAP_Y | SWMHD_LEAVE_ROOM | SWMHD_BOUNDED_X | SWMHD_BOUNDED_Y | SWMHD_GM_IS_PREV_STATE)) return SWMHD_EINVAL;
+    if (flags & ~(SWMHD_STRICT | SWMHD_TILE_KERNEL | SWMHD_MARCH_KERNEL | SWMHD_WRAP_X | SWMHD_WRAP_Y | SWMHD_LEAVE_ROOM | SWMHD_BOUNDED_X | SWMHD_BOUNDED_Y | SWMHD_GM_IS_PREV_STATE | SWMHD_RK3_ANCHOR)) return SWMHD_EINVAL;
     if (flags & SWMHD_GM_IS_PREV_STATE) {
         if (!rk || !rk->Gm) return SWMHD_EINVAL;
+        if (flags & (SWMHD_STRICT | SWMHD_BOUNDED_X | SWMHD_BOUNDED_Y)) return SWMHD_ENOTSUP;
+    }
+    if (flags & SWMHD_RK3_ANCHOR) {
+        if (!rk || (flags & SWMHD_GM_IS_PREV_STATE)) return SWMHD_EINVAL;
         if (flags & (SWMHD_STRICT | SWMHD_BOUNDED_X | SWMHD_BOUNDED_Y)) return SWMHD_ENOTSUP;
     }
     if (((flags & SWMHD_BOUNDED_X) && (flags & SWMHD_WRAP_X)) || ((flags & SWMHD_BOUNDED_Y) && (flags & SWMHD_WRAP_Y))) return SWMHD_EINVAL;
@@ -121,7 +125,8 @@
     a.dx = dx; a.dy = dy; a.rdx = T(1) / dx; a.rdy = T(1) / dy; a.grav = grav; a.fcor = fcor; a.j0 = j0; a.j1 = j1;
     a.j0b = j1b > j0b ? j0b : 0; a.j1b = j1b > j0b ? j1b : 0;
     a.fuse = 0; a.first = 0; a.store_G = 1; a.drop_G = 0; a.dt = a.gamma = a.zeta = T(0);
-    a.gm_prev = (flags & SWMHD_GM_IS_PREV_STATE) ? 1 : 0; a.cu = a.cg = a.dtg = T(0);
+    a.gm_prev = (flags & SWMHD_GM_IS_PREV_STATE) ? 1 : 0; a.cu = a.cg = a.dtg = a.dtw = T(0);
+    a.anchor = (flags & SWMHD_RK3_ANCHOR) ? 1 : 0;
     a.wrap = ((flags & SWMHD_WRAP_X) ? 1 : 0) | ((flags & SWMHD_WRAP_Y) ? 2 : 0);
     a.leave_room = (flags & SWMHD_LEAVE_ROOM) ? 1 : 0;
     a.edge_cols = 0;
@@ -131,6 +136,10 @@
     if (rk) {
         a.fuse = 1; a.first = rk->Gm ? 0 : 1; a.store_G = rk->store_G; a.dt = rk->dt; a.gamma = rk->gamma; a.zeta = rk->zeta;
         a.cu = a.gm_prev ? rk->zeta : T(0); a.cg = a.gm_prev ? -rk->zeta : rk->dt * rk->zeta; a.dtg = rk->dt * rk->gamma;
+        if (a.anchor) {
+            a.store_G = 0; a.cu = a.cg = T(0);
+            a.dtw = rk->Gm ? T(0) : rk->dt * rk->zeta;
+        }
         for (int f = 0; f < 4; ++f) { a.Unew[f] = rk->Unew[f] + off; a.Gm[f] = rk->Gm ? rk->Gm[f] + off : nullptr; }
     }
     hipStream_t s = (hipStream_t)stream;
@@ -176,11 +185,11 @@
     if (flags & (SWMHD_BOUNDED_X | SWMHD_BOUNDED_Y)) return SWMHD_ENOTSUP;
     Rk3Buffers<T> b;
     if (!b.set(q, q_alt, Ga, Gb)) return SWMHD_EINVAL;
-    const bool from_state = !(flags & SWMHD_STRICT);
+    const bool anchor = !(flags & SWMHD_STRICT);
     const int need = (SWMHD_HALO_X | SWMHD_HALO_Y) & ~(((flags & SWMHD_WRAP_X) ? SWMHD_HALO_X : 0) | ((flags & SWMHD_WRAP_Y) ? SWMHD_HALO_Y : 0));
     for (int n = 0; n < nsteps; ++n)
         for (int st = 0; st < 3; ++st) {
-            const Rk3Stage<T> g = b.stage(st, from_state);
+            const Rk3Stage<T> g = b.stage(st, anchor);
             int rc = tend_rk3_common<T>(b.cur, b.alt, b.gn, g.Gm, Nx, Ny, Hx, Hy, sy, dx, dy, grav, fcor, formulation, lorentz, dt, g.gamma,
                                         g.zeta, g.store_G, 0, Ny, flags | g.flags, stream);
             if (rc) return rc;
@@ -219,6 +228,7 @@
     return halo_multi_common<T>(f, nf, Nx, Ny, Hx, Hy, (int64_t)sy, which, stream);
 }
 static_assert(GM_IS_PREV_STATE == SWMHD_GM_IS_PREV_STATE, "common.hpp mirrors swmhd.h");
+static_assert(RK3_ANCHOR == SWMHD_RK3_ANCHOR, "common.hpp mirrors swmhd.h");
 #define SW_INST(T)                                                                                                                   \
     template int tendencies_rk3_two_ranges<T>(const T *const *, T *const *, T *const *, const T *const *, int, int, int, int, long, T, \
                                               T, T, T, int, int, T, T, T, int, int, int, int, int, int, void *);                      \
diff --git a/swmhd_amd/csrc/tendency_march_kernels.inc b/swmhd_amd/csrc/tendency_march_kernels.inc
--- a/swmhd_amd/csrc/tendency_march_kernels.inc
+++ b/swmhd_amd/csrc/tendency_march_kernels.inc
@@ -9,7 +9,8 @@
 
 template <typename T, int LOR, int NT, int MODE>
 __global__ __launch_bounds__(NT, 3) void k_tendency_vi_march(TendArgs<T> a, int nstrips, int nseg, int LY) {
-    constexpr bool FUSE = (MODE & 1) != 0, HAS_GM = (MODE & 2) != 0, STORE_G = (MODE & 4) != 0;
+    constexpr bool FUSE = (MODE & 1) != 0, HAS_GM = (MODE & 2) != 0, STORE_G = (MODE & 4) != 0, ANCHOR = (MODE & 8) != 0;
+    constexpr bool STORE_W = ANCHOR && FUSE && !HAS_GM;
     constexpr int XH = 3, RW = NT + 2 * XH, TXO = NT - 2 * XH;
     __shared__ T Ru[3][RW];
     __shared__ T Rvn[1][RW];
@@ -45,7 +46,7 @@
     auto rowoff = [&](int row) -> unsigned { return (unsigned)((row + a.Hy) * isy) * (unsigned)sizeof(T); };
     const unsigned pbytes = (unsigned)((a.Ny + 2 * a.Hy) * isy) * (unsigned)sizeof(T);
     __amdgpu_buffer_rsrc_t rG[4], rU[4];
-    if constexpr (STORE_G) {
+    if constexpr (STORE_G || STORE_W) {
         rG[0] = out_rsrc(a.G1 - off0, pbytes); rG[1] = out_rsrc(a.G2 - off0, pbytes);
         rG[2] = out_rsrc(a.Gh - off0, pbytes); rG[3] = out_rsrc(a.GA - off0, pbytes);
     }
@@ -198,13 +199,19 @@
             for (int f = 0; f < 4; ++f) {
                 T un;
                 if constexpr (!HAS_GM) un = Us[f] + a.dtg * Gs[f];
+                else if constexpr (ANCHOR) un = fma_<T>(a.dtg, Gs[f], Gms[f]);
                 else if constexpr (STORE_G) un = fma_<T>(a.cg, Gms[f], fma_<T>(a.dtg, Gs[f], fma_<T>(a.cu, Us[f], Us[f])));
                 else un = Us[f] + a.dt * (a.gamma * Gs[f] + a.zeta * Gms[f]);
                 buffer_store<T>(un, rU[f], o);
             }
         }
+        if constexpr (STORE_W) {
+            const T Us[4] = {U[3], V[2], Hh[2], Aa[2]};
+#pragma unroll
+            for (int f = 0; f < 4; ++f) buffer_store<T>(Us[f] + a.dtw * Gs[f], rG[f], o);
+        }
         fhy = fhy_n; fay = fay_n; km = kc;
-        constexpr int YOUNGER = ((FUSE && HAS_GM) ? 4 : 0) + (STORE_G ? 4 : 0) + (FUSE ? 4 : 0);
+        constexpr int YOUNGER = ((FUSE && HAS_GM) ? 4 : 0) + (STORE_G ? 4 : 0) + (FUSE ? 4 : 0) + (STORE_W ? 4 : 0);
         wait_vmem_all_but<YOUNGER>();
     };
     auto shift1 = [&]() {
@@ -226,11 +233,12 @@
     }
 }
 
-constexpr int CONS_W3_MODES = (1 << 7) | (1 << 5) | (1 << 4);
+constexpr int CONS_W3_MODES = (1 << 7) | (1 << 5) | (1 << 4) | (1 << 9) | (1 << 11);
 constexpr int cons_minwaves(int mode, int elem_size) { return elem_size == 4 ? 3 : (((CONS_W3_MODES >> mode) & 1) ? 3 : 2); }
 template <typename T, int LOR, int NT, int MODE>
 __global__ __launch_bounds__(NT, cons_minwaves(MODE, (int)sizeof(T))) void k_tendency_cons_march(TendArgs<T> a, int nstrips, int nseg, int LY) {
-    constexpr bool FUSE = (MODE & 1) != 0, HAS_GM = (MODE & 2) != 0, STORE_G = (MODE & 4) != 0;
+    constexpr bool FUSE = (MODE & 1) != 0, HAS_GM = (MODE & 2) != 0, STORE_G = (MODE & 4) != 0, ANCHOR = (MODE & 8) != 0;
+    constexpr bool STORE_W = ANCHOR && FUSE && !HAS_GM;
     constexpr int XH = 3, RW = NT + 2 * XH, TXO = NT - 2 * XH;
     __shared__ T Ruh[3][RW];
     __shared__ T Rvh[3][RW];
@@ -283,7 +291,7 @@
     };
     const unsigned pbytes = (unsigned)((a.Ny + 2 * a.Hy) * isy) * (unsigned)sizeof(T);
     __amdgpu_buffer_rsrc_t rG[4], rU[4];
-    if constexpr (STORE_G) {
+    if constexpr (STORE_G || STORE_W) {
         rG[0] = out_rsrc(a.G1 - off0, pbytes); rG[1] = out_rsrc(a.G2 - off0, pbytes);
         rG[2] = out_rsrc(a.Gh - off0, pbytes); rG[3] = out_rsrc(a.GA - off0, pbytes);
     }
@@ -503,15 +511,21 @@
                 for (int f = 0; f < 4; ++f) {
                     T un;
                     if constexpr (!HAS_GM) un = Us[f] + a.dtg * Gs[f];
+                    else if constexpr (ANCHOR) un = fma_<T>(a.dtg, Gs[f], Gms[f]);
                     else if constexpr (STORE_G) un = fma_<T>(a.cg, Gms[f], fma_<T>(a.dtg, Gs[f], fma_<T>(a.cu, Us[f], Us[f])));
-                else un = Us[f] + a.dt * (a.gamma * Gs[f] + a.zeta * Gms[f]);
+                    else un = Us[f] + a.dt * (a.gamma * Gs[f] + a.zeta * Gms[f]);
                     buffer_store<T>(un, rU[f], o);
                 }
             }
+            if constexpr (STORE_W) {
+                const T Us[4] = {uw[2], vw[2], hc, aw[2]};
+#pragma unroll
+                for (int f = 0; f < 4; ++f) buffer_store<T>(Us[f] + a.dtw * Gs[f], rG[f], o);
+            }
         }
         d1 = d1n; d2 = d2n; fya_s = fya_n; hff_s = hff_n; vs_ = vn;
         }
-        constexpr int YOUNGER = STEADY ? ((FUSE && HAS_GM) ? 4 : 0) + (STORE_G ? 4 : 0) + (FUSE ? 4 : 0) : 0;
+        constexpr int YOUNGER = STEADY ? ((FUSE && HAS_GM) ? 4 : 0) + (STORE_G ? 4 : 0) + (FUSE ? 4 : 0) + (STORE_W ? 4 : 0) : 0;
         wait_vmem_all_but<YOUNGER>();
         insert_row(nu, nv, nh, na);
     };
diff --git a/swmhd_amd/csrc/tendency_pk_kernels.inc b/swmhd_amd/csrc/tendency_pk_kernels.inc
--- a/swmhd_amd/csrc/tendency_pk_kernels.inc
+++ b/swmhd_amd/csrc/tendency_pk_kernels.inc
@@ -4,7 +4,8 @@
 __global__ __launch_bounds__(NT, 3) void k_tendency_vi_march_pk(TendArgs<float> a, int nstrips, int nseg, int LY) {
     using T = sw_f2;
     using S = float;
-    constexpr bool FUSE = (MODE & 1) != 0, HAS_GM = (MODE & 2) != 0, STORE_G = (MODE & 4) != 0;
+    constexpr bool FUSE = (MODE & 1) != 0, HAS_GM = (MODE & 2) != 0, STORE_G = (MODE & 4) != 0, ANCHOR = (MODE & 8) != 0;
+    constexpr bool STORE_W = ANCHOR && FUSE && !HAS_GM;
     constexpr int XL = 2, PAD = 4, RW = 2 * NT + 2 * PAD, TXO = 2 * (NT - 2 * XL);
     __shared__ __attribute__((aligned(8))) S Ru[3][RW];
     __shared__ __attribute__((aligned(8))) S Rvn[1][RW];
@@ -48,7 +49,7 @@
     auto rowoff = [&](int row) -> unsigned { return (unsigned)((row + a.Hy) * isy) * (unsigned)sizeof(S); };
     const unsigned pbytes = (unsigned)((a.Ny + 2 * a.Hy) * isy) * (unsigned)sizeof(S);
     __amdgpu_buffer_rsrc_t rG[4], rU[4];
-    if constexpr (STORE_G) {
+    if constexpr (STORE_G || STORE_W) {
         rG[0] = out_rsrc(a.G1 - off0, pbytes); rG[1] = out_rsrc(a.G2 - off0, pbytes);
         rG[2] = out_rsrc(a.Gh - off0, pbytes); rG[3] = out_rsrc(a.GA - off0, pbytes);
     }
@@ -195,13 +196,19 @@
             for (int f = 0; f < 4; ++f) {
                 T un;
                 if constexpr (!HAS_GM) un = Us[f] + T(a.dtg) * Gs[f];
+                else if constexpr (ANCHOR) un = fma_<T>(T(a.dtg), Gs[f], Gms[f]);
                 else if constexpr (STORE_G) un = fma_<T>(T(a.cg), Gms[f], fma_<T>(T(a.dtg), Gs[f], fma_<T>(T(a.cu), Us[f], Us[f])));
                 else un = Us[f] + T(a.dt) * (T(a.gamma) * Gs[f] + T(a.zeta) * Gms[f]);
                 buffer_store<T>(un, rU[f], o);
             }
         }
+        if constexpr (STORE_W) {
+            const T Us[4] = {U[3], V[2], Hh[2], Aa[2]};
+#pragma unroll
+            for (int f = 0; f < 4; ++f) buffer_store<T>(Us[f] + T(a.dtw) * Gs[f], rG[f], o);
+        }
         fhy = fhy_n; fay = fay_n; km = kc;
-        constexpr int YOUNGER = ((FUSE && HAS_GM) ? 4 : 0) + (STORE_G ? 4 : 0) + (FUSE ? 4 : 0);
+        constexpr int YOUNGER = ((FUSE && HAS_GM) ? 4 : 0) + (STORE_G ? 4 : 0) + (FUSE ? 4 : 0) + (STORE_W ? 4 : 0);
         wait_vmem_all_but<YOUNGER>();
 #pragma unroll
         for (int k = 0; k < 7; ++k) uw[k] = uw[k + 1];
diff --git a/swmhd_amd/csrc/tendency_tile_kernels.inc b/swmhd_amd/csrc/tendency_tile_kernels.inc
--- a/swmhd_amd/csrc/tendency_tile_kernels.inc
+++ b/swmhd_amd/csrc/tendency_tile_kernels.inc
@@ -217,10 +217,18 @@
             if (a.fuse) {
                 const T Gs[4] = {G1, G2, Gh, GA};
                 const T Us[4] = {U_(i, j), V_(i, j), H_(i, j), A_(i, j)};
+                T *const Gp[4] = {a.G1, a.G2, a.Gh, a.GA};
 #pragma unroll
                 for (int f = 0; f < 4; ++f) {
                     T un;
-                    if (a.first) {
+                    if (!STRICT && !BND && a.anchor) {
+                        if (a.first) {
+                            un = Us[f] + a.dtg * Gs[f];
+                            Gp[f][o] = Us[f] + a.dtw * Gs[f];
+                        } else {
+                            un = a.Gm[f][o] + a.dtg * Gs[f];
+                        }
+                    } else if (a.first) {
                         if constexpr (STRICT) un = Us[f] + a.dt * a.gamma * Gs[f];
                         else un = Us[f] + (a.dt * a.gamma) * Gs[f];
                     } else if (!STRICT && a.gm_prev) {
@@ -355,7 +363,7 @@
             const MarchGeometry mg = packed_fp32_geometry(a.Nx, rows, a.leave_room);
             const int nstrips = mg.nstrips, LY = mg.LY, nseg = two ? two_range_segments(LY) : mg.nseg;
             dim3 mgrid(nstrips * nseg), mblock(256);
-            int mode = (a.fuse ? 1 : 0) | ((a.fuse && !a.first) ? 2 : 0) | ((a.store_G || !a.fuse) ? 4 : 0);
+            int mode = (a.fuse ? 1 : 0) | ((a.fuse && !a.first) ? 2 : 0) | ((a.store_G || !a.fuse) ? 4 : 0) | (a.anchor ? 8 : 0);
             TendArgs<T> ap = a;
             if (a.gm_prev && mode == 3) { mode = 7; ap.drop_G = 1; }
 #define SW_PK_MARCH(MODE_)                                                                                                  \
@@ -363,13 +371,14 @@
                 if (lorentz == 1) hipLaunchKernelGGL((k_tendency_vi_march_pk<1, 256, MODE_>), mgrid, mblock, 0, s, ap, nstrips, nseg, LY); \
                 else hipLaunchKernelGGL((k_tendency_vi_march_pk<0, 256, MODE_>), mgrid, mblock, 0, s, ap, nstrips, nseg, LY);            \
                 break;
-            switch (mode) { SW_PK_MARCH(4) SW_PK_MARCH(5) SW_PK_MARCH(1) SW_PK_MARCH(7) SW_PK_MARCH(3) default: return hipErrorInvalidValue; }
+            switch (mode) { SW_PK_MARCH(4) SW_PK_MARCH(5) SW_PK_MARCH(1) SW_PK_MARCH(7) SW_PK_MARCH(3) SW_PK_MARCH(9) SW_PK_MARCH(11)
+                            default: return hipErrorInvalidValue; }
 #undef SW_PK_MARCH
             return hipGetLastError();
         }
     }
     if (march) {
-        int mode = (a.fuse ? 1 : 0) | ((a.fuse && !a.first) ? 2 : 0) | ((a.store_G || !a.fuse) ? 4 : 0);
+        int mode = (a.fuse ? 1 : 0) | ((a.fuse && !a.first) ? 2 : 0) | ((a.store_G || !a.fuse) ? 4 : 0) | (a.anchor ? 8 : 0);
         TendArgs<T> ax = a;
         if (formulation == 0 && mode == 3 && sizeof(T) == 8 && cons_minwaves(7, 8) > cons_minwaves(3, 8)) {
             mode = 7; ax.drop_G = 1;
@@ -392,7 +401,8 @@
                 if (mg.nt == 128) SW_VI_GO(128, MODE_);                                                                         \
                 else SW_VI_GO(256, MODE_);                                                                                      \
                 break;
-            switch (mode) { SW_VI_MARCH(4) SW_VI_MARCH(5) SW_VI_MARCH(1) SW_VI_MARCH(7) SW_VI_MARCH(3) default: return hipErrorInvalidValue; }
+            switch (mode) { SW_VI_MARCH(4) SW_VI_MARCH(5) SW_VI_MARCH(1) SW_VI_MARCH(7) SW_VI_MARCH(3) SW_VI_MARCH(9) SW_VI_MARCH(11)
+                            default: return hipErrorInvalidValue; }
 #undef SW_VI_MARCH
 #undef SW_VI_GO
         } else {
@@ -406,7 +416,8 @@
                     else hipLaunchKernelGGL((k_tendency_cons_march<T, 0, 256, MODE_>), mgrid, mblock, 0, s, ax, nstrips, nseg, LY);            \
                 }                                                                                                               \
                 break;
-            switch (mode) { SW_CONS_MARCH(4) SW_CONS_MARCH(5) SW_CONS_MARCH(1) SW_CONS_MARCH(7) SW_CONS_MARCH(3) default: return hipErrorInvalidValue; }
+            switch (mode) { SW_CONS_MARCH(4) SW_CONS_MARCH(5) SW_CONS_MARCH(1) SW_CONS_MARCH(7) SW_CONS_MARCH(3) SW_CONS_MARCH(9) SW_CONS_MARCH(11)
+                            default: return hipErrorInvalidValue; }
 #undef SW_CONS_MARCH
         }
         return hipGetLastError();
diff --git a/swmhd_amd/model.py b/swmhd_amd/model.py
--- a/swmhd_amd/model.py
+++ b/swmhd_amd/model.py
@@ -10,10 +10,13 @@
 RK3_ZETA = (0.0, -17.0 / 60.0, -5.0 / 12.0)
 
 
-def rk3_stage(stage, from_state):
-    fs = from_state and stage == 1
-    store = 1 if stage == 1 or (stage == 0 and not from_state) else 0
-    return RK3_GAMMA[stage], RK3_ZETA[1] / RK3_GAMMA[0] if fs else RK3_ZETA[stage], store, fs
+RK3_ANCHOR_WEIGHT = 0.25
+
+
+def rk3_stage(stage, anchor):
+    if anchor:
+        return RK3_GAMMA[stage], RK3_ANCHOR_WEIGHT if stage == 0 else 0.0, 0, True
+    return RK3_GAMMA[stage], RK3_ZETA[stage], 1 if stage < 2 else 0, False
 
 
 def loopback_rings(nranks, timeout_s=60.0):
@@ -247,9 +250,10 @@
         q = _lib.ptr_array([f.ptr for f in self._raw_fields])
         qn = _lib.ptr_array([self._alt[n].ptr for n in self.names])
         Gn = _lib.ptr_array([f.ptr for f in self.Gn])
-        gamma, zeta, store, prev_state = rk3_stage(stage, not self.strict and not any(self._bounded))
-        if prev_state:
-            Gm, extra_flags = qn, extra_flags | _lib.GM_IS_PREV_STATE
+        gamma, zeta, store, anchor = rk3_stage(stage, not self.strict and not any(self._bounded))
+        if anchor:
+            extra_flags |= _lib.RK3_ANCHOR
+            Gm = None if stage == 0 else _lib.ptr_array([f.ptr for f in (self.Gm if stage == 1 else self.Gn)])
         else:
             Gm = _lib.ptr_array([f.ptr for f in self.Gm]) if stage > 0 else None
         f = getattr(self._L, f"swmhd_tendencies_rk3_{self.sfx}")
```

New measurement: 14070, median of 6. 3.1% higher.
